# lexsightllc/DEWI-Design-for-an-Entropy-Weighted-Index-for-Text-Image-Corpora

Hardware: AMD Instinct MI355X
Metric: queries/sec + p50 latency, 1M×768 corpus, k=10, η=0.3, at 1/2/4/8 GPUs (higher is better)
Workload: dtype f32; 1 GPU; 1000000 docs x d=768 fp32, query batch=1, k=10, eta=0.3, brute-force cosine kNN + DEWI re-rank (BASELINE.json configs[1]); docs=1000000, dim=768, k=10, batch=1, candidates=20, parallelism=single GPU, queries_in_flight=1, rows_per_gpu=1000000, conditioning_steps_before_warmup=455

## Files before the change

### dewi-design-for-an-entropy-weighted-index-for-text-image-corpora_amd/csrc/abi.cpp

```cpp
#include <hip/hip_runtime.h>
#include <stdlib.h>

#include <cmath>
#include <cstdarg>
#include <cstdio>
#include <cstring>
#include <mutex>
#include <vector>

#include "launch.hpp"

namespace {

thread_local char g_err[512] = "";

int fail(int code, const char* fmt, ...) {
  va_list ap;
  va_start(ap, fmt);
  vsnprintf(g_err, sizeof(g_err), fmt, ap);
  va_end(ap);
  return code;
}
int hip_fail(hipError_t e, const char* what) {
  return fail(DEWI_ERR_HIP, "%s: %s", what, hipGetErrorString(e));
// ... 133 lines not shown
  return rp;
}

struct Batch {
  const void* d_E; int elem_type; int64_t n_rows; int dim;
  const float* d_Q; int n_queries;
  int space; hipStream_t stream;
};

struct SelectOut {
  int k; dewi::RerankParams rp;
  const float* d_dewi32; const float* d_ent32; int64_t id_offset;
  int64_t* d_out_ids; float* d_out_scores; dewi_candidate* d_out_cand;
};

int run_scan(const KnnLayout& L, const Batch& B, int n_candidates, char* ws, const uint32_t* d_filter = nullptr,
             const uint32_t* d_qwords = nullptr, int64_t n_union = 0) {
  uint64_t* keys = reinterpret_cast<uint64_t*>(ws + L.keys_off);
  float* qn = reinterpret_cast<float*>(ws + L.qn_off);
  hipError_t e;
  if (!L.plan.raw_queries) {
    e = dewi::launch_prepare_queries(B.d_Q, qn, B.n_queries, B.dim, B.space, B.elem_type ? 1 : 0, B.stream);
    if (e != hipSuccess) return hip_fail(e, "prepare_queries");
  }
  ScanTimer timer(B.stream);
  const float* q_prepared = L.plan.raw_queries ? nullptr : qn;
  int q = 0;
  while (q < B.n_queries) {
    static const bool nq8_enabled = [] { const char* e = getenv("DEWI_SCAN_NQ8"); return e == nullptr || atoi(e) != 0; }();
    const bool can8 = !B.elem_type && L.plan.fast && L.plan.slots == 1 && nq8_enabled;
    const int left = B.n_queries - q;
    const int nq = (can8 && left >= 8) ? 8 : ((L.plan.nq_max > 1 && left >= L.plan.nq_max) ? L.plan.nq_max : 1);
    if (d_filter) {
      dewi::QWords qw;
      if (d_qwords) {
        qw.words = d_qwords + static_cast<int64_t>(q / 32) * n_union;
        qw.shift = q % 32;
      }
      e = dewi::launch_scan_f32_filtered(L.plan, static_cast<const float*>(B.d_E), B.dim, B.d_Q, q_prepared, q, nq, n_candidates,
                                         B.space, keys, d_filter, B.stream, qw);
    } else if (B.elem_type) {
      e = dewi::launch_scan_bf16(L.plan, static_cast<const uint16_t*>(B.d_E), B.n_rows, B.dim, B.d_Q, q_prepared, q, nq,
                                 n_candidates, B.space, keys, B.stream);
    } else {
      e = dewi::launch_scan_f32(L.plan, static_cast<const float*>(B.d_E), B.n_rows, B.dim, B.d_Q, q_prepared, q, nq, n_candidates,
                                B.space, keys, B.stream);
    }
    if (e != hipSuccess) return hip_fail(e, "scan launch");
    q += nq;
  }
  return DEWI_OK;
}

int check_common(const Batch& B) {
  if (!B.d_E || !B.d_Q) return fail(DEWI_ERR_INVALID_ARG, "null embedding or query pointer");
  if (B.n_rows <= 0) return fail(DEWI_ERR_INVALID_ARG, "n_rows must be positive (got %lld)", static_cast<long long>(B.n_rows));
  if (B.n_rows > 0xFFFFFFFFll) return fail(DEWI_ERR_UNSUPPORTED, "n_rows %lld exceeds 2^32-1 rows per device", static_cast<long long>(B.n_rows));
  if (B.dim <= 0) return fail(DEWI_ERR_INVALID_ARG, "dim must be positive (got %d)", B.dim);
  if (B.n_queries <= 0) return fail(DEWI_ERR_INVALID_ARG, "n_queries must be positive (got %d)", B.n_queries);
  if (B.space != DEWI_SPACE_COSINE && B.space != DEWI_SPACE_L2) return fail(DEWI_ERR_INVALID_ARG, "unknown space %d", B.space);
  return DEWI_OK;
}

int resolve_cut(int k, int64_t n, int n_override, int* c) {
  int64_t c64 = (2ll * k < n) ? 2ll * k : n;
  if (n_override > 0) {
    if (n_override < k) return fail(DEWI_ERR_INVALID_ARG, "n_candidates %d must be at least k = %d", n_override, k);
    c64 = n_override < n ? n_override : n;
  }
  if (c64 > (1ll << 30)) return fail(DEWI_ERR_UNSUPPORTED, "candidate count %lld exceeds 2^30", static_cast<long long>(c64));
  *c = static_cast<int>(c64);
  return DEWI_OK;
}

enum class BatchPath { Rows, Depth, Big };
struct BatchPlan {
  BatchPath path;
  int c_local;
  KnnLayout rows;
  dewi::MfmaF32Layout depth;
  dewi::MfmaLayout big;
  bool shadow;
  size_t flags_off;
  size_t total;
};

bool plan_repair(BatchPlan& P, size_t path_total, int64_t n_rows, int dim, int corpus_elem_bytes, int n_queries, int n_candidates,
                 int cus) {
  if (n_candidates > dewi::kMaxSortCandidates) return false;
  P.rows = layout_knn(n_rows, dim, corpus_elem_bytes, n_queries, n_candidates, cus);
  if (!dewi::scan_flagged_supported(P.rows.plan, corpus_elem_bytes)) return false;
  P.flags_off = align_up(path_total > P.rows.total ? path_total : P.rows.total, 256);
  P.total = P.flags_off + align_up(static_cast<size_t>(n_queries) * 4, 256);
  return true;
}

BatchPlan plan_batch(int elem_type, int64_t n_rows, int dim, int n_queries, int n_candidates, int space, int cus) {
  BatchPlan P{};
  const int elem_bytes = elem_type ? 2 : 4;
  P.c_local = n_candidates < n_rows ? n_candidates : static_cast<int>(n_rows);
  const bool mfma = g_tuning.mfma != 0 && P.c_local == n_candidates &&
                    (space == DEWI_SPACE_COSINE || elem_type == 0 || g_tuning.mfma == 2);
  const bool depth_ok = mfma && dewi::mfma_f32_path_supported(elem_type, n_rows, dim, n_queries, n_candidates, space);
  const bool big_ok = mfma && elem_type == 1 && dewi::mfma_path_supported(n_rows, dim, n_queries, n_candidates, space);
  bool repairable = false;
  if (depth_ok && (elem_type == 0 || n_queries <= 32 || !big_ok)) {
    P.path = BatchPath::Depth;
    P.depth = dewi::plan_mfma_f32(elem_type, n_rows, dim, n_queries, n_candidates, cus);
    repairable = plan_repair(P, P.depth.total, n_rows, dim, elem_bytes, n_queries, n_candidates, cus);
  } else if (big_ok) {
    P.path = BatchPath::Big;
    P.big = dewi::plan_mfma(n_rows, dim, n_queries, n_candidates, cus);
    repairable = plan_repair(P, P.big.total, n_rows, dim, elem_bytes, n_queries, n_candidates, cus);
  }
  if (!repairable) {
    P.path = BatchPath::Rows;
    P.rows = layout_knn(n_rows, dim, elem_bytes, n_queries, P.c_local, cus);
    P.total = P.rows.total;
  }
  return P;
}

int batch_scan(const BatchPlan& P, const Batch& B, int n_candidates, void* d_ws, size_t ws_bytes, int cus) {
  if (int rc = check_workspace(d_ws, ws_bytes, P.total)) return rc;
  char* ws = static_cast<char*>(d_ws);
  switch (P.path) {
    case BatchPath::Depth:
      return launched(dewi::launch_mfma_f32(P.depth, B.elem_type, B.d_E, B.n_rows, B.dim, B.d_Q, B.n_queries, n_candidates, B.space,
                                            ws, B.stream),
                      "depth-split mfma scan launch");
    case BatchPath::Big:
      return launched(dewi::launch_mfma_bf16(P.big, static_cast<const uint16_t*>(B.d_E), B.n_rows, B.dim, B.d_Q, B.n_queries,
                                             n_candidates, B.space, ws, cus, B.stream),
                      "mfma scan launch");
    default:
      return run_scan(P.rows, B, P.c_local, ws);
  }
}

int batch_repair(const BatchPlan& P, char* ws, const Batch& B, const SelectOut& O, int n_candidates) {
  const KnnLayout& L = P.rows;
  uint32_t* flags = reinterpret_cast<uint32_t*>(ws + P.flags_off);
  uint64_t* keys = reinterpret_cast<uint64_t*>(ws + L.keys_off);
  hipError_t e = B.elem_type ? dewi::launch_scan_flagged_bf16(L.plan, static_cast<const uint16_t*>(B.d_E), B.n_rows, B.dim, B.d_Q,
                                                              B.n_queries, n_candidates, B.space, keys, flags, B.stream)
                             : dewi::launch_scan_flagged_f32(L.plan, static_cast<const float*>(B.d_E), B.n_rows, B.dim, B.d_Q,
                                                             B.n_queries, n_candidates, B.space, keys, flags, B.stream);
  if (e != hipSuccess) return hip_fail(e, "repair scan launch");
  const int sorted = L.plan.slots == 1 ? L.plan.n_lists : 0;
  e = dewi::launch_select_rerank(keys, L.plan.keys_per_query, sorted, B.n_queries, n_candidates, O.k, O.rp, O.d_dewi32, O.d_ent32,
                                 O.id_offset, O.d_out_ids, O.d_out_scores, O.d_out_cand, nullptr, dewi::SegmentLayout{}, B.stream,
                                 dewi::RefineParams{nullptr, nullptr, nullptr, 0, 0.f, 0}, dewi::QueryFlags{flags, 2});
  return launched(e, "repair select launch");
}

int batch_select(const BatchPlan& P, const Batch& B, const SelectOut& O, int n_candidates, void* d_ws, size_t ws_bytes) {
  if (int rc = check_workspace(d_ws, ws_bytes, P.total)) return rc;
  char* ws = static_cast<char*>(d_ws);
  const int n_queries = B.n_queries, k = O.k;
  hipError_t e = hipSuccess;
  if (P.path == BatchPath::Rows && P.c_local > dewi::kMaxSortCandidates) {
    const KnnLayout& L = P.rows;
    uint64_t* g1 = reinterpret_cast<uint64_t*>(ws + L.big_off);
    e = dewi::launch_select_rerank_large(reinterpret_cast<const uint64_t*>(ws + L.keys_off), L.plan.keys_per_query, n_queries,
                                         P.c_local, L.p2, k, O.rp, O.d_dewi32, O.d_ent32, O.id_offset, g1,
                                         g1 + static_cast<size_t>(n_queries) * L.p2, O.d_out_ids, O.d_out_scores, O.d_out_cand,
                                         n_candidates, B.stream);
    return launched(e, "select_rerank_large launch");
  }
  if (P.path == BatchPath::Rows) {
    const KnnLayout& L = P.rows;
    const int sorted = (L.plan.slots == 1 && P.c_local == n_candidates) ? L.plan.n_lists : 0;
    e = dewi::launch_select_rerank(reinterpret_cast<const uint64_t*>(ws + L.keys_off), L.plan.keys_per_query, sorted, n_queries,
                                   n_candidates, k, O.rp, O.d_dewi32, O.d_ent32, O.id_offset, O.d_out_ids, O.d_out_scores,
                                   O.d_out_cand, nullptr, dewi::SegmentLayout{}, B.stream);
    return launched(e, "select launch");
  }
  const bool big = P.path == BatchPath::Big;
  const int per = big ? 256 : 32;
  const int groups = big ? P.big.groups : P.depth.groups;
  const int n_seg = big ? P.big.n_seg : P.depth.n_seg;
  const int seg_cap = big ? P.big.seg_cap : P.depth.seg_cap;
  const size_t cand_off = big ? P.big.cand_off : P.depth.cand_off, cnt_off = big ? P.big.cnt_off : P.depth.cnt_off;
  static const int stage_override = [] { const char* e = getenv("DEWI_STAGE_KEYS"); return e ? atoi(e) : 0; }();
  const int stage_keys = stage_override > 0 ? stage_override : ((big && P.shadow) ? 12288 : 8192);
  const dewi::SegmentLayout seg{n_seg, seg_cap, 1, static_cast<int64_t>(per) * seg_cap, big ? 1 : per, stage_keys, big ? n_seg : 1};
  const bool refine_l2 = !big && B.space == DEWI_SPACE_L2 && B.elem_type == 0;
  if (!B.d_E || !B.d_Q) return fail(DEWI_ERR_INVALID_ARG, "a matrix-core batch needs the corpus and the raw queries in its finish step (repair of refused queries)");
  uint32_t* flags = reinterpret_cast<uint32_t*>(ws + P.flags_off);
  for (int g = 0; g < groups && e == hipSuccess; ++g) {
    const int q0 = g * per;
    const int nq = n_queries - q0 < per ? n_queries - q0 : per;
    const uint64_t* keys = reinterpret_cast<const uint64_t*>(ws + cand_off) + static_cast<int64_t>(g) * n_seg * per * seg_cap;
    const uint32_t* counts = reinterpret_cast<const uint32_t*>(ws + cnt_off) + static_cast<int64_t>(g) * n_seg * per;
    dewi::RefineParams rf{nullptr, nullptr, nullptr, 0, 0.f, 0};
    if (refine_l2)
      rf = dewi::RefineParams{static_cast<const float*>(B.d_E),
                              reinterpret_cast<const float*>(ws + P.depth.qn_off) + static_cast<int64_t>(q0) * B.dim,
                              reinterpret_cast<const float*>(ws + P.depth.qn2_off) + q0, B.dim, dewi::depth_l2_margin(B.dim),
                              DEWI_SPACE_L2};
    else if (P.shadow)
      rf = dewi::RefineParams{static_cast<const float*>(B.d_E), B.d_Q + static_cast<int64_t>(q0) * B.dim, nullptr, B.dim,
                              dewi::shadow_margin(B.dim), DEWI_SPACE_COSINE};
    e = dewi::launch_select_rerank(keys, 0, 0, nq, n_candidates, k, O.rp, O.d_dewi32, O.d_ent32, O.id_offset,
                                   O.d_out_ids ? O.d_out_ids + static_cast<int64_t>(q0) * k : nullptr,
                                   O.d_out_scores ? O.d_out_scores + static_cast<int64_t>(q0) * k : nullptr,
                                   O.d_out_cand ? O.d_out_cand + static_cast<int64_t>(q0) * n_candidates : nullptr, counts, seg,
                                   B.stream, rf, dewi::QueryFlags{flags + q0, 1});
  }
  if (e != hipSuccess) return hip_fail(e, "select launch");
  return batch_repair(P, ws, B, O, n_candidates);
}

int knn_rerank_impl(const Batch& B, const float* d_dewi32, const float* d_ent32, int k, double eta, double pref,
                    int64_t* d_out_ids, float* d_out_scores, void* d_ws, size_t ws_bytes, int n_candidates_override = 0,
                    int transform = DEWI_SIM_RAW) {
  int rc = check_common(B);
  if (rc) return rc;
  if (k <= 0) return DEWI_OK;
  if (k > B.n_rows)
    return fail(DEWI_ERR_K_OUT_OF_BOUNDS, "kth(=%lld) out of bounds (%lld)", static_cast<long long>(B.n_rows - k),
                static_cast<long long>(B.n_rows));
  if (!d_dewi32 || !d_ent32 || !d_out_ids || !d_out_scores) return fail(DEWI_ERR_INVALID_ARG, "null payload or output pointer");
  int c = 0;
  rc = resolve_cut(k, B.n_rows, n_candidates_override, &c);
  if (rc) return rc;
  DeviceInfo dev;
  rc = ensure_device(dev);
  if (rc) return rc;
  const BatchPlan P = plan_batch(B.elem_type, B.n_rows, B.dim, B.n_queries, c, B.space, dev.cus);
  rc = batch_scan(P, B, c, d_ws, ws_bytes, dev.cus);
  if (rc) return rc;
  const SelectOut O{k, make_rerank(eta, pref, transform, B.space), d_dewi32, d_ent32, 0, d_out_ids, d_out_scores, nullptr};
  return batch_select(P, B, O, c, d_ws, ws_bytes);
}

enum class ShadowMode { Plain, Lists, Big, Depth };
struct ShadowPlan {
  ShadowMode mode;
  int c;
  int list_len;
  KnnLayout lists;
  BatchPlan P;
};

ShadowPlan plan_shadow(bool have_shadow, int64_t n_rows, int dim, int n_queries, int k, int space, int cus) {
  ShadowPlan S{};
  S.mode = ShadowMode::Plain;
  S.P.shadow = true;
  const int64_t c64 = (2ll * k < n_rows) ? 2ll * k : n_rows;
  S.c = static_cast<int>(c64 < (1ll << 30) ? c64 : (1ll << 30));
  const bool usable = have_shadow && g_tuning.mfma != 0 && space == DEWI_SPACE_COSINE && k > 0 && k <= n_rows &&
                      dim % 8 == 0 && dim >= 136 && dim <= 1536;
  if (!usable) return S;
  const bool use_big = n_queries > 32 && c64 <= 512 && dewi::mfma_path_supported(n_rows, dim, n_queries, S.c, space);
  const bool use_depth = !use_big && c64 <= 256 &&
                         dewi::mfma_f32_path_supported(1, n_rows, dim, n_queries < dewi::kMfmaMinQueries ? dewi::kMfmaMinQueries : n_queries,
                                                       S.c, space);
  const int list_len = (n_queries == 1 && n_rows >= 64 * 1024) ? dewi::shadow_list_len(static_cast<int>(c64 < 64 ? c64 : 64)) : 0;
  if (list_len > 0) {
    S.lists = layout_knn(n_rows, dim, 2, 1, list_len, cus);
    if (S.lists.plan.fast && S.lists.plan.slots == 1 && S.lists.plan.n_lists <= 4 * 64 &&
        plan_repair(S.P, S.lists.total, n_rows, dim, 4, 1, S.c, cus)) {
      S.mode = ShadowMode::Lists;
      S.list_len = list_len;
      return S;
    }
  }
  S.P.c_local = S.c;
  if (use_big) {
    S.P.path = BatchPath::Big;
    S.P.big = dewi::plan_mfma(n_rows, dim, n_queries, S.c, cus, true);
    if (plan_repair(S.P, S.P.big.total, n_rows, dim, 4, n_queries, S.c, cus)) S.mode = ShadowMode::Big;
  } else if (use_depth) {
    S.P.path = BatchPath::Depth;
    S.P.depth = dewi::plan_mfma_f32(1, n_rows, dim, n_queries, S.c, cus, true);
    if (plan_repair(S.P, S.P.depth.total, n_rows, dim, 4, n_queries, S.c, cus)) S.mode = ShadowMode::Depth;
  }
  return S;
}

}

extern "C" {

int dewi_abi_version(void) { return DEWI_ABI_VERSION; }
const char* dewi_last_error(void) { return g_err; }

int dewi_device_info(int* out_compute_units, int* out_wavefront, size_t* out_total_mem) {
  DeviceInfo d;
  int rc = ensure_device(d);
  if (rc) return rc;
  if (out_compute_units) *out_compute_units = d.cus;
  if (out_wavefront) *out_wavefront = d.wave;
  if (out_total_mem) *out_total_mem = d.mem;
  return DEWI_OK;
}

int dewi_normalize_rows_f32(const float* d_src, float* d_dst, int64_t n_rows, int dim, void* stream) {
  if (n_rows < 0 || dim <= 0) return fail(DEWI_ERR_INVALID_ARG, "bad shape %lld x %d", static_cast<long long>(n_rows), dim);
  if (n_rows == 0) return DEWI_OK;
  if (!d_src || !d_dst) return fail(DEWI_ERR_INVALID_ARG, "null pointer");
  return launched(dewi::launch_normalize_rows(d_src, d_dst, n_rows, dim, static_cast<hipStream_t>(stream)), "normalize_rows launch");
}

int dewi_row_cosine_f32(const float* d_a, const float* d_b, float* d_out, int64_t n_rows, int dim, void* stream) {
  if (n_rows < 0 || dim <= 0) return fail(DEWI_ERR_INVALID_ARG, "bad shape %lld x %d", static_cast<long long>(n_rows), dim);
  if (n_rows == 0) return DEWI_OK;
  if (!d_a || !d_b || !d_out) return fail(DEWI_ERR_INVALID_ARG, "null pointer");
  return launched(dewi::launch_row_cosine(d_a, d_b, d_out, n_rows, dim, 1e-8f, static_cast<hipStream_t>(stream)), "row_cosine launch");
}

int dewi_convert_f32_to_bf16(const float* d_src, uint16_t* d_dst, int64_t n_elems, void* stream) {
  if (n_elems < 0) return fail(DEWI_ERR_INVALID_ARG, "negative element count");
  if (n_elems == 0) return DEWI_OK;
  if (!d_src || !d_dst) return fail(DEWI_ERR_INVALID_ARG, "null pointer");
  return launched(dewi::launch_f32_to_bf16(d_src, d_dst, n_elems, static_cast<hipStream_t>(stream)), "f32_to_bf16 launch");
}

int dewi_payload_soa_f64(const double* d_dewi, const double* d_ht_mean, const double* d_hi_mean, float* d_dewi32,
                         float* d_ent32, int64_t n_rows, void* stream) {
  if (n_rows < 0) return fail(DEWI_ERR_INVALID_ARG, "negative row count");
  if (n_rows == 0) return DEWI_OK;
  if (!d_dewi || !d_ht_mean || !d_hi_mean || !d_dewi32 || !d_ent32) return fail(DEWI_ERR_INVALID_ARG, "null pointer");
  return launched(dewi::launch_payload_soa(d_dewi, d_ht_mean, d_hi_mean, d_dewi32, d_ent32, n_rows, static_cast<hipStream_t>(stream)),
                  "payload_soa launch");
}

size_t dewi_knn_workspace_bytes(int64_t n_rows, int dim, int n_queries, int n_candidates) {
  DeviceInfo dev;
  if (ensure_device(dev)) return 0;
  if (n_rows <= 0 || dim <= 0 || n_queries <= 0 || n_candidates <= 0) return 0;
  size_t a = layout_knn(n_rows, dim, 4, n_queries, n_candidates, dev.cus).total;
  const size_t b = layout_knn(n_rows, dim, 2, n_queries, n_candidates, dev.cus).total;
  if (b > a) a = b;
  if (const int ll = dewi::shadow_list_len(n_candidates)) {
    const size_t s = layout_knn(n_rows, dim, 2, n_queries, ll, dev.cus).total;
    if (s > a) a = s;
  }
  if (dewi::mfma_path_supported(n_rows, dim, n_queries, n_candidates, DEWI_SPACE_COSINE)) {
    for (int pre = 0; pre < 2; ++pre) {
      const size_t m = dewi::plan_mfma(n_rows, dim, n_queries, n_candidates, dev.cus, pre != 0).total;
      if (m > a) a = m;
    }
  }
  for (int et = 0; et < 2; ++et) {
    const int nq = et == 1 && n_queries < dewi::kMfmaMinQueries ? dewi::kMfmaMinQueries : n_queries;
    if (dewi::mfma_f32_path_supported(et, n_rows, dim, nq, n_candidates, DEWI_SPACE_COSINE)) {
      for (int pre = 0; pre < 2; ++pre) {
        const size_t m = dewi::plan_mfma_f32(et, n_rows, dim, n_queries, n_candidates, dev.cus, pre != 0).total;
        if (m > a) a = m;
      }
    }
  }
  return align_up(a, 256) + align_up(static_cast<size_t>(n_queries) * 4, 256);
}

int dewi_knn_scan_kernel(int elem_type, int64_t n_rows, int dim, int n_queries, int n_candidates, int space, char* out,
                         size_t out_bytes) {
  if (!out || out_bytes < 16) return fail(DEWI_ERR_INVALID_ARG, "name buffer too small");
  if (n_rows <= 0 || dim <= 0 || n_queries <= 0 || n_candidates <= 0) return fail(DEWI_ERR_INVALID_ARG, "non-positive size");
  DeviceInfo dev;
  int rc = ensure_device(dev);
  if (rc) return rc;
  const BatchPlan P = plan_batch(elem_type, n_rows, dim, n_queries, n_candidates < n_rows ? n_candidates : static_cast<int>(n_rows),
                                 space, dev.cus);
  const char* e = elem_type ? "bf16" : "f32";
  if (P.path == BatchPath::Depth) {
    snprintf(out, out_bytes, "mfma_scan_f32<%s", elem_type ? "true" : "false");
  } else if (P.path == BatchPath::Big) {
    snprintf(out, out_bytes, "mfma_scan_bf16_s16");
  } else {
    const dewi::ScanPlan& p = P.rows.plan;
    const int nq = n_queries >= p.nq_max ? p.nq_max : 1;
    switch (p.kind) {
      case dewi::kScanFast: snprintf(out, out_bytes, "scan_rows_%s", e); break;
      case dewi::kScanAnyLong:
        if (p.odd_contig && nq == 1) {
          snprintf(out, out_bytes, "scan_rows_odd_contig<%d, %d, %d, %d, %d>", elem_type ? 1 : 0, p.u_pad, p.odd_contig_rows, space, p.slots);
          break;
        }
        snprintf(out, out_bytes, "scan_rows_any<%d, %d, %d, %d, %d, %d, %s>", elem_type ? 1 : 0, p.u_pad,
                                        nq > 1 ? p.rows_per_iter_batch : p.rows_per_iter, nq, space, p.slots,
                                        p.odd_rows ? "true" : "false"); break;
      case dewi::kScanAnyShort: snprintf(out, out_bytes, "scan_short_rows_any<%d, %d, %d, %d, %d, %s>", elem_type ? 1 : 0,
                                         p.rows_per_iter / (64 >> p.log2p), nq, space, p.slots, p.odd_rows ? "true" : "false"); break;
      default: snprintf(out, out_bytes, "scan_generic_%s", e); break;
    }
  }
  return DEWI_OK;
}

int dewi_knn_rerank_f32(const float* d_E, int64_t n_rows, int dim, const float* d_Q, int n_queries,
                        const float* d_dewi32, const float* d_ent32, int k, double eta, double entropy_pref, int space,
                        int64_t* d_out_ids, float* d_out_scores, void* d_workspace, size_t workspace_bytes,
                        void* stream) {
  return knn_rerank_impl(Batch{d_E, 0, n_rows, dim, d_Q, n_queries, space, static_cast<hipStream_t>(stream)}, d_dewi32, d_ent32, k,
                         eta, entropy_pref, d_out_ids, d_out_scores, d_workspace, workspace_bytes);
}

int dewi_knn_rerank_f32_shadow(const float* d_E, const uint16_t* d_E_bf16, int64_t n_rows, int dim, const float* d_Q,
                               int n_queries, const float* d_dewi32, const float* d_ent32, int k, double eta,
                               double entropy_pref, int space, int64_t* d_out_ids, float* d_out_scores, void* d_workspace,
                               size_t workspace_bytes, void* stream_) {
  const Batch B{d_E, 0, n_rows, dim, d_Q, n_queries, space, static_cast<hipStream_t>(stream_)};
  int rc = check_common(B);
  if (rc) return rc;
  DeviceInfo dev;
  rc = ensure_device(dev);
  if (rc) return rc;
  const ShadowPlan S = plan_shadow(d_E_bf16 != nullptr, n_rows, dim, n_queries, k, space, dev.cus);
  if (S.mode == ShadowMode::Plain)
    return knn_rerank_impl(B, d_dewi32, d_ent32, k, eta, entropy_pref, d_out_ids, d_out_scores, d_workspace, workspace_bytes);
  if (!d_dewi32 || !d_ent32 || !d_out_ids || !d_out_scores) return fail(DEWI_ERR_INVALID_ARG, "null payload or output pointer");
  const BatchPlan& P = S.P;
  rc = check_workspace(d_workspace, workspace_bytes, P.total);
  if (rc) return rc;
  char* ws = static_cast<char*>(d_workspace);
  hipStream_t stream = B.stream;
  const SelectOut O{k, make_rerank(eta, entropy_pref, DEWI_SIM_RAW, space), d_dewi32, d_ent32, 0, d_out_ids, d_out_scores, nullptr};
  if (S.mode == ShadowMode::Lists) {
    const KnnLayout& L = S.lists;
    rc = run_scan(L, Batch{d_E_bf16, 1, n_rows, dim, d_Q, 1, space, stream}, S.list_len, ws);
    if (rc) return rc;
    const dewi::RefineParams rf{d_E, d_Q, nullptr, dim, dewi::shadow_margin(dim), DEWI_SPACE_COSINE, S.list_len};
    const hipError_t e = dewi::launch_select_rerank(reinterpret_cast<const uint64_t*>(ws + L.keys_off), L.plan.keys_per_query,
                                                    L.plan.n_lists, 1, S.c, k, O.rp, d_dewi32, d_ent32, 0, d_out_ids, d_out_scores,
                                                    nullptr, nullptr, dewi::SegmentLayout{}, stream, rf,
                                                    dewi::QueryFlags{reinterpret_cast<uint32_t*>(ws + P.flags_off), 1});
    if (e != hipSuccess) return hip_fail(e, "select launch (one query, bf16 shadow)");
    return batch_repair(P, ws, B, O, S.c);
  }
  const float bias = 2.f * dewi::shadow_margin(dim);
  hipError_t e = S.mode == ShadowMode::Big
                     ? dewi::launch_mfma_bf16(P.big, d_E_bf16, n_rows, dim, d_Q, n_queries, S.c, space, ws, dev.cus, stream, bias)
                     : dewi::launch_mfma_f32(P.depth, 1, d_E_bf16, n_rows, dim, d_Q, n_queries, S.c, space, ws, stream, bias);
  if (e != hipSuccess) return hip_fail(e, "mfma scan launch (bf16 shadow)");
  return batch_select(P, B, O, S.c, d_workspace, workspace_bytes);
}

int dewi_knn_refusal_flags(int elem_type, int through_shadow, int64_t n_rows, int dim, int n_queries, int k, int n_candidates,
                           int space, size_t* out_offset_bytes) {
  if (!out_offset_bytes) return fail(DEWI_ERR_INVALID_ARG, "null pointer");
  if (n_rows <= 0 || dim <= 0 || n_queries <= 0) return fail(DEWI_ERR_INVALID_ARG, "non-positive size");
  DeviceInfo dev;
  int rc = ensure_device(dev);
  if (rc) return rc;
  *out_offset_bytes = static_cast<size_t>(-1);
  if (through_shadow && elem_type == 0) {
    const ShadowPlan S = plan_shadow(true, n_rows, dim, n_queries, k, space, dev.cus);
    if (S.mode != ShadowMode::Plain) {
      *out_offset_bytes = S.P.flags_off;
      return DEWI_OK;
    }
  }
  int64_t c64 = n_candidates > 0 ? n_candidates : 2ll * k;
  if (c64 > n_rows) c64 = n_rows;
  if (c64 <= 0 || c64 > (1ll << 30)) return DEWI_OK;
  const BatchPlan P = plan_batch(elem_type, n_rows, dim, n_queries, static_cast<int>(c64), space, dev.cus);
  if (P.path != BatchPath::Rows) *out_offset_bytes = P.flags_off;
  return DEWI_OK;
}

int dewi_knn_rerank_candidates(const void* d_E, int elem_type, int64_t n_rows, int dim, const float* d_Q, int n_queries,
                               const float* d_dewi32, const float* d_ent32, int k, int n_candidates, double eta,
                               double entropy_pref, int space, int sim_transform, int64_t* d_out_ids,
                               float* d_out_scores, void* d_workspace, size_t workspace_bytes, void* stream) {
  if (n_candidates <= 0) return fail(DEWI_ERR_INVALID_ARG, "n_candidates must be positive (got %d)", n_candidates);
  if (sim_transform != DEWI_SIM_RAW && sim_transform != DEWI_SIM_ONE_MINUS_DIST && sim_transform != DEWI_SIM_INV_ONE_PLUS_DIST)
    return fail(DEWI_ERR_INVALID_ARG, "unknown sim_transform %d", sim_transform);
  return knn_rerank_impl(Batch{d_E, elem_type, n_rows, dim, d_Q, n_queries, space, static_cast<hipStream_t>(stream)}, d_dewi32,
                         d_ent32, k, eta, entropy_pref, d_out_ids, d_out_scores, d_workspace, workspace_bytes, n_candidates,
                         sim_transform);
}

int dewi_prepare_queries_bf16(const float* d_Q, int n_queries, int dim, int space, uint16_t* d_out, void* stream) {
  if (!d_Q || !d_out) return fail(DEWI_ERR_INVALID_ARG, "null pointer");
  if (n_queries <= 0 || dim <= 0) return fail(DEWI_ERR_INVALID_ARG, "non-positive size");
  if (space != DEWI_SPACE_COSINE && space != DEWI_SPACE_L2) return fail(DEWI_ERR_INVALID_ARG, "unknown space %d", space);
  return launched(dewi::launch_prepare_queries_bf16(d_Q, d_out, n_queries, n_queries, dim, space, nullptr, static_cast<hipStream_t>(stream)),
                  "prepare_queries_bf16 launch");
}

int dewi_knn_scan(const void* d_E, int elem_type, int64_t n_rows, int dim, const float* d_Q, int n_queries,
                  int n_candidates, int space, void* d_workspace, size_t workspace_bytes, void* stream_) {
  const Batch B{d_E, elem_type, n_rows, dim, d_Q, n_queries, space, static_cast<hipStream_t>(stream_)};
  int rc = check_common(B);
  if (rc) return rc;
  if (n_candidates <= 0) return DEWI_OK;
  if (n_candidates > (1 << 30)) return fail(DEWI_ERR_UNSUPPORTED, "n_candidates %d exceeds 2^30", n_candidates);
  DeviceInfo dev;
  rc = ensure_device(dev);
  if (rc) return rc;
  const BatchPlan P = plan_batch(elem_type, n_rows, dim, n_queries, n_candidates, space, dev.cus);
  return batch_scan(P, B, n_candidates, d_workspace, workspace_bytes, dev.cus);
}

int dewi_knn_finish(void* d_workspace, size_t workspace_bytes, const void* d_E, int elem_type, int64_t n_rows, int dim,
                    const float* d_Q, int n_queries, int n_candidates, int space, int k, double eta, double entropy_pref,
                    const float* d_dewi32, const float* d_ent32, int64_t id_offset, int64_t* d_out_ids,
                    float* d_out_scores, dewi_candidate* d_out_cand, void* stream_) {
  if (n_rows <= 0 || dim <= 0 || n_queries <= 0) return fail(DEWI_ERR_INVALID_ARG, "non-positive size");
  if (space != DEWI_SPACE_COSINE && space != DEWI_SPACE_L2) return fail(DEWI_ERR_INVALID_ARG, "unknown space %d", space);
  if (n_candidates <= 0) return DEWI_OK;
  if (n_candidates > (1 << 30)) return fail(DEWI_ERR_UNSUPPORTED, "n_candidates %d exceeds 2^30", n_candidates);
  if (!d_dewi32 || !d_ent32) return fail(DEWI_ERR_INVALID_ARG, "null payload pointer");
  const bool records = d_out_cand != nullptr;
  if (!records) {
    if (k <= 0) return DEWI_OK;
    if (k > n_candidates) return fail(DEWI_ERR_K_OUT_OF_BOUNDS, "kth(=%d) out of bounds (%d)", n_candidates - k, n_candidates);
    if (!d_out_ids || !d_out_scores) return fail(DEWI_ERR_INVALID_ARG, "null output pointer");
  } else if (id_offset < 0 || id_offset + n_rows > 0x7FFFFFFFll) {
// ... 886 lines not shown
```

### dewi-design-for-an-entropy-weighted-index-for-text-image-corpora_amd/csrc/knn_scan.hip

```cpp
#include "scan_any.hpp"

namespace dewi {

template <int U, int R, int NQ, int SPACE, int S, bool NT, bool LIST = false, bool QMASK = false>
__device__ __forceinline__ void scan_rows_f32_body(const float* __restrict__ E, int64_t n_rows,
                                                   const float* __restrict__ Q, int n_candidates,
                                                   uint64_t* __restrict__ keys, int64_t keys_per_query,
                                                   MergeShared& merge_buf, const uint32_t* __restrict__ filt = nullptr,
                                                   const uint32_t* __restrict__ qword = nullptr, int qshift = 0) {
  constexpr int D4 = 64 * U;
  constexpr bool DENSE = S == 0;
  const int lane = lane_id();
  const int wave_in_block = static_cast<int>(threadIdx.x) >> 6;
  const int64_t gwave = static_cast<int64_t>(blockIdx.x) * (kScanThreads / kWave) + wave_in_block;
  const int64_t n_waves = static_cast<int64_t>(gridDim.x) * (kScanThreads / kWave);

  f32x4 qf[NQ][U];
#pragma unroll
  for (int qi = 0; qi < NQ; ++qi) {
    const f32x4* qp = reinterpret_cast<const f32x4*>(Q) + static_cast<int64_t>(qi) * D4 + lane;
#pragma unroll
    for (int u = 0; u < U; ++u) qf[qi][u] = qp[u * 64];
    if constexpr (SPACE == DEWI_SPACE_COSINE) {
      double ss = 0.0;
// ... 72 lines not shown
      for (int r = 0; r < R; ++r) consume(v[r], rows[r], row0 + r, qbits[r]);
      slot = (slot + 1) & (kWave - 1);
    }
  } else if constexpr (LIST) {
    uint32_t ahead[R];
    int slot = 0;
    for (int64_t g = gwave; g < n_groups; g += n_waves) {
      if (slot == 0) {
        const int64_t gl = g + static_cast<int64_t>(lane) * n_waves;
#pragma unroll
        for (int r = 0; r < R; ++r) ahead[r] = gl < n_groups ? list[gl * R + r] : 0u;
      }
      const int64_t row0 = g * R;
      int64_t rows[R];
      f32x4 v[R][U];
#pragma unroll
      for (int r = 0; r < R; ++r) {
        rows[r] = static_cast<uint32_t>(__builtin_amdgcn_readlane(static_cast<int>(ahead[r]), slot));
        const f32x4* p = Ev + rows[r] * D4 + lane;
#pragma unroll
        for (int u = 0; u < U; ++u) v[r][u] = load_x4<NT>(p + u * 64);
      }
#pragma unroll
      for (int r = 0; r < R; ++r) consume(v[r], rows[r], row0 + r);
      slot = (slot + 1) & (kWave - 1);
    }
  } else {
  for (int64_t g = gwave; g < n_groups; g += n_waves) {
    const int64_t row0 = g * R;
    f32x4 v[R][U];
#pragma unroll
    for (int r = 0; r < R; ++r) {
      const f32x4* p = Ev + row_of(row0 + r) * D4 + lane;
#pragma unroll
      for (int u = 0; u < U; ++u) v[r][u] = load_x4<NT>(p + u * 64);
    }
#pragma unroll
    for (int r = 0; r < R; ++r) consume(v[r], row_of(row0 + r), row0 + r);
  }
  }
  for (int64_t row = n_groups * R + gwave; row < n_rows; row += n_waves) {
    f32x4 v[U];
    const f32x4* p = Ev + row_of(row) * D4 + lane;
#pragma unroll
    for (int u = 0; u < U; ++u) v[u] = load_x4<NT>(p + u * 64);
    if constexpr (QMASK) consume(v, row_of(row), row, static_cast<uint32_t>(__builtin_amdgcn_readfirstlane(static_cast<int>(qword[row]))));
    else consume(v, row_of(row), row);
  }

  DEWI_STORE_LISTS(S, NQ, lst);
}

template <int U, int R, int NQ, int SPACE, int S, bool NT>
__global__ __launch_bounds__(kScanThreads) void scan_rows_f32(const float* __restrict__ E, int64_t n_rows,
                                                              const float* __restrict__ Q, int n_candidates,
                                                              uint64_t* __restrict__ keys,
                                                              int64_t keys_per_query) {
  __shared__ MergeShared merge_buf;
  scan_rows_f32_body<U, R, NQ, SPACE, S, NT>(E, n_rows, Q, n_candidates, keys, keys_per_query, merge_buf);
}

template <int U, int R, int NQ, int SPACE, int S, bool NT>
__global__ __launch_bounds__(kScanThreads) void scan_rows_f32_list(const float* __restrict__ E, const uint32_t* __restrict__ filt,
                                                                   const float* __restrict__ Q, int n_candidates,
                                                                   uint64_t* __restrict__ keys, int64_t keys_per_query) {
  __shared__ MergeShared merge_buf;
  scan_rows_f32_body<U, R, NQ, SPACE, S, NT, true>(E, 0, Q, n_candidates, keys, keys_per_query, merge_buf, filt);
}

template <int U, int R, int NQ, int SPACE, int S, bool NT>
__global__ __launch_bounds__(kScanThreads) void scan_rows_f32_qmask(const float* __restrict__ E, const uint32_t* __restrict__ filt,
                                                                    const uint32_t* __restrict__ qword, int qshift,
                                                                    const float* __restrict__ Q, int n_candidates,
                                                                    uint64_t* __restrict__ keys, int64_t keys_per_query) {
  __shared__ MergeShared merge_buf;
  scan_rows_f32_body<U, R, NQ, SPACE, S, NT, true, true>(E, 0, Q, n_candidates, keys, keys_per_query, merge_buf, filt, qword,
                                                          qshift);
}

template <int U, int R, int SPACE, int S>
__global__ __launch_bounds__(kScanThreads) void scan_rows_f32_flagged(const float* __restrict__ E, int64_t n_rows,
                                                                      const float* __restrict__ Q, int n_candidates,
                                                                      uint64_t* __restrict__ keys, int64_t keys_per_query,
                                                                      const uint32_t* __restrict__ flags, int n_queries) {
  __shared__ MergeShared merge_buf;
  for_each_flagged(flags, n_queries, [&](int q) {
    scan_rows_f32_body<U, R, 1, SPACE, S, true>(E, n_rows, Q + static_cast<int64_t>(q) * (256 * U), n_candidates,
                                                keys + static_cast<int64_t>(q) * keys_per_query, keys_per_query, merge_buf);
  });
}

template <int VEC>
struct VecT;
template <>
struct VecT<1> { using type = float; };
template <>
struct VecT<4> { using type = f32x4; };

template <int VEC, int NQ, int SPACE, int S>
__global__ __launch_bounds__(kScanThreads) void scan_generic_f32(const float* __restrict__ E, int64_t n_rows, int dim,
                                                                 const float* __restrict__ Qn, int group,
                                                                 int n_candidates, uint64_t* __restrict__ keys,
                                                                 int64_t keys_per_query) {
  using V = typename VecT<VEC>::type;
  constexpr bool DENSE = S == 0;
  __shared__ MergeShared merge_buf;
  const int lane = lane_id();
  const int wave_in_block = static_cast<int>(threadIdx.x) >> 6;
  const int64_t gwave = static_cast<int64_t>(blockIdx.x) * (kScanThreads / kWave) + wave_in_block;
  const int64_t n_waves = static_cast<int64_t>(gridDim.x) * (kScanThreads / kWave);
  const int rows_per_step = kWave / group;
  const int sub = lane / group;
  const int lg = lane % group;
  const int units = dim / VEC;

  ScanLists<S, NQ> lst;
  DEWI_INIT_LISTS(S, NQ, lst);

  const int64_t n_steps = (n_rows + rows_per_step - 1) / rows_per_step;
  for (int64_t st = gwave; st < n_steps; st += n_waves) {
    const int64_t row = st * rows_per_step + sub;
    float acc[NQ];
#pragma unroll
    for (int qi = 0; qi < NQ; ++qi) acc[qi] = 0.f;
    if (row < n_rows) {
      const V* ep = reinterpret_cast<const V*>(E + row * dim);
      for (int u = lg; u < units; u += group) {
        const V e = ep[u];
#pragma unroll
        for (int qi = 0; qi < NQ; ++qi) {
          const V q = reinterpret_cast<const V*>(Qn + static_cast<int64_t>(qi) * dim)[u];
          if constexpr (VEC == 4) {
            acc[qi] = accum4<SPACE>(e, q, acc[qi]);
          } else {
            if constexpr (SPACE == DEWI_SPACE_COSINE) {
              acc[qi] = __builtin_fmaf(e, q, acc[qi]);
            } else {
              const float d = e - q;
              acc[qi] = __builtin_fmaf(d, d, acc[qi]);
            }
          }
        }
      }
    }
    for (int off = group >> 1; off > 0; off >>= 1) {
#pragma unroll
      for (int qi = 0; qi < NQ; ++qi) acc[qi] += __shfl_xor(acc[qi], off, kWave);
    }
    for (int r = 0; r < rows_per_step; ++r) {
      const int64_t rr = st * rows_per_step + r;
      if (rr >= n_rows) break;
#pragma unroll
      for (int qi = 0; qi < NQ; ++qi) {
        float s = __shfl(acc[qi], r * group, kWave);
        if constexpr (SPACE == DEWI_SPACE_L2) s = -s;
        if constexpr (DENSE) {
          if (lane == 0) keys[qi * keys_per_query + rr] = make_key(s, static_cast<uint32_t>(rr));
        } else {
          lst[qi].offer(s, static_cast<uint32_t>(rr), lane);
        }
      }
    }
  }
  DEWI_STORE_LISTS(S, NQ, lst);
}

template <int VEC, int NQ, int SPACE, int S>
__global__ __launch_bounds__(kScanThreads) void scan_generic_f32_list(const float* __restrict__ E, const uint32_t* __restrict__ filt, int dim,
                                                                      const float* __restrict__ Qn, int group,
                                                                      int n_candidates, uint64_t* __restrict__ keys,
                                                                      int64_t keys_per_query) {
// ... 371 lines not shown

template <int U, int NQ, int SPACE, int S, bool LIST>
static bool launch_fast_r(const ScanPlan& plan, const float* E, int64_t n_rows, const float* Q, int c,
                          uint64_t* keys, hipStream_t stream, const uint32_t* filt, QWords qw) {
  const int r = NQ >= 4 ? plan.rows_per_iter_batch : plan.rows_per_iter;
  if (r >= 8) {
    if constexpr (U <= 3 && NQ == 1 && S == 1) {
      launch_fast_nt<U, 8, NQ, SPACE, S, LIST>(plan, E, n_rows, Q, c, keys, stream, filt, qw);
      return true;
    }
  }
  if (r >= 4) {
    if constexpr (U <= 3 && NQ == 1) {
      launch_fast_nt<U, 4, NQ, SPACE, S, LIST>(plan, E, n_rows, Q, c, keys, stream, filt, qw);
      return true;
    }
  }
  if (r >= 2) {
    if constexpr (U <= 3) {
      launch_fast_nt<U, 2, NQ, SPACE, S, LIST>(plan, E, n_rows, Q, c, keys, stream, filt, qw);
      return true;
    }
  }
  launch_fast_nt<U, 1, NQ, SPACE, S, LIST>(plan, E, n_rows, Q, c, keys, stream, filt, qw);
  return true;
}

template <int NQ, int SPACE, int S, bool LIST>
static bool launch_fast_u(const ScanPlan& plan, int dim, const float* E, int64_t n_rows, const float* Q, int c,
                          uint64_t* keys, hipStream_t stream, const uint32_t* filt, QWords qw) {
  switch (dim / 256) {
    case 1: return launch_fast_r<1, NQ, SPACE, S, LIST>(plan, E, n_rows, Q, c, keys, stream, filt, qw);
    case 2: return launch_fast_r<2, NQ, SPACE, S, LIST>(plan, E, n_rows, Q, c, keys, stream, filt, qw);
    case 3: return launch_fast_r<3, NQ, SPACE, S, LIST>(plan, E, n_rows, Q, c, keys, stream, filt, qw);
    case 4: return launch_fast_r<4, NQ, SPACE, S, LIST>(plan, E, n_rows, Q, c, keys, stream, filt, qw);
    case 6: return launch_fast_r<6, NQ, SPACE, S, LIST>(plan, E, n_rows, Q, c, keys, stream, filt, qw);
    default: return false;
  }
}

template <int NQ, int SPACE, int S, bool LIST>
static void launch_generic(const ScanPlan& plan, int dim, const float* E, int64_t n_rows, const float* Qn, int c,
                           uint64_t* keys, hipStream_t stream, const uint32_t* filt, QWords qw) {
  if constexpr (LIST) {
    if (qw.words) {
      if (plan.vec == 4)
        hipLaunchKernelGGL((scan_generic_f32_qmask<4, NQ, SPACE, S>), dim3(plan.blocks), dim3(kScanThreads), 0, stream, E,
                           filt, qw.words, qw.shift, dim, Qn, plan.group, c, keys, plan.keys_per_query);
      else
        hipLaunchKernelGGL((scan_generic_f32_qmask<1, NQ, SPACE, S>), dim3(plan.blocks), dim3(kScanThreads), 0, stream, E,
                           filt, qw.words, qw.shift, dim, Qn, plan.group, c, keys, plan.keys_per_query);
      return;
    }
    if (plan.vec == 4)
      hipLaunchKernelGGL((scan_generic_f32_list<4, NQ, SPACE, S>), dim3(plan.blocks), dim3(kScanThreads), 0, stream, E,
                         filt, dim, Qn, plan.group, c, keys, plan.keys_per_query);
    else
      hipLaunchKernelGGL((scan_generic_f32_list<1, NQ, SPACE, S>), dim3(plan.blocks), dim3(kScanThreads), 0, stream, E,
                         filt, dim, Qn, plan.group, c, keys, plan.keys_per_query);
    return;
  }
  if (plan.vec == 4)
    hipLaunchKernelGGL((scan_generic_f32<4, NQ, SPACE, S>), dim3(plan.blocks), dim3(kScanThreads), 0, stream, E,
                       n_rows, dim, Qn, plan.group, c, keys, plan.keys_per_query);
  else
    hipLaunchKernelGGL((scan_generic_f32<1, NQ, SPACE, S>), dim3(plan.blocks), dim3(kScanThreads), 0, stream, E,
                       n_rows, dim, Qn, plan.group, c, keys, plan.keys_per_query);
}

template <int NQ, int SPACE, int S, bool LIST = false>
static hipError_t launch_scan_impl(const ScanPlan& plan, const float* E, int64_t n_rows, int dim, const float* Qraw,
                                   const float* Qn, int c, uint64_t* keys, hipStream_t stream, const uint32_t* filt = nullptr,
                                   QWords qw = {}) {
  if (plan.fast) {
    if (!launch_fast_u<NQ, SPACE, S, LIST>(plan, dim, E, n_rows, Qraw, c, keys, stream, filt, qw)) return hipErrorInvalidValue;
  } else {
    launch_generic<NQ, SPACE, S, LIST>(plan, dim, E, n_rows, Qn, c, keys, stream, filt, qw);
  }
  return hipGetLastError();
}

template <int U, int SPACE>
static hipError_t launch_flagged_s(const ScanPlan& plan, const float* E, int64_t n_rows, const float* Q, int n_queries, int c,
                                   uint64_t* keys, const uint32_t* flags, hipStream_t stream) {
  constexpr int R = U == 1 ? 4 : (U == 2 ? 2 : 1);
  switch (plan.slots) {
    case 0:
      hipLaunchKernelGGL((scan_rows_f32_flagged<U, R, SPACE, 0>), dim3(plan.blocks), dim3(kScanThreads), 0, stream, E, n_rows, Q, c,
                         keys, plan.keys_per_query, flags, n_queries);
      break;
    case 1:
      hipLaunchKernelGGL((scan_rows_f32_flagged<U, R, SPACE, 1>), dim3(plan.blocks), dim3(kScanThreads), 0, stream, E, n_rows, Q, c,
                         keys, plan.keys_per_query, flags, n_queries);
      break;
    default:
      hipLaunchKernelGGL((scan_rows_f32_flagged<U, R, SPACE, kMaxSlots>), dim3(plan.blocks), dim3(kScanThreads), 0, stream, E, n_rows,
                         Q, c, keys, plan.keys_per_query, flags, n_queries);
      break;
  }
  return hipGetLastError();
}

bool scan_flagged_supported(const ScanPlan& plan, int elem_bytes) {
  (void)elem_bytes;
  if (plan.kind == kScanFast) return true;
  return !plan.odd_rows && (plan.kind == kScanAnyShort || (plan.kind == kScanAnyLong && plan.u_pad <= 8));
}

hipError_t launch_scan_flagged_f32(const ScanPlan& plan, const float* d_E, int64_t n_rows, int dim, const float* d_q_raw,
                                   int n_queries, int n_candidates, int space, uint64_t* d_keys, const uint32_t* d_flags,
                                   hipStream_t stream) {
  if (plan.kind == kScanAnyLong || plan.kind == kScanAnyShort)
    return launch_scan_any_flagged_f32(plan, d_E, n_rows, dim, d_q_raw, n_queries, n_candidates, space, d_keys, d_flags, stream);
  if (plan.kind != kScanFast) return hipErrorInvalidValue;
#define DEWI_FLAGGED(UU)                                                                                                 \
  case UU:                                                                                                               \
    return space == DEWI_SPACE_COSINE                                                                                    \
               ? launch_flagged_s<UU, DEWI_SPACE_COSINE>(plan, d_E, n_rows, d_q_raw, n_queries, n_candidates, d_keys, d_flags, stream) \
               : launch_flagged_s<UU, DEWI_SPACE_L2>(plan, d_E, n_rows, d_q_raw, n_queries, n_candidates, d_keys, d_flags, stream);
  switch (dim / 256) {
    DEWI_FLAGGED(1)
    DEWI_FLAGGED(2)
    DEWI_FLAGGED(3)
    DEWI_FLAGGED(4)
    DEWI_FLAGGED(6)
    default: break;
  }
#undef DEWI_FLAGGED
  return hipErrorInvalidValue;
}

template <bool LIST>
static hipError_t scan_f32_dispatch(const ScanPlan& plan, const float* d_E, int64_t n_rows, int dim, const float* d_q_raw,
                                    const float* d_q_norm, int q0, int nq, int n_candidates, int space, uint64_t* d_keys,
                                    hipStream_t stream, const uint32_t* filt, QWords qw) {
  if (plan.odd_rows)
    return LIST ? launch_scan_odd_f32_list(plan, d_E, dim, d_q_raw, q0, nq, n_candidates, space, d_keys, filt, stream, qw)
                : launch_scan_odd_f32(plan, d_E, n_rows, dim, d_q_raw, q0, nq, n_candidates, space, d_keys, stream);
  if (plan.kind == kScanAnyLong || plan.kind == kScanAnyShort)
    return LIST ? launch_scan_any_f32_list(plan, d_E, dim, d_q_raw, q0, nq, n_candidates, space, d_keys, filt, stream, qw)
                : launch_scan_any_f32(plan, d_E, n_rows, dim, d_q_raw, q0, nq, n_candidates, space, d_keys, stream);
  const float* qr = d_q_raw + static_cast<int64_t>(q0) * dim;
  const float* qn = d_q_norm ? d_q_norm + static_cast<int64_t>(q0) * dim : nullptr;
  uint64_t* keys = d_keys + static_cast<int64_t>(q0) * plan.keys_per_query;
#define DEWI_DISPATCH_S(NQ, SPACE)                                                                              \
  switch (plan.slots) {                                                                                          \
    case 0: return launch_scan_impl<NQ, SPACE, 0, LIST>(plan, d_E, n_rows, dim, qr, qn, n_candidates, keys, stream, filt, qw);   \
    case 1: return launch_scan_impl<NQ, SPACE, 1, LIST>(plan, d_E, n_rows, dim, qr, qn, n_candidates, keys, stream, filt, qw);   \
    default: return launch_scan_impl<NQ, SPACE, kMaxSlots, LIST>(plan, d_E, n_rows, dim, qr, qn, n_candidates, keys, stream, filt, qw); \
  }
#define DEWI_DISPATCH(NQ)                                  \
  if (space == DEWI_SPACE_COSINE) {                        \
    DEWI_DISPATCH_S(NQ, DEWI_SPACE_COSINE)                 \
  } else {                                                 \
    DEWI_DISPATCH_S(NQ, DEWI_SPACE_L2)                     \
  }
  if (nq == 1) {
    DEWI_DISPATCH(1)
  } else if (nq == 4) {
    DEWI_DISPATCH(4)
  } else if (nq == 8 && plan.fast && plan.slots == 1) {
    if (space == DEWI_SPACE_COSINE)
      return launch_scan_impl<8, DEWI_SPACE_COSINE, 1, LIST>(plan, d_E, n_rows, dim, qr, qn, n_candidates, keys, stream, filt, qw);
    return launch_scan_impl<8, DEWI_SPACE_L2, 1, LIST>(plan, d_E, n_rows, dim, qr, qn, n_candidates, keys, stream, filt, qw);
  }
#undef DEWI_DISPATCH
#undef DEWI_DISPATCH_S
  return hipErrorInvalidValue;
}

hipError_t launch_scan_f32(const ScanPlan& plan, const float* d_E, int64_t n_rows, int dim, const float* d_q_raw,
                           const float* d_q_norm, int q0, int nq, int n_candidates, int space, uint64_t* d_keys,
                           hipStream_t stream) {
  return scan_f32_dispatch<false>(plan, d_E, n_rows, dim, d_q_raw, d_q_norm, q0, nq, n_candidates, space, d_keys, stream, nullptr,
                                  QWords{});
}

hipError_t launch_scan_f32_filtered(const ScanPlan& plan, const float* d_E, int dim, const float* d_q_raw, const float* d_q_norm,
                                    int q0, int nq, int n_candidates, int space, uint64_t* d_keys, const uint32_t* d_filter,
                                    hipStream_t stream, QWords qw) {
  if (qw.words && (qw.shift < 0 || qw.shift + nq > 32)) return hipErrorInvalidValue;
  return scan_f32_dispatch<true>(plan, d_E, 0, dim, d_q_raw, d_q_norm, q0, nq, n_candidates, space, d_keys, stream, d_filter, qw);
}

}
```

### dewi-design-for-an-entropy-weighted-index-for-text-image-corpora_amd/csrc/knn_scan_any_bf16.hip

```cpp
#include "scan_any.hpp"

namespace dewi {

hipError_t launch_scan_any_bf16(const ScanPlan& plan, const uint16_t* d_E, int64_t n_rows, int dim, const float* d_q_raw, int q0,
                                int nq, int n_candidates, int space, uint64_t* d_keys, hipStream_t stream) {
  return launch_scan_any_impl<1>(plan, d_E, n_rows, dim, d_q_raw, q0, nq, n_candidates, space, d_keys, stream);
}

hipError_t launch_scan_any_flagged_bf16(const ScanPlan& plan, const uint16_t* d_E, int64_t n_rows, int dim, const float* d_q_raw,
                                        int n_queries, int n_candidates, int space, uint64_t* d_keys, const uint32_t* d_flags,
                                        hipStream_t stream) {
  (void)dim;
  return launch_scan_any_flagged_impl<1>(plan, d_E, n_rows, d_q_raw, n_queries, n_candidates, space, d_keys, d_flags, stream);
}

}
```

### dewi-design-for-an-entropy-weighted-index-for-text-image-corpora_amd/csrc/knn_scan_any_f32.hip

```cpp
#include "scan_any.hpp"

namespace dewi {

hipError_t launch_scan_any_f32(const ScanPlan& plan, const float* d_E, int64_t n_rows, int dim, const float* d_q_raw, int q0,
                               int nq, int n_candidates, int space, uint64_t* d_keys, hipStream_t stream) {
  return launch_scan_any_impl<0>(plan, d_E, n_rows, dim, d_q_raw, q0, nq, n_candidates, space, d_keys, stream);
}

hipError_t launch_scan_any_f32_list(const ScanPlan& plan, const float* d_E, int dim, const float* d_q_raw, int q0, int nq,
                                    int n_candidates, int space, uint64_t* d_keys, const uint32_t* d_filter, hipStream_t stream,
                                    QWords qw) {
  return launch_scan_any_impl<0, false, true>(plan, d_E, 0, dim, d_q_raw, q0, nq, n_candidates, space, d_keys, stream, d_filter, qw);
}

hipError_t launch_scan_any_flagged_f32(const ScanPlan& plan, const float* d_E, int64_t n_rows, int dim, const float* d_q_raw,
                                       int n_queries, int n_candidates, int space, uint64_t* d_keys, const uint32_t* d_flags,
                                       hipStream_t stream) {
  (void)dim;
  return launch_scan_any_flagged_impl<0>(plan, d_E, n_rows, d_q_raw, n_queries, n_candidates, space, d_keys, d_flags, stream);
}

}
```

### dewi-design-for-an-entropy-weighted-index-for-text-image-corpora_amd/csrc/knn_scan_bf16.hip

```cpp
#include "scan_common.hpp"

#ifndef DEWI_BF16_PAIRS
#define DEWI_BF16_PAIRS 2
#endif

namespace dewi {

template <int H, int NQ, int SPACE, int S, bool NT>
__device__ __forceinline__ void scan_rows_bf16_body(const uint16_t* __restrict__ E, int64_t n_rows,
                                                    const float* __restrict__ Q, int n_candidates,
                                                    uint64_t* __restrict__ keys, int64_t keys_per_query,
                                                    MergeShared& merge_buf) {
  constexpr int D = 256 * H;
  constexpr int UPR = 32 * H;
  constexpr bool DENSE = S == 0;
  const int lane = lane_id();
  const int wave_in_block = static_cast<int>(threadIdx.x) >> 6;
  const int64_t gwave = static_cast<int64_t>(blockIdx.x) * (kScanThreads / kWave) + wave_in_block;
  const int64_t n_waves = static_cast<int64_t>(gridDim.x) * (kScanThreads / kWave);

  bool second[H];
  float qf[NQ][H][8];
#pragma unroll
  for (int j = 0; j < H; ++j) second[j] = (64 * j + lane) >= UPR;
#pragma unroll
  for (int qi = 0; qi < NQ; ++qi) {
    double ss = 0.0;
#pragma unroll
    for (int j = 0; j < H; ++j) {
      const int unit = 64 * j + lane - (second[j] ? UPR : 0);
      const f32x4* qp = reinterpret_cast<const f32x4*>(Q + static_cast<int64_t>(qi) * D) + 2 * unit;
      const f32x4 a = qp[0], b = qp[1];
      qf[qi][j][0] = a.x; qf[qi][j][1] = a.y; qf[qi][j][2] = a.z; qf[qi][j][3] = a.w;
      qf[qi][j][4] = b.x; qf[qi][j][5] = b.y; qf[qi][j][6] = b.z; qf[qi][j][7] = b.w;
      if (!second[j]) {
#pragma unroll
        for (int i = 0; i < 8; ++i) ss += square_f64(qf[qi][j][i]);
      }
    }
    float norm = 1.f;
    bool scale = false;
    if constexpr (SPACE == DEWI_SPACE_COSINE) {
      norm = wave_query_norm(ss);
      scale = norm > 0.f;
    }
#pragma unroll
    for (int j = 0; j < H; ++j) {
#pragma unroll
      for (int i = 0; i < 8; ++i) {
        const float v = scale ? __fdiv_rn(qf[qi][j][i], norm) : qf[qi][j][i];
        qf[qi][j][i] = round_to_bf16(v);
      }
    }
  }

  uint32_t qp[NQ][H][4];
  if constexpr (SPACE == DEWI_SPACE_COSINE) {
#pragma unroll
    for (int qi = 0; qi < NQ; ++qi) {
#pragma unroll
      for (int j = 0; j < H; ++j) {
#pragma unroll
        for (int i = 0; i < 4; ++i)
          qp[qi][j][i] = (__float_as_uint(qf[qi][j][2 * i]) >> 16) | (__float_as_uint(qf[qi][j][2 * i + 1]) & 0xFFFF0000u);
      }
    }
  }
  auto dot = [&](u32x4 e, int qi, int j, float acc) {
    if constexpr (SPACE == DEWI_SPACE_COSINE) return dot8_packed(e, qp[qi][j], acc);
    else return dot8<SPACE>(e, qf[qi][j], acc);
  };

  ScanLists<S, NQ> lst;
  DEWI_INIT_LISTS(S, NQ, lst);

  auto finish_row = [&](int qi, float acc, int64_t row) {
    float s = wave_sum_f32(acc);
    if constexpr (SPACE == DEWI_SPACE_L2) s = -s;
    if constexpr (DENSE) {
      if (lane == 0) keys[qi * keys_per_query + row] = make_key(s, static_cast<uint32_t>(row));
    } else {
      lst[qi].offer(s, static_cast<uint32_t>(row), lane);
    }
  };
  auto consume_pair = [&](const u32x4(&v)[H], int64_t row0, bool has_second) {
#pragma unroll
    for (int qi = 0; qi < NQ; ++qi) {
      float a0 = 0.f, a1 = 0.f;
#pragma unroll
      for (int j = 0; j < H; ++j) {
        if (2 * j + 1 < H) {
          a0 = dot(v[j], qi, j, a0);
        } else if (2 * j >= H) {
          a1 = dot(v[j], qi, j, a1);
        } else {
          const float t = dot(v[j], qi, j, 0.f);
          a0 += second[j] ? 0.f : t;
          a1 += second[j] ? t : 0.f;
        }
      }
      finish_row(qi, a0, row0);
      if (has_second) finish_row(qi, a1, row0 + 1);
    }
  };

  const u32x4* Ev = reinterpret_cast<const u32x4*>(E);
  const int64_t n_pairs = n_rows >> 1;
  int64_t p = gwave;
  constexpr int P = DEWI_BF16_PAIRS;
  if constexpr (P > 1) {
    for (; p + (P - 1) * n_waves < n_pairs; p += P * n_waves) {
      u32x4 v[P][H];
#pragma unroll
      for (int u = 0; u < P; ++u) {
        const u32x4* base = Ev + (p + u * n_waves) * (2 * UPR) + lane;
#pragma unroll
        for (int j = 0; j < H; ++j) v[u][j] = load_u4<NT>(base + 64 * j);
      }
#pragma unroll
      for (int u = 0; u < P; ++u) consume_pair(v[u], 2 * (p + u * n_waves), true);
    }
  }
  for (; p < n_pairs; p += n_waves) {
    const u32x4* base = Ev + p * (2 * UPR) + lane;
    u32x4 v[H];
#pragma unroll
    for (int j = 0; j < H; ++j) v[j] = load_u4<NT>(base + 64 * j);
    consume_pair(v, 2 * p, true);
  }
  if ((n_rows & 1) && (n_pairs % n_waves) == gwave) {
    const u32x4* base = Ev + n_pairs * (2 * UPR) + lane;
    u32x4 v[H];
#pragma unroll
    for (int j = 0; j < H; ++j) {
      const u32x4 zero = {0u, 0u, 0u, 0u};
      v[j] = zero;
      if (!second[j]) v[j] = load_u4<NT>(base + 64 * j);
    }
    consume_pair(v, 2 * n_pairs, false);
  }

  DEWI_STORE_LISTS(S, NQ, lst);
}

template <int H, int NQ, int SPACE, int S, bool NT>
__global__ __launch_bounds__(kScanThreads) void scan_rows_bf16(const uint16_t* __restrict__ E, int64_t n_rows,
                                                               const float* __restrict__ Q, int n_candidates,
                                                               uint64_t* __restrict__ keys,
                                                               int64_t keys_per_query) {
  __shared__ MergeShared merge_buf;
  scan_rows_bf16_body<H, NQ, SPACE, S, NT>(E, n_rows, Q, n_candidates, keys, keys_per_query, merge_buf);
}

template <int H, int SPACE, int S>
__global__ __launch_bounds__(kScanThreads) void scan_rows_bf16_flagged(const uint16_t* __restrict__ E, int64_t n_rows,
                                                                       const float* __restrict__ Q, int n_candidates,
                                                                       uint64_t* __restrict__ keys, int64_t keys_per_query,
                                                                       const uint32_t* __restrict__ flags, int n_queries) {
  __shared__ MergeShared merge_buf;
  for_each_flagged(flags, n_queries, [&](int q) {
    scan_rows_bf16_body<H, 1, SPACE, S, true>(E, n_rows, Q + static_cast<int64_t>(q) * (256 * H), n_candidates,
                                              keys + static_cast<int64_t>(q) * keys_per_query, keys_per_query, merge_buf);
  });
}

template <int VEC, int NQ, int SPACE, int S>
__global__ __launch_bounds__(kScanThreads) void scan_generic_bf16(const uint16_t* __restrict__ E, int64_t n_rows, int dim,
                                                                  const float* __restrict__ Qn, int group,
                                                                  int n_candidates, uint64_t* __restrict__ keys,
                                                                  int64_t keys_per_query) {
  constexpr bool DENSE = S == 0;
  __shared__ MergeShared merge_buf;
  const int lane = lane_id();
  const int wave_in_block = static_cast<int>(threadIdx.x) >> 6;
  const int64_t gwave = static_cast<int64_t>(blockIdx.x) * (kScanThreads / kWave) + wave_in_block;
  const int64_t n_waves = static_cast<int64_t>(gridDim.x) * (kScanThreads / kWave);
  const int rows_per_step = kWave / group;
  const int sub = lane / group, lg = lane % group;
  const int units = dim / VEC;

  ScanLists<S, NQ> lst;
  DEWI_INIT_LISTS(S, NQ, lst);
  const int64_t n_steps = (n_rows + rows_per_step - 1) / rows_per_step;
  for (int64_t st = gwave; st < n_steps; st += n_waves) {
    const int64_t row = st * rows_per_step + sub;
    float acc[NQ];
#pragma unroll
    for (int qi = 0; qi < NQ; ++qi) acc[qi] = 0.f;
    if (row < n_rows) {
      const uint16_t* ep = E + row * dim;
      for (int u = lg; u < units; u += group) {
        if constexpr (VEC == 8) {
          const u32x4 e = reinterpret_cast<const u32x4*>(ep)[u];
#pragma unroll
          for (int qi = 0; qi < NQ; ++qi) {
            const f32x4* qp = reinterpret_cast<const f32x4*>(Qn + static_cast<int64_t>(qi) * dim) + 2 * u;
            const f32x4 a = qp[0], b = qp[1];
            const float q8[8] = {a.x, a.y, a.z, a.w, b.x, b.y, b.z, b.w};
            acc[qi] = dot8<SPACE>(e, q8, acc[qi]);
          }
        } else {
          const float e = __uint_as_float(static_cast<uint32_t>(ep[u]) << 16);
#pragma unroll
          for (int qi = 0; qi < NQ; ++qi) {
            const float q = Qn[static_cast<int64_t>(qi) * dim + u];
            if constexpr (SPACE == DEWI_SPACE_COSINE) {
              acc[qi] = __builtin_fmaf(e, q, acc[qi]);
            } else {
              const float d = e - q;
              acc[qi] = __builtin_fmaf(d, d, acc[qi]);
            }
          }
        }
      }
    }
    for (int off = group >> 1; off > 0; off >>= 1) {
#pragma unroll
      for (int qi = 0; qi < NQ; ++qi) acc[qi] += __shfl_xor(acc[qi], off, kWave);
    }
    for (int r = 0; r < rows_per_step; ++r) {
      const int64_t rr = st * rows_per_step + r;
      if (rr >= n_rows) break;
#pragma unroll
      for (int qi = 0; qi < NQ; ++qi) {
        float s = __shfl(acc[qi], r * group, kWave);
        if constexpr (SPACE == DEWI_SPACE_L2) s = -s;
        if constexpr (DENSE) {
          if (lane == 0) keys[qi * keys_per_query + rr] = make_key(s, static_cast<uint32_t>(rr));
        } else {
          lst[qi].offer(s, static_cast<uint32_t>(rr), lane);
        }
      }
    }
  }
  DEWI_STORE_LISTS(S, NQ, lst);
}

template <int H, int NQ, int SPACE, int S>
static void launch_fast_h(const ScanPlan& plan, const uint16_t* E, int64_t n_rows, const float* Q, int c, uint64_t* keys,
                          hipStream_t stream) {
  if (plan.nontemporal)
    hipLaunchKernelGGL((scan_rows_bf16<H, NQ, SPACE, S, true>), dim3(plan.blocks), dim3(kScanThreads), 0, stream, E,
                       n_rows, Q, c, keys, plan.keys_per_query);
  else
    hipLaunchKernelGGL((scan_rows_bf16<H, NQ, SPACE, S, false>), dim3(plan.blocks), dim3(kScanThreads), 0, stream, E,
                       n_rows, Q, c, keys, plan.keys_per_query);
}

template <int NQ, int SPACE, int S>
static hipError_t launch_bf16_impl(const ScanPlan& plan, const uint16_t* E, int64_t n_rows, int dim, const float* Qraw,
                                   const float* Qn, int c, uint64_t* keys, hipStream_t stream) {
  if (plan.fast) {
    switch (dim / 256) {
      case 1: launch_fast_h<1, NQ, SPACE, S>(plan, E, n_rows, Qraw, c, keys, stream); break;
      case 2: launch_fast_h<2, NQ, SPACE, S>(plan, E, n_rows, Qraw, c, keys, stream); break;
      case 3: launch_fast_h<3, NQ, SPACE, S>(plan, E, n_rows, Qraw, c, keys, stream); break;
      case 4: launch_fast_h<4, NQ, SPACE, S>(plan, E, n_rows, Qraw, c, keys, stream); break;
      default: return hipErrorInvalidValue;
    }
  } else if (plan.vec == 8) {
    hipLaunchKernelGGL((scan_generic_bf16<8, NQ, SPACE, S>), dim3(plan.blocks), dim3(kScanThreads), 0, stream, E,
                       n_rows, dim, Qn, plan.group, c, keys, plan.keys_per_query);
  } else {
    hipLaunchKernelGGL((scan_generic_bf16<1, NQ, SPACE, S>), dim3(plan.blocks), dim3(kScanThreads), 0, stream, E,
                       n_rows, dim, Qn, plan.group, c, keys, plan.keys_per_query);
  }
  return hipGetLastError();
}

template <int H, int SPACE>
static hipError_t launch_flagged_bf16_s(const ScanPlan& plan, const uint16_t* E, int64_t n_rows, const float* Q, int n_queries, int c,
                                        uint64_t* keys, const uint32_t* flags, hipStream_t stream) {
  switch (plan.slots) {
    case 0:
      hipLaunchKernelGGL((scan_rows_bf16_flagged<H, SPACE, 0>), dim3(plan.blocks), dim3(kScanThreads), 0, stream, E, n_rows, Q, c, keys,
                         plan.keys_per_query, flags, n_queries);
      break;
    case 1:
      hipLaunchKernelGGL((scan_rows_bf16_flagged<H, SPACE, 1>), dim3(plan.blocks), dim3(kScanThreads), 0, stream, E, n_rows, Q, c, keys,
                         plan.keys_per_query, flags, n_queries);
      break;
    default:
      hipLaunchKernelGGL((scan_rows_bf16_flagged<H, SPACE, kMaxSlots>), dim3(plan.blocks), dim3(kScanThreads), 0, stream, E, n_rows, Q,
                         c, keys, plan.keys_per_query, flags, n_queries);
      break;
  }
  return hipGetLastError();
}

hipError_t launch_scan_flagged_bf16(const ScanPlan& plan, const uint16_t* d_E, int64_t n_rows, int dim, const float* d_q_raw,
                                    int n_queries, int n_candidates, int space, uint64_t* d_keys, const uint32_t* d_flags,
                                    hipStream_t stream) {
  if (plan.kind == kScanAnyLong || plan.kind == kScanAnyShort)
    return launch_scan_any_flagged_bf16(plan, d_E, n_rows, dim, d_q_raw, n_queries, n_candidates, space, d_keys, d_flags, stream);
  if (plan.kind != kScanFast) return hipErrorInvalidValue;
#define DEWI_FLAGGED(HH)                                                                                                      \
  case HH:                                                                                                                    \
    return space == DEWI_SPACE_COSINE                                                                                         \
               ? launch_flagged_bf16_s<HH, DEWI_SPACE_COSINE>(plan, d_E, n_rows, d_q_raw, n_queries, n_candidates, d_keys, d_flags, stream) \
               : launch_flagged_bf16_s<HH, DEWI_SPACE_L2>(plan, d_E, n_rows, d_q_raw, n_queries, n_candidates, d_keys, d_flags, stream);
  switch (dim / 256) {
    DEWI_FLAGGED(1)
    DEWI_FLAGGED(2)
    DEWI_FLAGGED(3)
    DEWI_FLAGGED(4)
    default: break;
  }
#undef DEWI_FLAGGED
  return hipErrorInvalidValue;
}

hipError_t launch_scan_bf16(const ScanPlan& plan, const uint16_t* d_E, int64_t n_rows, int dim, const float* d_q_raw,
                            const float* d_q_norm, int q0, int nq, int n_candidates, int space, uint64_t* d_keys,
                            hipStream_t stream) {
  if (plan.odd_rows) return launch_scan_odd_bf16(plan, d_E, n_rows, dim, d_q_raw, q0, nq, n_candidates, space, d_keys, stream);
  if (plan.kind == kScanAnyLong || plan.kind == kScanAnyShort)
    return launch_scan_any_bf16(plan, d_E, n_rows, dim, d_q_raw, q0, nq, n_candidates, space, d_keys, stream);
  const float* qr = d_q_raw + static_cast<int64_t>(q0) * dim;
  const float* qn = d_q_norm ? d_q_norm + static_cast<int64_t>(q0) * dim : nullptr;
  uint64_t* keys = d_keys + static_cast<int64_t>(q0) * plan.keys_per_query;
#define DEWI_BF16_S(NQ, SPACE)                                                                                  \
  switch (plan.slots) {                                                                                         \
    case 0: return launch_bf16_impl<NQ, SPACE, 0>(plan, d_E, n_rows, dim, qr, qn, n_candidates, keys, stream);  \
    case 1: return launch_bf16_impl<NQ, SPACE, 1>(plan, d_E, n_rows, dim, qr, qn, n_candidates, keys, stream);  \
    default: return launch_bf16_impl<NQ, SPACE, kMaxSlots>(plan, d_E, n_rows, dim, qr, qn, n_candidates, keys, stream); \
  }
#define DEWI_BF16(NQ)                    \
  if (space == DEWI_SPACE_COSINE) {      \
    DEWI_BF16_S(NQ, DEWI_SPACE_COSINE)   \
  } else {                               \
    DEWI_BF16_S(NQ, DEWI_SPACE_L2)       \
  }
  if (nq == 1) {
    DEWI_BF16(1)
  } else if (nq == 4) {
    DEWI_BF16(4)
  }
#undef DEWI_BF16
#undef DEWI_BF16_S
  return hipErrorInvalidValue;
}

}
```

### dewi-design-for-an-entropy-weighted-index-for-text-image-corpora_amd/csrc/launch.hpp

```cpp
#pragma once
#include <hip/hip_runtime.h>
#include <stddef.h>
#include <stdint.h>

#include <mutex>

#include "../../include/dewi_hip.h"

namespace dewi {

struct PerDeviceOnce {
  std::mutex mu;
  uint64_t done[4] = {0, 0, 0, 0};
  template <class F>
  hipError_t run(F&& f) {
    int dev = 0;
    hipError_t e = hipGetDevice(&dev);
    if (e != hipSuccess) return e;
    std::lock_guard<std::mutex> lk(mu);
    const bool tracked = dev >= 0 && dev < 256;
    if (tracked && ((done[dev >> 6] >> (dev & 63)) & 1ull)) return hipSuccess;
    e = f();
    if (e == hipSuccess && tracked) done[dev >> 6] |= 1ull << (dev & 63);
    return e;
// ... 39 lines not shown
};

struct Tuning {
  int scan_blocks;
  int rows_per_iter;
  int nontemporal;
  int mfma;
};

void timing_begin(hipStream_t stream);
void timing_end(hipStream_t stream);

ScanPlan plan_scan(int64_t n_rows, int dim, int elem_bytes, int n_candidates, int compute_units,
                   const Tuning& tuning);

hipError_t launch_prepare_queries(const float* d_q, float* d_qn, int n_queries, int dim, int space, int to_bf16,
                                  hipStream_t stream);
hipError_t launch_prepare_queries_padded(const float* d_q, float* d_qn, int n_queries, int n_rows_out, int dim, int space,
                                         float* d_qn2, hipStream_t stream);
hipError_t launch_scan_f32(const ScanPlan& plan, const float* d_E, int64_t n_rows, int dim, const float* d_q_raw,
                           const float* d_q_norm, int q0, int nq, int n_candidates, int space, uint64_t* d_keys,
                           hipStream_t stream);

struct QWords {
  const uint32_t* words = nullptr;
  int shift = 0;
};

hipError_t launch_scan_f32_filtered(const ScanPlan& plan, const float* d_E, int dim, const float* d_q_raw, const float* d_q_norm,
                                    int q0, int nq, int n_candidates, int space, uint64_t* d_keys, const uint32_t* d_filter,
                                    hipStream_t stream, QWords qw = {});
hipError_t launch_scan_any_f32_list(const ScanPlan& plan, const float* d_E, int dim, const float* d_q_raw, int q0, int nq,
                                    int n_candidates, int space, uint64_t* d_keys, const uint32_t* d_filter, hipStream_t stream,
                                    QWords qw = {});
hipError_t launch_scan_odd_f32_list(const ScanPlan& plan, const float* d_E, int dim, const float* d_q_raw, int q0, int nq,
                                    int n_candidates, int space, uint64_t* d_keys, const uint32_t* d_filter, hipStream_t stream,
                                    QWords qw = {});
constexpr int kFilterHeaderWords = 16;
constexpr int kFilterMaxBuckets = 8;
int64_t filter_blocks(int64_t n_rows);
size_t filter_scratch_words(int64_t n_rows, int n_buckets);
hipError_t launch_filter_prepare(const uint8_t* d_mask, int64_t n_rows, int n_buckets, uint32_t* d_filter, uint32_t* d_scratch,
                                 hipStream_t stream);
hipError_t launch_query_filter_prepare(const uint8_t* d_masks, int64_t n_rows, int n_queries, int n_buckets, uint8_t* d_union,
                                       uint32_t* d_counts, uint32_t* d_filter, uint32_t* d_scratch, uint32_t* d_words,
                                       hipStream_t stream);

constexpr int kIvfMaxCells = 65536;
struct IvfListsLayout {
  int64_t bins, chunk, blocks;
  size_t rows_off, err_off, scratch_off, total_words;
};
inline IvfListsLayout ivf_lists_layout(int64_t n_rows, int n_cells, int n_buckets) {
  IvfListsLayout L;
  L.bins = static_cast<int64_t>(n_cells) * n_buckets;
  L.chunk = L.bins > 4096 ? (L.bins + 63) / 64 * 64 : 4096;
  L.blocks = (n_rows + L.chunk - 1) / L.chunk;
  L.rows_off = static_cast<size_t>(L.bins) + 1;
  L.err_off = L.rows_off + static_cast<size_t>(n_rows);
  L.scratch_off = L.err_off + 1;
  L.total_words = L.scratch_off + static_cast<size_t>(L.bins) * static_cast<size_t>(L.blocks);
  return L;
}
hipError_t launch_ivf_lists_build(const int32_t* d_assign, int64_t n_rows, int n_cells, int n_buckets, uint32_t* d_lists,
                                  hipStream_t stream);
struct IvfProbeLayout {
  int n_groups;
  size_t group_words, counts_off, bits_off, seg_off, total_words;
};
hipError_t launch_ivf_probe_prepare(const uint32_t* d_lists, int64_t n_rows, int n_cells, int n_buckets, const int64_t* d_probe_ids,
                                    int n_queries, int nprobe, int group, uint32_t* d_out, const IvfProbeLayout& L,
                                    hipStream_t stream);

hipError_t launch_scan_any_f32(const ScanPlan& plan, const float* d_E, int64_t n_rows, int dim, const float* d_q_raw, int q0,
                               int nq, int n_candidates, int space, uint64_t* d_keys, hipStream_t stream);
hipError_t launch_scan_any_bf16(const ScanPlan& plan, const uint16_t* d_E, int64_t n_rows, int dim, const float* d_q_raw, int q0,
                                int nq, int n_candidates, int space, uint64_t* d_keys, hipStream_t stream);

hipError_t launch_scan_odd_f32(const ScanPlan& plan, const float* d_E, int64_t n_rows, int dim, const float* d_q_raw, int q0,
                               int nq, int n_candidates, int space, uint64_t* d_keys, hipStream_t stream);
hipError_t launch_scan_odd_bf16(const ScanPlan& plan, const uint16_t* d_E, int64_t n_rows, int dim, const float* d_q_raw, int q0,
                                int nq, int n_candidates, int space, uint64_t* d_keys, hipStream_t stream);

bool scan_flagged_supported(const ScanPlan& plan, int elem_bytes);
hipError_t launch_scan_flagged_f32(const ScanPlan& plan, const float* d_E, int64_t n_rows, int dim, const float* d_q_raw,
                                   int n_queries, int n_candidates, int space, uint64_t* d_keys, const uint32_t* d_flags,
                                   hipStream_t stream);
hipError_t launch_scan_flagged_bf16(const ScanPlan& plan, const uint16_t* d_E, int64_t n_rows, int dim, const float* d_q_raw,
                                    int n_queries, int n_candidates, int space, uint64_t* d_keys, const uint32_t* d_flags,
                                    hipStream_t stream);
hipError_t launch_scan_any_flagged_f32(const ScanPlan& plan, const float* d_E, int64_t n_rows, int dim, const float* d_q_raw,
                                       int n_queries, int n_candidates, int space, uint64_t* d_keys, const uint32_t* d_flags,
                                       hipStream_t stream);
hipError_t launch_scan_any_flagged_bf16(const ScanPlan& plan, const uint16_t* d_E, int64_t n_rows, int dim, const float* d_q_raw,
                                        int n_queries, int n_candidates, int space, uint64_t* d_keys, const uint32_t* d_flags,
                                        hipStream_t stream);

hipError_t launch_scan_bf16(const ScanPlan& plan, const uint16_t* d_E, int64_t n_rows, int dim, const float* d_q_raw,
                            const float* d_q_norm, int q0, int nq, int n_candidates, int space, uint64_t* d_keys,
                            hipStream_t stream);

struct MfmaLayout {
  int groups;
  int q_pad;
  int64_t n_tiles;
  int64_t n_sample_tiles;
  int tile_stride;
  int64_t sample_stride;
  int n_blocks;
  int n_seg;
  int seg_cap;
  size_t qb_off, thr_off, cnt_off, dense_off, cand_off, total;
};
hipError_t launch_prepare_queries_bf16(const float* d_Q, uint16_t* d_out, int n_queries, int n_rows_out, int dim, int space,
                                       float* d_qn2, hipStream_t stream);
bool mfma_path_supported(int64_t n_rows, int dim, int n_queries, int n_candidates, int space);
MfmaLayout plan_mfma(int64_t n_rows, int dim, int n_queries, int n_candidates, int compute_units, bool preselect = false);
hipError_t launch_mfma_bf16(const MfmaLayout& m, const uint16_t* d_E, int64_t n_rows, int dim, const float* d_Q,
                            int n_queries, int n_candidates, int space, char* ws, int compute_units,
                            hipStream_t stream, float thr_bias = 0.f);
float shadow_margin(int dim);
hipError_t launch_mfma_bf16_filter(const uint16_t* d_E, int64_t n_rows, int dim, const uint16_t* d_qb, const float* d_thr,
                                   int n_active, float thr_bias, uint64_t* d_out, int seg_cap, uint32_t* d_cnt, int n_blocks,
                                   hipStream_t stream);
hipError_t launch_prepare_queries_bf16_frag(const float* d_Q, uint16_t* d_out, int n_queries, int n_rows_out, int dim,
                                            hipStream_t stream);

constexpr int kMfmaF32MinQueries = 5;
struct MfmaF32Layout {
  int groups;
  int q_pad;
  int64_t n_tiles;
  int64_t tile_stride;
  int64_t n_sample_tiles;
  int sample_blocks;
  int64_t sample_stride;
  int n_blocks;
  int n_seg;
  int seg_cap;
  size_t qn_off, qn2_off, thr_off, cnt_off, dense_off, cand_off, total;
};
bool mfma_f32_path_supported(int elem_type, int64_t n_rows, int dim, int n_queries, int n_candidates, int space);
float depth_l2_margin(int dim);
MfmaF32Layout plan_mfma_f32(int elem_type, int64_t n_rows, int dim, int n_queries, int n_candidates, int compute_units,
                            bool preselect = false);
hipError_t launch_mfma_f32(const MfmaF32Layout& m, int elem_type, const void* d_E, int64_t n_rows, int dim, const float* d_Q,
                           int n_queries, int n_candidates, int space, char* ws, hipStream_t stream, float thr_bias = 0.f);

hipError_t launch_sample_threshold(const float* dense, int64_t n_sample, int64_t stride, int n_candidates, float* thr,
                                   int n_queries, hipStream_t stream);

struct RerankParams {
  float w_sim;
  float w_dewi;
  float w_ent;
  int use_ent;
  int transform;
  int space;
};
struct SegmentLayout {
  int n_seg;
  int cap;
  int raw;
  int64_t seg_stride;
  int64_t count_stride;
  int lds_keys;
  int64_t count_query_stride;
};
struct RefineParams {
  const float* E;
  const float* Q;
  const float* qn2;
  int dim;
  float margin;
  int space;
  int list_len;
};
inline int shadow_list_len(int n_candidates) {
  if (n_candidates > 32) return 0;
  return n_candidates <= 16 ? 32 : 2 * n_candidates;
}
struct QueryFlags {
  uint32_t* p;
  int mode;
};
hipError_t launch_select_rerank(const uint64_t* d_keys, int64_t keys_per_query, int sorted_lists, int n_queries,
                                int n_candidates, int k, const RerankParams& rp, const float* d_dewi32, const float* d_ent32,
                                int64_t id_offset, int64_t* d_out_ids, float* d_out_scores,
                                dewi_candidate* d_out_cand, const uint32_t* d_counts, const SegmentLayout& seg,
                                hipStream_t stream, const RefineParams& refine = RefineParams{nullptr, nullptr, nullptr, 0, 0.f, 0},
                                const QueryFlags& flags = QueryFlags{nullptr, 0});
hipError_t launch_select_rerank_large(const uint64_t* d_keys, int64_t keys_per_query, int n_queries, int n_candidates,
                                      int p2, int k, const RerankParams& rp, const float* d_dewi32,
                                      const float* d_ent32, int64_t id_offset, uint64_t* d_g1, uint64_t* d_g2,
                                      int64_t* d_out_ids, float* d_out_scores, dewi_candidate* d_out_cand, int n_out,
                                      hipStream_t stream);
size_t merge_large_workspace_bytes(int n_queries, int n_candidates);
hipError_t launch_merge_rerank_large(const dewi_candidate* d_lists, int n_lists, int n_queries, int list_len,
                                     int n_candidates, int k, const RerankParams& rp, void* d_ws, int64_t* d_out_ids,
                                     float* d_out_scores, hipStream_t stream);
hipError_t launch_merge_rerank(const dewi_candidate* d_lists, int n_lists, int n_queries, int list_len,
                               int n_candidates, int k, const RerankParams& rp, int64_t* d_out_ids,
                               float* d_out_scores, hipStream_t stream);

int64_t range_chunks(int64_t n_scan);
hipError_t launch_range_count(const uint64_t* d_keys, int64_t n_scan, int n_queries, const float* d_thresholds,
                              uint32_t* d_chunk_counts, int64_t* d_counts, hipStream_t stream);
hipError_t launch_range_collect(const uint64_t* d_keys, int64_t n_scan, int n_queries, const float* d_thresholds,
                                const uint32_t* d_chunk_offsets, const int64_t* d_lims, int64_t capacity, const RerankParams& rp,
                                const float* d_dewi32, const float* d_ent32, int64_t* d_out_rows, float* d_out_sims,
                                float* d_out_scores, hipStream_t stream);

struct RangeShadowLayout {
  int groups;
  int q_pad;
  int n_blocks;
  int n_seg;
  int seg_cap;
  bool fits;
  size_t qb_off, cnt_off, offs_off, pass_off, flags_off, cand_off, total;
};
bool range_shadow_supported(int64_t n_rows, int dim, int space);
RangeShadowLayout plan_range_shadow(int64_t n_rows, int dim, int n_queries, int seg_cap, int compute_units);
hipError_t launch_range_shadow_count(const RangeShadowLayout& L, const float* d_E, const uint16_t* d_E_bf16, int64_t n_rows, int dim,
                                     int64_t first_row, const float* d_Q, int n_queries, const float* d_thresholds,
                                     int64_t* d_counts, char* ws, hipStream_t stream);
hipError_t launch_range_shadow_collect(const RangeShadowLayout& L, int64_t n_rows, int64_t first_row, int n_queries, const char* ws,
                                       const int64_t* d_lims, int64_t capacity, const RerankParams& rp, const float* d_dewi32,
                                       const float* d_ent32, int64_t* d_out_rows, float* d_out_sims, float* d_out_scores,
                                       hipStream_t stream);

constexpr int kGroupsHeaderWords = 16;
constexpr int kGroupsErrBadRow = 0;
constexpr int kGroupsErrGaveUp = 1;
struct GroupsLayout {
  size_t parent_off, count_off, members_off, best_off, total;
};
GroupsLayout groups_layout(int64_t n_rows);
hipError_t launch_groups_begin(const GroupsLayout& L, int64_t n_rows, char* ws, hipStream_t stream);
hipError_t launch_groups_union_lists(const GroupsLayout& L, int64_t n_rows, const int64_t* d_lims, const int64_t* d_rows,
                                     int n_queries, int64_t n_results, int64_t first_row, char* ws, hipStream_t stream);
hipError_t launch_groups_union_pairs(const GroupsLayout& L, int64_t n_rows, const int64_t* d_a, const int64_t* d_b, int64_t n_pairs,
                                     char* ws, hipStream_t stream);
hipError_t launch_groups_finish(const GroupsLayout& L, int64_t n_rows, int keep, const float* d_key, int64_t id_offset,
                                int64_t* d_labels, int64_t* d_sizes, int64_t* d_reps, char* ws, hipStream_t stream);

constexpr int kDiverseMaxCandidates = DEWI_DIVERSE_MAX_CANDIDATES;
hipError_t launch_diverse_rerank(const void* d_E, int elem_type, int64_t n_rows, int dim, const dewi_candidate* d_cand,
                                 int n_queries, int n_candidates, int k, const RerankParams& rp, float lam, float one_minus_lam,
                                 float max_sim, int64_t id_offset, int64_t* d_out_ids, float* d_out_scores, float* d_out_mmr,
                                 hipStream_t stream);

constexpr int kI8MaxCandidates = DEWI_I8_MAX_CANDIDATES;
constexpr int kI8MaxDim = DEWI_I8_MAX_DIM;
constexpr int kI8MaxBlocks = 256;
ScanPlan plan_scan_i8(int64_t n_rows, int dim, int n_candidates);
hipError_t launch_quantize_rows_i8(const float* d_E, int64_t n_rows, int dim, int8_t* d_codes, float* d_scales, hipStream_t stream);
hipError_t launch_prepare_queries_i8(const float* d_Q, int n_queries, int dim, int8_t* d_codes, float* d_scales, float* d_qn,
                                     hipStream_t stream);
hipError_t launch_scan_i8(const ScanPlan& plan, const int8_t* d_codes, const float* d_scales, int64_t n_rows, int dim,
                          const float* d_q_raw, int q0, int nq, int n_candidates, uint64_t* d_keys, hipStream_t stream);
hipError_t launch_rescore_candidates_f32(const float* d_E, int64_t n_rows, int dim, const float* d_Q, int n_queries,
                                         dewi_candidate* d_cand, int n_candidates, int64_t id_offset, hipStream_t stream);

hipError_t launch_rows_move(void* d_E, int elem_type, uint16_t* d_shadow, float* d_dewi32, float* d_ent32, int32_t* d_aux,
                            int64_t n_rows, int dim, int64_t n_keep, const int64_t* d_src, const int64_t* d_dst,
                            int64_t n_moves, int32_t* d_error, hipStream_t stream);
// ... 37 lines not shown
```

### dewi-design-for-an-entropy-weighted-index-for-text-image-corpora_amd/csrc/scan_any.hpp

```cpp
#pragma once
#include "scan_common.hpp"

namespace dewi {

template <int ELEM, int SPACE>
struct UnitFrag;

template <int SPACE>
struct UnitFrag<0, SPACE> {
  f32x4 q;
  __device__ __forceinline__ void load(const float* __restrict__ qrow, int unit, bool active) {
    q = f32x4{0.f, 0.f, 0.f, 0.f};
    if (active) q = reinterpret_cast<const f32x4*>(qrow)[unit];
  }
  __device__ __forceinline__ void load_shifted(const float* __restrict__ qrow, int first, int dim) {
    float t[4];
#pragma unroll
    for (int e = 0; e < 4; ++e) {
      const int idx = first + e;
      t[e] = static_cast<unsigned>(idx) < static_cast<unsigned>(dim) ? qrow[idx] : 0.f;
    }
    q = f32x4{t[0], t[1], t[2], t[3]};
  }
  __device__ __forceinline__ double sumsq() const { return square_f64(q.x) + square_f64(q.y) + square_f64(q.z) + square_f64(q.w); }
  __device__ __forceinline__ void scale(float norm) {
    q.x = __fdiv_rn(q.x, norm);
    q.y = __fdiv_rn(q.y, norm);
    q.z = __fdiv_rn(q.z, norm);
    q.w = __fdiv_rn(q.w, norm);
  }
  __device__ __forceinline__ void finish() {}
  __device__ __forceinline__ float dot(u32x4 e, float acc) const { return accum4<SPACE>(__builtin_bit_cast(f32x4, e), q, acc); }
};

template <int SPACE>
struct UnitFrag<1, SPACE> {
  float f[8];
  uint32_t p[4];
  __device__ __forceinline__ void load(const float* __restrict__ qrow, int unit, bool active) {
    f32x4 a = {0.f, 0.f, 0.f, 0.f}, b = {0.f, 0.f, 0.f, 0.f};
    if (active) {
      a = reinterpret_cast<const f32x4*>(qrow)[2 * unit];
      b = reinterpret_cast<const f32x4*>(qrow)[2 * unit + 1];
    }
    f[0] = a.x; f[1] = a.y; f[2] = a.z; f[3] = a.w;
    f[4] = b.x; f[5] = b.y; f[6] = b.z; f[7] = b.w;
  }
  __device__ __forceinline__ void load_shifted(const float* __restrict__ qrow, int first, int dim) {
#pragma unroll
    for (int e = 0; e < 8; ++e) {
      const int idx = first + e;
      f[e] = static_cast<unsigned>(idx) < static_cast<unsigned>(dim) ? qrow[idx] : 0.f;
    }
  }
  __device__ __forceinline__ double sumsq() const {
    double s = 0.0;
#pragma unroll
    for (int i = 0; i < 8; ++i) s += square_f64(f[i]);
    return s;
  }
  __device__ __forceinline__ void scale(float norm) {
#pragma unroll
    for (int i = 0; i < 8; ++i) f[i] = __fdiv_rn(f[i], norm);
  }
  __device__ __forceinline__ void finish() {
#pragma unroll
    for (int i = 0; i < 8; ++i) f[i] = round_to_bf16(f[i]);
    if constexpr (SPACE == DEWI_SPACE_COSINE) {
#pragma unroll
      for (int i = 0; i < 4; ++i) p[i] = (__float_as_uint(f[2 * i]) >> 16) | (__float_as_uint(f[2 * i + 1]) & 0xFFFF0000u);
    }
  }
  __device__ __forceinline__ float dot(u32x4 e, float acc) const {
    if constexpr (SPACE == DEWI_SPACE_COSINE) return dot8_packed(e, p, acc);
    else return dot8<SPACE>(e, f, acc);
  }
};

template <int ELEM>
__device__ __forceinline__ u32x4 unit_keep_mask(int first, int dim) {
  uint32_t m[4];
#pragma unroll
  for (int d = 0; d < 4; ++d) {
// ... 258 lines not shown
  for (int g = 0; g < G; ++g) {
    const int head = (off0 + g * row_bytes) & 15;
    const int head_el = head / kElemBytes;
    const int units = (head + row_bytes + 15) >> 4;
#pragma unroll
    for (int u = 0; u < U; ++u) {
      act[g][u] = lane + 64 * u < units;
      keep[g][u] = unit_keep_mask<ELEM>((lane + 64 * u) * kCols - head_el, dim);
      qf[g][u].load_shifted(Q, (lane + 64 * u) * kCols - head_el, dim);
    }
  }
  if constexpr (SPACE == DEWI_SPACE_COSINE) {
    const float norm = wave_query_norm(strided_sumsq(Q, dim, lane));
    if (norm > 0.f) {
#pragma unroll
      for (int g = 0; g < G; ++g) {
#pragma unroll
        for (int u = 0; u < U; ++u) qf[g][u].scale(norm);
      }
    }
  }
#pragma unroll
  for (int g = 0; g < G; ++g) {
#pragma unroll
    for (int u = 0; u < U; ++u) qf[g][u].finish();
  }

  WaveList<DENSE ? 1 : S> lst;
  if constexpr (!DENSE) lst.init(n_candidates, lane);

  auto fetch = [&](u32x4(&v)[U], int64_t row, const bool(&a)[U]) {
    const u32x4* p = E + ((off0 + row * row_bytes) >> 4) + lane;
#pragma unroll
    for (int u = 0; u < U; ++u) {
      v[u] = u32x4{0u, 0u, 0u, 0u};
      if (a[u]) v[u] = load_u4<true>(p + 64 * u);
    }
  };
  auto consume = [&](const u32x4(&v)[U], int64_t row, const u32x4(&k)[U], const UnitFrag<ELEM, SPACE>(&q)[U]) {
    float acc = 0.f;
#pragma unroll
    for (int u = 0; u < U; ++u) acc = q[u].dot(and_u4(v[u], k[u]), acc);
    float s = wave_sum_f32(acc);
    if constexpr (SPACE == DEWI_SPACE_L2) s = -s;
    if constexpr (DENSE) {
      if (lane == 0) keys[row] = make_key(s, static_cast<uint32_t>(row));
    } else {
      lst.offer(s, static_cast<uint32_t>(row), lane);
    }
  };

  const int64_t n_groups = n_rows / R;
  for (int64_t grp = gwave; grp < n_groups; grp += n_waves) {
    u32x4 v[R][U];
#pragma unroll
    for (int r = 0; r < R; ++r) fetch(v[r], grp * R + r, act[r % G]);
#pragma unroll
    for (int r = 0; r < R; ++r) consume(v[r], grp * R + r, keep[r % G], qf[r % G]);
  }
  for (int64_t row = n_groups * R + gwave; row < n_rows; row += n_waves) {
    const int g_row = static_cast<int>(row & (G - 1));
#pragma unroll
    for (int g = 0; g < G; ++g) {
      if (g_row == g) {
        u32x4 v[U];
        fetch(v, row, act[g]);
        consume(v, row, keep[g], qf[g]);
      }
    }
  }

  if constexpr (S == 1) {
    block_merge_store(lst, merge_buf, keys + static_cast<int64_t>(blockIdx.x) * n_candidates, n_candidates, lane, wave_in_block);
  } else if constexpr (!DENSE) {
    lst.store(keys + gwave * n_candidates, n_candidates, lane);
  }
}
constexpr int odd_contig_rows(int u, int rows_any) { return u == 1 ? (rows_any >= 12 ? 12 : 8) : (rows_any >= 6 ? 8 : 4); }

template <int ELEM, int U, int R, int SPACE, int S>
__global__ __launch_bounds__(kScanThreads) void scan_rows_any_flagged(const u32x4* __restrict__ E, int64_t n_rows, int units,
                                                                      const float* __restrict__ Q, int n_candidates,
                                                                      uint64_t* __restrict__ keys, int64_t keys_per_query,
                                                                      const uint32_t* __restrict__ flags, int n_queries) {
  __shared__ MergeShared merge_buf;
  const int dim = units * (ELEM ? 8 : 4);
  for_each_flagged(flags, n_queries, [&](int q) {
    scan_rows_any_body<ELEM, U, R, 1, SPACE, S>(E, n_rows, units, Q + static_cast<int64_t>(q) * dim, n_candidates,
                                                keys + static_cast<int64_t>(q) * keys_per_query, keys_per_query, merge_buf);
  });
}

__device__ __forceinline__ float group_sum_f32(float v, int log2p) {
#define DEWI_STEP(CTRL, MASK) v = v + __int_as_float(dpp_i32<CTRL, MASK>(0, __float_as_int(v)));
  if (log2p >= 1) { DEWI_STEP(0xB1, 0xF) }
  if (log2p >= 2) { DEWI_STEP(0x4E, 0xF) }
  if (log2p >= 3) { DEWI_STEP(0x141, 0xF) }
  if (log2p >= 4) { DEWI_STEP(0x140, 0xF) }
  if (log2p >= 5) { DEWI_STEP(0x142, 0xA) }
#undef DEWI_STEP
  return v;
}

template <int ELEM, int R, int NQ, int SPACE, int S, bool PH = false, bool LIST = false, bool QMASK = false>
__device__ __forceinline__ void scan_short_rows_any_body(const u32x4* __restrict__ E, int64_t n_rows, int units, int log2p,
                                                         const float* __restrict__ Q, int n_candidates,
                                                         uint64_t* __restrict__ keys, int64_t keys_per_query,
                                                         MergeShared& merge_buf, const uint32_t* __restrict__ filt = nullptr,
                                                         const uint32_t* __restrict__ qword = nullptr, int qshift = 0) {
  constexpr int kCols = ELEM ? 8 : 4;
  constexpr int kElemBytes = ELEM ? 2 : 4;
  constexpr bool DENSE = S == 0;
  const int lane = lane_id();
  const int wave_in_block = __builtin_amdgcn_readfirstlane(static_cast<int>(threadIdx.x) >> 6);
  const int64_t gwave = static_cast<int64_t>(blockIdx.x) * (kScanThreads / kWave) + wave_in_block;
  const int64_t n_waves = static_cast<int64_t>(gridDim.x) * (kScanThreads / kWave);
  const int dim = PH ? units : units * kCols;
  const int group = 1 << log2p;
  const int rows_per_load = kWave >> log2p;
  const int sub = lane >> log2p;
  const int pos = lane & (group - 1);
  int off0 = 0, row_bytes = 0, head_el = 0;
  [[maybe_unused]] u32x4 keep;
  [[maybe_unused]] ListPart part{0, gwave, n_waves, 0, 0};
  if constexpr (LIST) {
    const int n_buckets = PH ? 16 >> __builtin_ctz(static_cast<unsigned>(dim * kElemBytes) | 16u) : 1;
    part = list_part(filt, n_buckets, gwave, n_waves);
  }
  if constexpr (PH) {
    off0 = static_cast<int>(reinterpret_cast<uintptr_t>(E) & 15u);
    E = reinterpret_cast<const u32x4*>(reinterpret_cast<const char*>(E) - off0);
    row_bytes = dim * kElemBytes;
    const int row_step = 16 >> __builtin_ctz(static_cast<unsigned>(row_bytes) | 16u);
    const int head = (off0 + (LIST ? part.bucket : (sub & (row_step - 1))) * row_bytes) & 15;
    head_el = head / kElemBytes;
    units = (head + row_bytes + 15) >> 4;
    keep = unit_keep_mask<ELEM>(pos * kCols - head_el, dim);
  }
  const bool act = pos < units;
  const bool holder = pos == group - 1;

  UnitFrag<ELEM, SPACE> qf[NQ];
#pragma unroll
  for (int qi = 0; qi < NQ; ++qi) {
    const float* qrow = Q + static_cast<int64_t>(qi) * dim;
    if constexpr (PH) qf[qi].load_shifted(qrow, pos * kCols - head_el, dim);
    else qf[qi].load(qrow, pos, act);
    if constexpr (SPACE == DEWI_SPACE_COSINE) {
      const float norm = wave_query_norm(PH ? strided_sumsq(qrow, dim, lane) : (sub == 0 ? qf[qi].sumsq() : 0.0));
      if (norm > 0.f) qf[qi].scale(norm);
    }
    qf[qi].finish();
  }

  ScanLists<S, NQ> lst;
  DEWI_INIT_LISTS(S, NQ, lst);

  const int64_t rows_per_step = static_cast<int64_t>(rows_per_load) * R;
  if constexpr (LIST) {
    const uint32_t* __restrict__ list = filt + kFilterHeaderWords + part.base;
    const int64_t n_steps = (part.count + rows_per_step - 1) / rows_per_step;
    for (int64_t st = part.wave_pos; st < n_steps; st += part.wave_cnt) {
      u32x4 v[R];
      int64_t row[R];
      [[maybe_unused]] uint32_t qb[R];
#pragma unroll
      for (int r = 0; r < R; ++r) {
        const int64_t j = st * rows_per_step + static_cast<int64_t>(r) * rows_per_load + sub;
        row[r] = j < part.count ? static_cast<int64_t>(list[j]) : -1;
        if constexpr (QMASK) qb[r] = j < part.count ? qword[part.base + j] >> qshift : 0u;
      }
#pragma unroll
// ... 22 lines not shown
              m &= m - 1ull;
              const float sc = __int_as_float(__builtin_amdgcn_readlane(__float_as_int(s), src));
              const uint32_t rw = static_cast<uint32_t>(__builtin_amdgcn_readlane(static_cast<int>(static_cast<uint32_t>(row[r])), src));
              lst[qi].offer(sc, rw, lane);
            }
          }
        }
      }
    }
  } else {
  const int64_t n_steps = (n_rows + rows_per_step - 1) / rows_per_step;
  const int64_t load_units = PH ? (static_cast<int64_t>(rows_per_load) * row_bytes) >> 4 : static_cast<int64_t>(rows_per_load) * units;
  for (int64_t st = gwave; st < n_steps; st += n_waves) {
    const int64_t row_first = st * rows_per_step + sub;
    u32x4 v[R];
    const u32x4* p = E + (PH ? (off0 + row_first * row_bytes) >> 4 : row_first * units) + pos;
#pragma unroll
    for (int r = 0; r < R; ++r) {
      const int64_t row = row_first + static_cast<int64_t>(r) * rows_per_load;
      v[r] = u32x4{0u, 0u, 0u, 0u};
      if (act && row < n_rows) v[r] = load_u4<true>(p + r * load_units);
    }
#pragma unroll
    for (int r = 0; r < R; ++r) {
      const int64_t row = row_first + static_cast<int64_t>(r) * rows_per_load;
      const bool mine = holder && row < n_rows;
      if constexpr (PH) v[r] = and_u4(v[r], keep);
#pragma unroll
      for (int qi = 0; qi < NQ; ++qi) {
        float s = group_sum_f32(qf[qi].dot(v[r], 0.f), log2p);
        if constexpr (SPACE == DEWI_SPACE_L2) s = -s;
        if constexpr (DENSE) {
          if (mine) keys[qi * keys_per_query + row] = make_key(s, static_cast<uint32_t>(row));
        } else {
          unsigned long long m = __ballot(mine && !(s < lst[qi].thr_s));
          while (m != 0ull) {
            const int src = __ffsll(m) - 1;
            m &= m - 1ull;
            const float sc = __int_as_float(__builtin_amdgcn_readlane(__float_as_int(s), src));
            const uint32_t rw = static_cast<uint32_t>(__builtin_amdgcn_readlane(static_cast<int>(static_cast<uint32_t>(row)), src));
            lst[qi].offer(sc, rw, lane);
          }
        }
      }
    }
  }
  }

  DEWI_STORE_LISTS(S, NQ, lst);
}

template <int ELEM, int R, int NQ, int SPACE, int S, bool PH = false>
__global__ __launch_bounds__(kScanThreads) void scan_short_rows_any(const u32x4* __restrict__ E, int64_t n_rows, int units,
                                                                    int log2p, const float* __restrict__ Q, int n_candidates,
                                                                    uint64_t* __restrict__ keys, int64_t keys_per_query) {
  __shared__ MergeShared merge_buf;
  scan_short_rows_any_body<ELEM, R, NQ, SPACE, S, PH>(E, n_rows, units, log2p, Q, n_candidates, keys, keys_per_query, merge_buf);
}

template <int ELEM, int R, int NQ, int SPACE, int S, bool PH = false>
__global__ __launch_bounds__(kScanThreads) void scan_short_rows_any_list(const u32x4* __restrict__ E, const uint32_t* __restrict__ filt,
                                                                         int units, int log2p, const float* __restrict__ Q,
                                                                         int n_candidates, uint64_t* __restrict__ keys,
                                                                         int64_t keys_per_query) {
  __shared__ MergeShared merge_buf;
  scan_short_rows_any_body<ELEM, R, NQ, SPACE, S, PH, true>(E, 0, units, log2p, Q, n_candidates, keys, keys_per_query, merge_buf, filt);
}

template <int ELEM, int R, int NQ, int SPACE, int S, bool PH = false>
__global__ __launch_bounds__(kScanThreads) void scan_short_rows_any_qmask(const u32x4* __restrict__ E, const uint32_t* __restrict__ filt,
                                                                          const uint32_t* __restrict__ qword, int qshift, int units,
                                                                          int log2p, const float* __restrict__ Q, int n_candidates,
                                                                          uint64_t* __restrict__ keys, int64_t keys_per_query) {
  __shared__ MergeShared merge_buf;
  scan_short_rows_any_body<ELEM, R, NQ, SPACE, S, PH, true, true>(E, 0, units, log2p, Q, n_candidates, keys, keys_per_query, merge_buf,
                                                                  filt, qword, qshift);
}

template <int ELEM, int R, int SPACE, int S>
__global__ __launch_bounds__(kScanThreads) void scan_short_rows_any_flagged(const u32x4* __restrict__ E, int64_t n_rows, int units,
                                                                            int log2p, const float* __restrict__ Q,
                                                                            int n_candidates, uint64_t* __restrict__ keys,
                                                                            int64_t keys_per_query,
                                                                            const uint32_t* __restrict__ flags, int n_queries) {
  __shared__ MergeShared merge_buf;
  const int dim = units * (ELEM ? 8 : 4);
  for_each_flagged(flags, n_queries, [&](int q) {
    scan_short_rows_any_body<ELEM, R, 1, SPACE, S>(E, n_rows, units, log2p, Q + static_cast<int64_t>(q) * dim, n_candidates,
                                                   keys + static_cast<int64_t>(q) * keys_per_query, keys_per_query, merge_buf);
  });
}

template <int ELEM, int NQ, int SPACE, int S, bool PH, bool LIST = false>
static hipError_t launch_any_long(const ScanPlan& plan, const u32x4* E, int64_t n_rows, const float* Q, int c, uint64_t* keys,
                                  hipStream_t stream, const uint32_t* filt = nullptr, QWords qw = {}) {
  const int width = PH ? plan.row_cols : plan.units;
#define DEWI_ANY_LAUNCH(UU, RR)                                                                                          \
  if constexpr (LIST) {                                                                                                  \
    if (qw.words)                                                                                                        \
      hipLaunchKernelGGL((scan_rows_any_qmask<ELEM, UU, RR, NQ, SPACE, S, PH>), dim3(plan.blocks), dim3(kScanThreads), 0, stream,\
                         E, filt, qw.words, qw.shift, width, Q, c, keys, plan.keys_per_query);                           \
    else                                                                                                                 \
      hipLaunchKernelGGL((scan_rows_any_list<ELEM, UU, RR, NQ, SPACE, S, PH>), dim3(plan.blocks), dim3(kScanThreads), 0, stream,\
                         E, filt, width, Q, c, keys, plan.keys_per_query);                                               \
  } else {                                                                                                               \
    hipLaunchKernelGGL((scan_rows_any<ELEM, UU, RR, NQ, SPACE, S, PH>), dim3(plan.blocks), dim3(kScanThreads), 0, stream, E,\
                       n_rows, width, Q, c, keys, plan.keys_per_query);                                                  \
  }                                                                                                                      \
  return hipGetLastError();
#define DEWI_ANY_CASE(UU)                                                                                       \
  case UU:                                                                                                      \
    if constexpr (any_rows(UU, NQ, 0) != any_rows(UU, NQ, 1)) {                                                 \
      if (plan.level == 0) { DEWI_ANY_LAUNCH(UU, any_rows(UU, NQ, 0)) }                                         \
    }                                                                                                           \
    if constexpr (any_rows(UU, NQ, 2) != any_rows(UU, NQ, 1)) {                                                 \
      if (plan.level == 2) { DEWI_ANY_LAUNCH(UU, any_rows(UU, NQ, 2)) }                                         \
    }                                                                                                           \
    DEWI_ANY_LAUNCH(UU, any_rows(UU, NQ, 1))
  constexpr bool kNarrow = PH ? (NQ == 1 || NQ == 4) : (ELEM == 0 ? (NQ == 1 || NQ == 4) : true);
  constexpr bool kMiddle = PH ? NQ == 1 : (ELEM == 0 ? (NQ == 1 || NQ == 4) : (NQ == 1 || NQ == 2));
  constexpr bool kWide = PH ? NQ == 1 : (ELEM == 0 ? (NQ == 1 || NQ == 2) : NQ == 1);
  if constexpr (kNarrow && NQ != 2) {
    switch (plan.u_pad) {
      DEWI_ANY_CASE(1)
      DEWI_ANY_CASE(2)
      DEWI_ANY_CASE(3)
      DEWI_ANY_CASE(4)
      default: break;
    }
  }
  if constexpr (kMiddle) {
    switch (plan.u_pad) {
      DEWI_ANY_CASE(5)
      DEWI_ANY_CASE(6)
      DEWI_ANY_CASE(8)
      default: break;
    }
  }
  if constexpr (kWide) {
    switch (plan.u_pad) {
      DEWI_ANY_CASE(10)
      DEWI_ANY_CASE(12)
      DEWI_ANY_CASE(16)
      default: break;
    }
  }
#undef DEWI_ANY_LAUNCH
#undef DEWI_ANY_CASE
  return hipErrorInvalidValue;
}

template <int ELEM, int NQ, int SPACE, int S, bool PH, bool LIST = false>
static hipError_t launch_any_kind(const ScanPlan& plan, const u32x4* E, int64_t n_rows, const float* Q, int c, uint64_t* keys,
                                  hipStream_t stream, const uint32_t* filt = nullptr, QWords qw = {}) {
  if (plan.kind == kScanAnyShort) {
    if constexpr (NQ == 2) {
      return hipErrorInvalidValue;
    } else if constexpr (LIST) {
      if (qw.words) {
        hipLaunchKernelGGL((scan_short_rows_any_qmask<ELEM, kAnyShortRows, NQ, SPACE, S, PH>), dim3(plan.blocks), dim3(kScanThreads),
                           0, stream, E, filt, qw.words, qw.shift, PH ? plan.row_cols : plan.units, plan.log2p, Q, c, keys,
                           plan.keys_per_query);
        return hipGetLastError();
      }
      hipLaunchKernelGGL((scan_short_rows_any_list<ELEM, kAnyShortRows, NQ, SPACE, S, PH>), dim3(plan.blocks), dim3(kScanThreads), 0,
                         stream, E, filt, PH ? plan.row_cols : plan.units, plan.log2p, Q, c, keys, plan.keys_per_query);
      return hipGetLastError();
    } else {
      hipLaunchKernelGGL((scan_short_rows_any<ELEM, kAnyShortRows, NQ, SPACE, S, PH>), dim3(plan.blocks), dim3(kScanThreads), 0, stream,
                         E, n_rows, PH ? plan.row_cols : plan.units, plan.log2p, Q, c, keys, plan.keys_per_query);
      return hipGetLastError();
    }
  }
  return launch_any_long<ELEM, NQ, SPACE, S, PH, LIST>(plan, E, n_rows, Q, c, keys, stream, filt, qw);
}

template <int ELEM, bool PH = false, bool LIST = false>
static hipError_t launch_scan_any_impl(const ScanPlan& plan, const void* d_E, int64_t n_rows, int dim, const float* d_q_raw, int q0,
                                       int nq, int n_candidates, int space, uint64_t* d_keys, hipStream_t stream,
                                       const uint32_t* filt = nullptr, QWords qw = {}) {
  const u32x4* E = static_cast<const u32x4*>(d_E);
  const float* Q = d_q_raw + static_cast<int64_t>(q0) * dim;
  uint64_t* keys = d_keys + static_cast<int64_t>(q0) * plan.keys_per_query;
#define DEWI_ANY_S(NQ, SPACE)                                                                                        \
  switch (plan.slots) {                                                                                              \
    case 0: return launch_any_kind<ELEM, NQ, SPACE, 0, PH, LIST>(plan, E, n_rows, Q, n_candidates, keys, stream, filt, qw);          \
    case 1: return launch_any_kind<ELEM, NQ, SPACE, 1, PH, LIST>(plan, E, n_rows, Q, n_candidates, keys, stream, filt, qw);          \
    default: return launch_any_kind<ELEM, NQ, SPACE, kMaxSlots, PH, LIST>(plan, E, n_rows, Q, n_candidates, keys, stream, filt, qw); \
  }
#define DEWI_ANY_Q(NQ)                 \
  if (space == DEWI_SPACE_COSINE) {    \
    DEWI_ANY_S(NQ, DEWI_SPACE_COSINE)  \
  } else {                             \
    DEWI_ANY_S(NQ, DEWI_SPACE_L2)      \
  }
  if constexpr (PH && !LIST) {
    if (nq == 1 && plan.odd_contig) {
#define DEWI_ODD_CONTIG(UU, RR, SPACE)                                                                                              \
  switch (plan.slots) {                                                                                                             \
    case 0: hipLaunchKernelGGL((scan_rows_odd_contig<ELEM, UU, RR, SPACE, 0>), dim3(plan.blocks), dim3(kScanThreads), 0, stream, E,  \
                               n_rows, dim, Q, n_candidates, keys, plan.keys_per_query); break;                                      \
    case 1: hipLaunchKernelGGL((scan_rows_odd_contig<ELEM, UU, RR, SPACE, 1>), dim3(plan.blocks), dim3(kScanThreads), 0, stream, E,  \
                               n_rows, dim, Q, n_candidates, keys, plan.keys_per_query); break;                                      \
    default: hipLaunchKernelGGL((scan_rows_odd_contig<ELEM, UU, RR, SPACE, kMaxSlots>), dim3(plan.blocks), dim3(kScanThreads), 0,    \
                                stream, E, n_rows, dim, Q, n_candidates, keys, plan.keys_per_query); break;                          \
  }                                                                                                                                 \
  return hipGetLastError();
#define DEWI_ODD_CONTIG_R(UU, RR)                                       \
  if (plan.u_pad == UU && plan.odd_contig_rows == RR) {                  \
    if (space == DEWI_SPACE_COSINE) { DEWI_ODD_CONTIG(UU, RR, DEWI_SPACE_COSINE) } \
    else { DEWI_ODD_CONTIG(UU, RR, DEWI_SPACE_L2) }                      \
  }
      DEWI_ODD_CONTIG_R(1, 12)
      DEWI_ODD_CONTIG_R(1, 8)
      DEWI_ODD_CONTIG_R(2, 8)
      DEWI_ODD_CONTIG_R(2, 4)
#undef DEWI_ODD_CONTIG_R
#undef DEWI_ODD_CONTIG
      return hipErrorInvalidValue;
    }
  }
  if (nq == 1) {
    DEWI_ANY_Q(1)
  } else if (nq == 2) {
    if constexpr (!PH) { DEWI_ANY_Q(2) }
  } else if (nq == 4) {
    if constexpr (PH && ELEM == 1) {
      if (space != DEWI_SPACE_COSINE) {
        for (int i = 0; i < 4; ++i) {
          const hipError_t e = launch_scan_any_impl<ELEM, PH, LIST>(plan, d_E, n_rows, dim, d_q_raw, q0 + i, 1, n_candidates, space, d_keys,
                                                                    stream, filt, qw);
          if (e != hipSuccess) return e;
        }
        return hipSuccess;
      }
      DEWI_ANY_S(4, DEWI_SPACE_COSINE)
    } else {
      DEWI_ANY_Q(4)
    }
  }
#undef DEWI_ANY_Q
#undef DEWI_ANY_S
  return hipErrorInvalidValue;
}

template <int ELEM, int SPACE, int S>
static hipError_t launch_any_flagged_s(const ScanPlan& plan, const u32x4* E, int64_t n_rows, const float* Q, int n_queries, int c,
                                       uint64_t* keys, const uint32_t* flags, hipStream_t stream) {
  if (plan.kind == kScanAnyShort) {
    hipLaunchKernelGGL((scan_short_rows_any_flagged<ELEM, kAnyShortRows, SPACE, S>), dim3(plan.blocks), dim3(kScanThreads), 0, stream,
                       E, n_rows, plan.units, plan.log2p, Q, c, keys, plan.keys_per_query, flags, n_queries);
    return hipGetLastError();
  }
#define DEWI_ANY_FLAGGED(UU)                                                                                                     \
  case UU:                                                                                                                       \
    hipLaunchKernelGGL((scan_rows_any_flagged<ELEM, UU, any_rows(UU, 1, 1), SPACE, S>), dim3(plan.blocks), dim3(kScanThreads), 0,  \
                       stream, E, n_rows, plan.units, Q, c, keys, plan.keys_per_query, flags, n_queries);                         \
    return hipGetLastError();
  switch (plan.u_pad) {
    DEWI_ANY_FLAGGED(1)
    DEWI_ANY_FLAGGED(2)
    DEWI_ANY_FLAGGED(3)
    DEWI_ANY_FLAGGED(4)
    DEWI_ANY_FLAGGED(5)
    DEWI_ANY_FLAGGED(6)
    DEWI_ANY_FLAGGED(8)
    default: break;
  }
#undef DEWI_ANY_FLAGGED
  return hipErrorInvalidValue;
}

template <int ELEM>
static hipError_t launch_scan_any_flagged_impl(const ScanPlan& plan, const void* d_E, int64_t n_rows, const float* d_q_raw,
                                               int n_queries, int n_candidates, int space, uint64_t* d_keys,
                                               const uint32_t* d_flags, hipStream_t stream) {
  const u32x4* E = static_cast<const u32x4*>(d_E);
#define DEWI_ANY_FS(SPACE)                                                                                                         \
  switch (plan.slots) {                                                                                                            \
    case 0: return launch_any_flagged_s<ELEM, SPACE, 0>(plan, E, n_rows, d_q_raw, n_queries, n_candidates, d_keys, d_flags, stream); \
    case 1: return launch_any_flagged_s<ELEM, SPACE, 1>(plan, E, n_rows, d_q_raw, n_queries, n_candidates, d_keys, d_flags, stream); \
    default: return launch_any_flagged_s<ELEM, SPACE, kMaxSlots>(plan, E, n_rows, d_q_raw, n_queries, n_candidates, d_keys, d_flags, stream); \
  }
  if (space == DEWI_SPACE_COSINE) {
    DEWI_ANY_FS(DEWI_SPACE_COSINE)
  } else {
    DEWI_ANY_FS(DEWI_SPACE_L2)
  }
#undef DEWI_ANY_FS
}

}
```

### dewi-design-for-an-entropy-weighted-index-for-text-image-corpora_amd/csrc/select_rerank.hip

```cpp
#include <stdlib.h>

#include "blend.hpp"
#include "select_common.hpp"

namespace dewi {

__device__ __forceinline__ int pow2_at_least(int v) {
  int p = 2;
  while (p < v) p <<= 1;
  return p;
}

constexpr uint32_t kOrdNaN = 0xFFFFFFFFu;
__device__ __forceinline__ int emit_position(int j, bool is_nan, int kk, uint32_t n_nan) {
  const int z = n_nan < static_cast<uint32_t>(kk) ? static_cast<int>(n_nan) : kk;
  return is_nan ? kk - z + j : j - z;
}

template <class Fetch>
__device__ void rerank_and_emit(SelectShared& sh, uint32_t& n_nan, int n_sel, int k, const RerankParams& rp, Fetch fetch,
                                int64_t* __restrict__ out_ids, float* __restrict__ out_scores) {
  const int tid = static_cast<int>(threadIdx.x), nt = static_cast<int>(blockDim.x);
  const int p2 = pow2_at_least(n_sel);
  const int kk = k < n_sel ? k : n_sel;
  int64_t my_id = -1;
  for (int t = tid; t < p2; t += nt) {
    uint64_t k2 = kKeyEmpty;
    if (t < n_sel) {
      float dewi, ent;
      int64_t id;
      fetch(t, dewi, ent, id);
      if (t == tid) my_id = id;
      const float adj = blend(rp, key_score(sh.sel[t]), dewi, ent);
      if (adj != adj) atomicAdd(&n_nan, 1u);
      k2 = (static_cast<uint64_t>(ord_f32(adj)) << 32) | static_cast<uint64_t>(0xFFFFFFFFu - static_cast<uint32_t>(t));
    }
    sh.sel2[t] = k2;
  }
  if (n_sel <= kRankSortMax) {
    __syncthreads();
    const int S = rank_split(n_sel, nt);
    if (S == 1) {
      for (int t = tid; t < n_sel; t += nt) {
        const uint64_t mine = sh.sel2[t];
        int rank = 0;
#pragma unroll 4
        for (int j = 0; j < n_sel; ++j) rank += sh.sel2[j] > mine ? 1 : 0;
        if (rank < k) {
          int64_t id = my_id;
          if (t != tid) {
            float dewi, ent;
            fetch(t, dewi, ent, id);
          }
          const uint32_t hi = static_cast<uint32_t>(mine >> 32);
          const int at = emit_position(rank, hi == kOrdNaN, kk, n_nan);
          out_ids[at] = id;
          out_scores[at] = unord_f32(hi);
        }
      }
    } else {
      const int part = tid & (S - 1);
      for (int t = tid / S; t < n_sel; t += nt / S) {
        const uint64_t mine = sh.sel2[t];
        int rank = 0;
        const int iters = (n_sel + S - 1) / S;
#pragma unroll 8
        for (int i = 0; i < iters; ++i) {
          const int j = part + i * S;
          rank += sh.sel2[j < p2 ? j : p2 - 1] > mine ? 1 : 0;
        }
        for (int m = 1; m < S; m <<= 1) rank += __shfl_xor(rank, m, kWave);
        if (part == 0 && rank < k) {
          float dewi, ent;
          int64_t id;
          fetch(t, dewi, ent, id);
          const uint32_t hi = static_cast<uint32_t>(mine >> 32);
          const int at = emit_position(rank, hi == kOrdNaN, kk, n_nan);
          out_ids[at] = id;
          out_scores[at] = unord_f32(hi);
        }
      }
    }
    return;
  }
  bitonic_sort_desc<false>(sh.sel2, nullptr, p2);
  for (int j = tid; j < kk; j += nt) {
    const uint64_t k2 = sh.sel2[j];
    const int t = static_cast<int>(0xFFFFFFFFu - static_cast<uint32_t>(k2));
    float dewi, ent;
    int64_t id;
    fetch(t, dewi, ent, id);
    const uint32_t hi = static_cast<uint32_t>(k2 >> 32);
    const int at = emit_position(j, hi == kOrdNaN, kk, n_nan);
    out_ids[at] = id;
    out_scores[at] = unord_f32(hi);
  }
}

template <class Keys>
__device__ int exact_top_candidates(const Keys& keys, int n_candidates, SelectShared& sh) {
  const int tid = static_cast<int>(threadIdx.x), nt = static_cast<int>(blockDim.x);
  const uint64_t thr = block_kth_largest(keys, static_cast<uint32_t>(n_candidates), sh);
  if (tid == 0) sh.count = 0;
  const int p2 = pow2_at_least(n_candidates);
  for (int t = tid; t < p2; t += nt) sh.sel[t] = kKeyEmpty;
  __syncthreads();
  keys.for_each(tid, nt, [&](uint64_t key) {
    if (key >= thr) {
      const uint32_t pos = atomicAdd(&sh.count, 1u);
      if (pos < static_cast<uint32_t>(p2)) sh.sel[pos] = key;
    }
  });
  __syncthreads();
  const int n_sel = static_cast<int>(sh.count < static_cast<uint32_t>(n_candidates) ? sh.count : n_candidates);
  if (n_sel <= kRankSortMax && sh.count <= static_cast<uint32_t>(kRankSortMax)) {
    for (int t = tid; t < n_sel; t += nt) sh.sel2[t] = sh.sel[t];
    __syncthreads();
    rank_sort_desc(sh.sel2, sh.sel, n_sel);
    return n_sel;
  }
  bitonic_sort_desc<false>(sh.sel, nullptr, p2);
  return n_sel;
}

__device__ int top_candidates_lds(const uint64_t* keys, int n, int n_candidates, SelectShared& sh, WideRadixShared& ws) {
  const int tid = static_cast<int>(threadIdx.x), nt = static_cast<int>(blockDim.x);
  const uint64_t thr = block_kth_largest_lds(keys, n, static_cast<uint32_t>(n_candidates), ws);
  if (tid == 0) sh.count = 0;
  __syncthreads();
  for (int i = tid; i < n; i += nt) {
    const uint64_t key = keys[i];
    if (key >= thr) {
      const uint32_t pos = atomicAdd(&sh.count, 1u);
      sh.sel2[pos] = key;
    }
  }
  __syncthreads();
  const int n_sel = static_cast<int>(sh.count);
  if (n_sel <= kRankSortMax) {
    if (tid < kWave) sh.sel2[n_sel + tid] = kKeyEmpty;
    __syncthreads();
    rank_sort_desc<true>(sh.sel2, sh.sel, n_sel);
    return n_sel;
  }
  const int p2 = pow2_at_least(n_sel);
  for (int t = tid; t < p2; t += nt) sh.sel[t] = t < n_sel ? sh.sel2[t] : kKeyEmpty;
  bitonic_sort_desc<false>(sh.sel, nullptr, p2);
  return n_sel;
}

__device__ __forceinline__ float refine_bound(const RefineParams& rf, float q2, float a) {
  const float d = a < 0.f ? -a : 0.f;
  return a == a ? (rf.space == DEWI_SPACE_L2 ? rf.margin * (3.f * q2 + 2.f * d) * 1.01f : rf.margin) : __builtin_inff();
}
__device__ __forceinline__ float refine_low(const RefineParams& rf, float q2, uint64_t thr) {
  if (thr == 1ull) return -__builtin_inff();
  const float a_c = key_score(thr);
  const float low = a_c - refine_bound(rf, q2, a_c);
  return low == low ? low : -__builtin_inff();
}
__device__ __forceinline__ void refine_append(SelectShared& sh, bool pass, uint64_t key, int lane) {
  const unsigned long long m = __ballot(pass);
  if (m != 0ull) {
    uint32_t base = 0;
    if (lane == 0) base = atomicAdd(&sh.count, static_cast<uint32_t>(__popcll(m)));
    base = static_cast<uint32_t>(__builtin_amdgcn_readfirstlane(static_cast<int>(base)));
    const uint32_t pos = base + static_cast<uint32_t>(__popcll(m & ((1ull << lane) - 1ull)));
    if (pass && pos < static_cast<uint32_t>(kMaxSortCandidates)) sh.sel2[pos] = key;
  }
}

__device__ __forceinline__ int refine_rescore(uint64_t* keys, int n_candidates, SelectShared& sh, const RefineParams& rf, int q);

__device__ __forceinline__ int refine_top_candidates(uint64_t* keys, int n, int n_candidates, SelectShared& sh,
                                                     WideRadixShared& ws, const RefineParams& rf, int q) {
  const int tid = static_cast<int>(threadIdx.x), nt = static_cast<int>(blockDim.x);
  const int lane = tid & 63;
  const uint64_t thr = block_kth_largest_lds(keys, n, static_cast<uint32_t>(n_candidates), ws);
  const float q2 = rf.space == DEWI_SPACE_L2 ? rf.qn2[q] : 0.f;
  const float low = refine_low(rf, q2, thr);
  if (tid == 0) sh.count = 0;
  __syncthreads();
  for (int i0 = 0; i0 < n; i0 += nt) {
    const int i = i0 + tid;
    const uint64_t key = i < n ? keys[i] : kKeyEmpty;
    const float a = key_score(key);
    refine_append(sh, key != kKeyEmpty && !(a + refine_bound(rf, q2, a) < low), key, lane);
  }
  __syncthreads();
  return refine_rescore(keys, n_candidates, sh, rf, q);
}

__device__ __forceinline__ int refine_from_segments(const SegmentKeys& kv, uint64_t* scratch, int n_candidates, SelectShared& sh,
                                                    const RefineParams& rf, int q) {
  const int tid = static_cast<int>(threadIdx.x), nt = static_cast<int>(blockDim.x);
  const int lane = tid & 63;
  const uint64_t thr = block_kth_largest(kv, static_cast<uint32_t>(n_candidates), sh);
  const float q2 = rf.space == DEWI_SPACE_L2 ? rf.qn2[q] : 0.f;
  const float low = refine_low(rf, q2, thr);
  if (tid == 0) sh.count = 0;
  __syncthreads();
  constexpr int kGroup = 4;
  const int sub = tid % kGroup;
  for (int seg0 = 0; seg0 < kv.n_seg; seg0 += nt / kGroup) {
    const int seg = seg0 + tid / kGroup;
    uint32_t cnt = seg < kv.n_seg ? kv.count[seg * kv.count_stride] : 0u;
// ... 76 lines not shown
  const int n4 = rf.dim >> 2;
  const int units = (n4 + 63) >> 6;
  bool have[kMaxUnits];
#pragma unroll
  for (int u = 0; u < kMaxUnits; ++u) have[u] = lane + 64 * u < n4;
  typedef float f32x4r __attribute__((ext_vector_type(4)));
  const f32x4r* qp = reinterpret_cast<const f32x4r*>(rf.Q + static_cast<int64_t>(q) * rf.dim) + lane;
  f32x4r qv[kMaxUnits];
#pragma unroll
  for (int u = 0; u < kMaxUnits; ++u) {
    qv[u] = f32x4r{0.f, 0.f, 0.f, 0.f};
    if (u < units && have[u]) qv[u] = qp[u * 64];
  }
  if (!l2) {
    double ss = 0.0;
#pragma unroll
    for (int u = 0; u < kMaxUnits; ++u)
      if (u < units) ss += square_f64(qv[u].x) + square_f64(qv[u].y) + square_f64(qv[u].z) + square_f64(qv[u].w);
    const float norm = wave_query_norm(ss);
    if (norm > 0.f) {
#pragma unroll
      for (int u = 0; u < kMaxUnits; ++u) {
        qv[u].x = __fdiv_rn(qv[u].x, norm);
        qv[u].y = __fdiv_rn(qv[u].y, norm);
        qv[u].z = __fdiv_rn(qv[u].z, norm);
        qv[u].w = __fdiv_rn(qv[u].w, norm);
      }
    }
  }
  for (int t0 = wave * kBatch; t0 < n_cand; t0 += n_waves * kBatch) {
    f32x4r e[kBatch][kMaxUnits];
    uint32_t rows[kBatch];
#pragma unroll
    for (int bb = 0; bb < kBatch; ++bb) {
      const int t = t0 + bb < n_cand ? t0 + bb : t0;
      rows[bb] = key_row(sh.sel2[t]);
      const f32x4r* ev = reinterpret_cast<const f32x4r*>(rf.E + static_cast<int64_t>(rows[bb]) * rf.dim) + lane;
#pragma unroll
      for (int u = 0; u < kMaxUnits; ++u) {
        e[bb][u] = f32x4r{0.f, 0.f, 0.f, 0.f};
        if (u < units && have[u]) e[bb][u] = ev[u * 64];
      }
    }
#pragma unroll
    for (int bb = 0; bb < kBatch; ++bb) {
      float acc = 0.f;
#pragma unroll
      for (int u = 0; u < kMaxUnits; ++u) {
        if (u < units) {
          if (l2) {
            float d;
            d = e[bb][u].x - qv[u].x; acc = __builtin_fmaf(d, d, acc);
            d = e[bb][u].y - qv[u].y; acc = __builtin_fmaf(d, d, acc);
            d = e[bb][u].z - qv[u].z; acc = __builtin_fmaf(d, d, acc);
            d = e[bb][u].w - qv[u].w; acc = __builtin_fmaf(d, d, acc);
          } else {
            acc = __builtin_fmaf(e[bb][u].x, qv[u].x, acc);
            acc = __builtin_fmaf(e[bb][u].y, qv[u].y, acc);
            acc = __builtin_fmaf(e[bb][u].z, qv[u].z, acc);
            acc = __builtin_fmaf(e[bb][u].w, qv[u].w, acc);
          }
        }
      }
      const float sum = wave_sum_f32(acc);
      const float sc = l2 ? -sum : sum;
      if (lane == 0 && t0 + bb < n_cand) keys[t0 + bb] = make_key(sc, rows[bb]);
    }
  }
  __syncthreads();
  if (n_cand <= 1024) {
    rank_sort_desc(keys, sh.sel, n_cand);
  } else {
    const int p2 = pow2_at_least(n_cand);
    for (int t = tid; t < p2; t += nt) sh.sel[t] = t < n_cand ? keys[t] : kKeyEmpty;
    bitonic_sort_desc<false>(sh.sel, nullptr, p2);
  }
  return n_cand < n_candidates ? n_cand : n_candidates;
}
__device__ __forceinline__ int refine_rescore(uint64_t* keys, int n_candidates, SelectShared& sh, const RefineParams& rf, int q) {
  if (rf.dim > 1024) return refine_rescore_units<6, 2>(keys, n_candidates, sh, rf, q);
  return refine_rescore_units<4, 4>(keys, n_candidates, sh, rf, q);
}

__device__ int gather_top_candidates(const uint64_t* __restrict__ keys, int64_t keys_per_query, int sorted_lists,
                                     int n_candidates, SelectShared& sh) {
  const int tid = static_cast<int>(threadIdx.x), nt = static_cast<int>(blockDim.x);
  if (sorted_lists > 0 && sorted_lists <= 4 * kWave && n_candidates <= kWave) {
    if (tid == 0) {
      sh.n_contrib = 0;
      sh.count = 0;
    }
    __syncthreads();
    if (tid < kWave) {
      uint64_t m[4];
      uint64_t lane_max = kKeyEmpty;
#pragma unroll
      for (int u = 0; u < 4; ++u) {
        const int l = tid + kWave * u;
        m[u] = l < sorted_lists ? keys[static_cast<int64_t>(l) * n_candidates] : kKeyEmpty;
        lane_max = m[u] > lane_max ? m[u] : lane_max;
      }
      const uint32_t mh = static_cast<uint32_t>(lane_max >> 32), ml = static_cast<uint32_t>(lane_max);
      int rank = 0;
#pragma unroll
      for (int j = 0; j < kWave; ++j) {
        const uint64_t o = (static_cast<uint64_t>(static_cast<uint32_t>(__builtin_amdgcn_readlane(static_cast<int>(mh), j))) << 32) |
                           static_cast<uint32_t>(__builtin_amdgcn_readlane(static_cast<int>(ml), j));
        rank += (o > lane_max || (o == lane_max && j < tid)) ? 1 : 0;
      }
      const unsigned long long who = __ballot(rank == n_candidates - 1);
      uint64_t bound = 1ull;
      if (who != 0ull) {
        const int src = __ffsll(who) - 1;
        bound = (static_cast<uint64_t>(static_cast<uint32_t>(__builtin_amdgcn_readlane(static_cast<int>(mh), src))) << 32) |
                static_cast<uint32_t>(__builtin_amdgcn_readlane(static_cast<int>(ml), src));
        if (bound == kKeyEmpty) bound = 1ull;
      }
#pragma unroll
      for (int u = 0; u < 4; ++u) {
        if (m[u] != kKeyEmpty && m[u] >= bound) sh.val[atomicAdd(&sh.n_contrib, 1u)] = static_cast<uint32_t>(tid + kWave * u);
      }
      if (tid == 0) sh.bound = bound;
    }
    __syncthreads();
    const uint64_t bound = sh.bound;
    for (int t = tid; t < static_cast<int>(sh.n_contrib); t += nt) {
      const uint64_t* lst = keys + static_cast<int64_t>(sh.val[t]) * n_candidates;
      for (int j = 0; j < n_candidates; ++j) {
        const uint64_t key = lst[j];
        if (key == kKeyEmpty || key < bound) break;
        const uint32_t pos = atomicAdd(&sh.count, 1u);
        if (pos < static_cast<uint32_t>(kMaxSortCandidates)) sh.sel2[pos] = key;
      }
    }
    __syncthreads();
    const int survivors = static_cast<int>(sh.count);
    if (survivors <= kRankSortMax) {
      rank_sort_desc(sh.sel2, sh.sel, survivors);
      return survivors < n_candidates ? survivors : n_candidates;
    }
    if (survivors <= kMaxSortCandidates) {
      const int p2 = pow2_at_least(survivors);
      for (int t = tid; t < p2; t += nt) sh.sel[t] = t < survivors ? sh.sel2[t] : kKeyEmpty;
      bitonic_sort_desc<false>(sh.sel, nullptr, p2);
      return survivors < n_candidates ? survivors : n_candidates;
    }
    __syncthreads();
  } else
  if (sorted_lists > 0 && sorted_lists <= kMaxSortCandidates) {
    uint64_t second = kKeyEmpty;
    for (int t = tid; t < sorted_lists; t += nt) {
      const uint64_t* lst = keys + static_cast<int64_t>(t) * n_candidates;
      sh.sel2[t] = lst[0];
      if (t == tid && n_candidates > 1) second = lst[1];
    }
    if (tid == 0) {
      sh.count = 0;
      sh.total = 0;
      sh.pick_digit = 0;
    }
    __syncthreads();
    const bool all_lists = sorted_lists < n_candidates;
    for (int t = tid; t < sorted_lists; t += nt) sh.val[t] = 0;
    __syncthreads();
    const int parts = nt / sorted_lists > 1 ? nt / sorted_lists : 1;
    const int slice = (sorted_lists + parts - 1) / parts;
    for (int idx = tid; idx < sorted_lists * parts; idx += nt) {
      const int t = idx / parts, part = idx % parts;
      const uint64_t mine = sh.sel2[t];
      const int j0 = part * slice, j1 = j0 + slice < sorted_lists ? j0 + slice : sorted_lists;
      uint32_t cnt = 0;
      for (int j = j0; j < j1; ++j) {
        const uint64_t o = sh.sel2[j];
        cnt += (o > mine || (o == mine && j < t)) ? 1u : 0u;
      }
      if (cnt) atomicAdd(&sh.val[t], cnt);
    }
    __syncthreads();
    for (int t = tid; t < sorted_lists; t += nt) {
      if (sh.val[t] == static_cast<uint32_t>(n_candidates - 1)) {
        sh.pick_digit = static_cast<uint32_t>(t);
        sh.total = 1;
      }
    }
    __syncthreads();
    uint64_t bound = 1ull;
    if (!all_lists && sh.total != 0) bound = sh.sel2[sh.pick_digit];
    if (bound == kKeyEmpty) bound = 1ull;
    __syncthreads();
    for (int t = tid; t < sorted_lists; t += nt) {
      if (!all_lists && sh.val[t] >= static_cast<uint32_t>(n_candidates)) continue;
      const uint64_t* lst = keys + static_cast<int64_t>(t) * n_candidates;
      for (int j = 0; j < n_candidates; ++j) {
        const uint64_t key = (j == 1 && t == tid) ? second : lst[j];
        if (key == kKeyEmpty || key < bound) break;
        const uint32_t pos = atomicAdd(&sh.count, 1u);
        if (pos < static_cast<uint32_t>(kMaxSortCandidates)) sh.sel2[pos] = key;
      }
    }
    __syncthreads();
    const int survivors = static_cast<int>(sh.count);
    if (survivors <= kRankSortMax) {
      rank_sort_desc(sh.sel2, sh.sel, survivors);
      return survivors < n_candidates ? survivors : n_candidates;
    }
    if (survivors <= kMaxSortCandidates) {
      const int p2 = pow2_at_least(survivors);
      for (int t = tid; t < p2; t += nt) sh.sel[t] = t < survivors ? sh.sel2[t] : kKeyEmpty;
      bitonic_sort_desc<false>(sh.sel, nullptr, p2);
      return survivors < n_candidates ? survivors : n_candidates;
    }
  }
  return exact_top_candidates(ArrayKeys{keys, keys_per_query}, n_candidates, sh);
}

__global__ __launch_bounds__(kSelectThreads) void select_rerank_kernel(
    const uint64_t* __restrict__ keys_all, int64_t keys_per_query, int sorted_lists, int n_candidates, int k,
    RerankParams rp, const float* __restrict__ dewi32, const float* __restrict__ ent32, int64_t id_offset,
    int64_t* __restrict__ out_ids, float* __restrict__ out_scores, dewi_candidate* __restrict__ out_cand,
    const uint32_t* __restrict__ counts, SegmentLayout seg, RefineParams refine, QueryFlags flags) {
  __shared__ SelectShared sh;
  __shared__ uint32_t n_nan;
  const int tid = static_cast<int>(threadIdx.x), nt = static_cast<int>(blockDim.x);
  const int q = static_cast<int>(blockIdx.x);
  const uint64_t* keys = keys_all + static_cast<int64_t>(q) * keys_per_query;
  int n_sel;
  if (tid == 0) n_nan = 0;
  if (flags.mode == 2) {
    if (flags.p[q] == 0u) return;
  } else if (flags.mode == 1 && tid == 0) {
    flags.p[q] = 0u;
  }
  auto refuse = [&]() {
    if (flags.mode == 1) {
      if (tid == 0) flags.p[q] = 1u;
      return;
    }
    if (out_cand != nullptr) {
      for (int j = tid; j < n_candidates; j += nt) {
        dewi_candidate rec;
        rec.sim = __builtin_nanf("");
        rec.dewi = 0.f;
        rec.ent = 0.f;
        rec.id = -2;
        out_cand[static_cast<int64_t>(q) * n_candidates + j] = rec;
      }
      return;
    }
    for (int j = tid; j < k; j += nt) {
      out_ids[static_cast<int64_t>(q) * k + j] = -1;
      out_scores[static_cast<int64_t>(q) * k + j] = __builtin_nanf("");
    }
  };
  if (counts != nullptr) {
    SegmentKeys kv{keys_all + static_cast<int64_t>(q) * seg.cap, counts + q * seg.count_query_stride, seg.seg_stride, seg.count_stride, seg.n_seg,
                   seg.cap, seg.raw != 0};
    extern __shared__ __attribute__((aligned(16))) uint64_t dyn_keys[];
    __shared__ WideRadixShared ws;
    __shared__ uint32_t seg_base[kSelectThreads], seg_cnt[kSelectThreads];
    const uint32_t cap = static_cast<uint32_t>(seg.cap);
    if (tid == 0) sh.total = 0;
    __syncthreads();
    if (seg.n_seg <= nt && seg.raw != 0) {
      const int lane = tid & 63, wave = tid >> 6, n_waves = nt >> 6;
      uint32_t c = 0;
      if (tid < seg.n_seg) {
        c = kv.count[tid * kv.count_stride];
        if (c > cap) sh.total = 1;
        c = c < cap ? c : cap;
      }
      uint32_t incl = c;
      for (int off = 1; off < 64; off <<= 1) {
        const uint32_t o = __shfl_up(incl, off, kWave);
        if (lane >= off) incl += o;
      }
      if (lane == 63) ws.wave_tot[wave] = incl;
      __syncthreads();
      if (sh.total) {
        refuse();
        return;
      }
      uint32_t before = 0, total = 0;
      for (int w = 0; w < n_waves; ++w) {
        const uint32_t wt = ws.wave_tot[w];
        before += w < wave ? wt : 0u;
        total += wt;
      }
      seg_base[tid] = before + incl - c;
      seg_cnt[tid] = c;
      __syncthreads();
      if (total <= static_cast<uint32_t>(seg.lds_keys)) {
        constexpr int kGroup = 2, kBatch = 8;
        const int sub = tid % kGroup;
        for (int sg = tid / kGroup; sg < seg.n_seg; sg += nt / kGroup) {
          const uint32_t n_rec = seg_cnt[sg], b = seg_base[sg];
          const uint64_t* sp = kv.p + sg * kv.seg_stride;
          for (uint32_t j0 = 0; j0 < n_rec; j0 += kGroup * kBatch) {
            uint64_t v[kBatch];
#pragma unroll
            for (int u = 0; u < kBatch; ++u) {
              const uint32_t j = j0 + sub + u * kGroup;
              v[u] = j < n_rec ? sp[j] : 0ull;
            }
#pragma unroll
            for (int u = 0; u < kBatch; ++u) {
              const uint32_t j = j0 + sub + u * kGroup;
              if (j < n_rec)
                dyn_keys[b + j] = make_key(__uint_as_float(static_cast<uint32_t>(v[u])), static_cast<uint32_t>(v[u] >> 32));
            }
          }
        }
        __syncthreads();
        if (refine.E != nullptr) {
          n_sel = refine_top_candidates(dyn_keys, static_cast<int>(total), n_candidates, sh, ws, refine, q);
          if (n_sel == -2) {
            refuse();
            return;
          }
        } else {
          n_sel = top_candidates_lds(dyn_keys, static_cast<int>(total), n_candidates, sh, ws);
        }
      } else if (refine.E != nullptr) {
        n_sel = refine_from_segments(kv, dyn_keys, n_candidates, sh, refine, q);
        if (n_sel == -2) {
          refuse();
          return;
        }
      } else {
        n_sel = exact_top_candidates(kv, n_candidates, sh);
      }
    } else {
      for (int s = tid; s < seg.n_seg; s += nt)
        if (kv.count[s * kv.count_stride] > cap) sh.total = 1;
      __syncthreads();
      if (sh.total) {
        refuse();
        return;
      }
      __syncthreads();
      if (refine.E != nullptr) {
        n_sel = refine_from_segments(kv, dyn_keys, n_candidates, sh, refine, q);
        if (n_sel == -2) {
          refuse();
          return;
        }
      } else {
        if (tid == 0) sh.count = 0;
        __syncthreads();
        kv.for_each(tid, nt, [&](uint64_t key) {
          const uint32_t pos = atomicAdd(&sh.count, 1u);
          if (pos < static_cast<uint32_t>(seg.lds_keys)) dyn_keys[pos] = key;
        });
        __syncthreads();
        const uint32_t total = sh.count;
        __syncthreads();
        if (total <= static_cast<uint32_t>(seg.lds_keys))
          n_sel = exact_top_candidates(ArrayKeys{dyn_keys, static_cast<int64_t>(total)}, n_candidates, sh);
        else
          n_sel = exact_top_candidates(kv, n_candidates, sh);
      }
    }
  } else if (refine.E != nullptr && refine.list_len > 0) {
    extern __shared__ __attribute__((aligned(16))) uint64_t dyn_scratch[];
    n_sel = refine_from_sorted_lists(keys, sorted_lists, refine.list_len, n_candidates, sh, dyn_scratch, refine, q);
    if (n_sel == -2) {
      refuse();
      return;
    }
  } else {
    n_sel = gather_top_candidates(keys, keys_per_query, sorted_lists, n_candidates, sh);
  }
  if (out_cand != nullptr) {
    dewi_candidate* oc = out_cand + static_cast<int64_t>(q) * n_candidates;
    for (int t = tid; t < n_candidates; t += nt) {
      dewi_candidate rec;
      if (t < n_sel) {
        const uint32_t row = key_row(sh.sel[t]);
        rec.sim = key_score(sh.sel[t]);
        rec.dewi = dewi32[row];
        rec.ent = ent32[row];
        rec.id = static_cast<int32_t>(static_cast<int64_t>(row) + id_offset);
      } else {
        rec.sim = -__builtin_inff();
        rec.dewi = 0.f;
        rec.ent = 0.f;
        rec.id = -1;
      }
      oc[t] = rec;
    }
    return;
  }
  auto fetch = [&](int t, float& dewi, float& ent, int64_t& id) {
    const uint32_t row = key_row(sh.sel[t]);
    dewi = dewi32[row];
    ent = ent32[row];
    id = static_cast<int64_t>(row) + id_offset;
  };
  rerank_and_emit(sh, n_nan, n_sel, k, rp, fetch, out_ids + static_cast<int64_t>(q) * k,
                  out_scores + static_cast<int64_t>(q) * k);
}

__global__ __launch_bounds__(kSelectThreads) void merge_rerank_kernel(const dewi_candidate* __restrict__ lists,
                                                                      int n_lists, int n_queries, int list_len,
                                                                      int n_candidates, int k, RerankParams rp,
                                                                      int64_t* __restrict__ out_ids,
                                                                      float* __restrict__ out_scores) {
  __shared__ SelectShared sh;
  __shared__ uint32_t n_nan;
  const int tid = static_cast<int>(threadIdx.x), nt = static_cast<int>(blockDim.x);
  const int q = static_cast<int>(blockIdx.x);
  const int m = n_lists * list_len;
  const int p2 = pow2_at_least(m);
  if (tid == 0) {
    sh.count = 0;
    sh.total = 0;
    n_nan = 0;
  }
  __syncthreads();
  const bool small = m <= kRankSortMax;
  for (int t = tid; t < p2; t += nt) {
    uint64_t key = kKeyEmpty;
    uint32_t src = 0;
    if (t < m) {
      const int l = t / list_len, j = t % list_len;
      const int64_t at = (static_cast<int64_t>(l) * n_queries + q) * list_len + j;
      const dewi_candidate rec = lists[at];
      if (rec.id == -2) sh.total = 1;
      if (rec.id >= 0) {
        key = make_key(rec.sim, static_cast<uint32_t>(rec.id));
        src = static_cast<uint32_t>(t);
        atomicAdd(&sh.count, 1u);
      }
    }
    if (small) {
      sh.sel2[t] = key;
    } else {
      sh.sel[t] = key;
      sh.val[t] = src;
    }
  }
  __syncthreads();
  if (sh.total) {
    for (int j = tid; j < k; j += nt) {
      out_ids[static_cast<int64_t>(q) * k + j] = -1;
      out_scores[static_cast<int64_t>(q) * k + j] = __builtin_nanf("");
    }
    return;
  }
  if (small) {
    for (int t = tid; t < m; t += nt) {
      const uint64_t mine = sh.sel2[t];
      int rank = 0;
      for (int j = 0; j < m; ++j) {
        const uint64_t o = sh.sel2[j];
        rank += (o > mine || (o == mine && j < t)) ? 1 : 0;
      }
      sh.sel[rank] = mine;
      sh.val[rank] = static_cast<uint32_t>(t);
    }
    __syncthreads();
  } else {
    bitonic_sort_desc<true>(sh.sel, sh.val, p2);
  }
  const int n_sel = static_cast<int>(sh.count < static_cast<uint32_t>(n_candidates) ? sh.count : n_candidates);
  auto fetch = [&](int t, float& dewi, float& ent, int64_t& id) {
    const int s = static_cast<int>(sh.val[t]);
    const int l = s / list_len, j = s % list_len;
    const dewi_candidate rec = lists[(static_cast<int64_t>(l) * n_queries + q) * list_len + j];
    dewi = rec.dewi;
    ent = rec.ent;
    id = rec.id;
  };
  rerank_and_emit(sh, n_nan, n_sel, k, rp, fetch, out_ids + static_cast<int64_t>(q) * k,
                  out_scores + static_cast<int64_t>(q) * k);
}

__device__ void bitonic_sort_desc_global(uint64_t* key, int p2) {
  const int tid = static_cast<int>(threadIdx.x), nt = static_cast<int>(blockDim.x);
  for (int size = 2; size <= p2; size <<= 1) {
    for (int stride = size >> 1; stride > 0; stride >>= 1) {
      __syncthreads();
      for (int t = tid; t < (p2 >> 1); t += nt) {
// ... 129 lines not shown
      while (lo < hi) {
        const int mid = (lo + hi) >> 1;
        const uint64_t ok = record_key(other[mid]);
        const bool beats = ok > mine || (ok == mine && o < l);
        if (beats) lo = mid + 1; else hi = mid;
      }
      rank += lo;
    }
    if (rank < n_candidates) {
      g1[rank] = mine;
      src[rank] = static_cast<uint32_t>(t);
    }
  }
  __syncthreads();
  if (refused) {
    for (int j = tid; j < k; j += nt) {
      out_ids[static_cast<int64_t>(q) * k + j] = -1;
      out_scores[static_cast<int64_t>(q) * k + j] = __builtin_nanf("");
    }
    return;
  }
  const int n_sel = static_cast<int>(n_valid < static_cast<uint32_t>(n_candidates) ? n_valid : n_candidates);
  auto record_at = [&](int t) {
    const uint32_t s = src[t];
    return list_of(static_cast<int>(s / list_len))[s % list_len];
  };
  for (int t = tid; t < p2; t += nt) {
    uint64_t k2 = kKeyEmpty;
    if (t < n_sel) {
      const dewi_candidate rec = record_at(t);
      const float adj = blend(rp, rec.sim, rec.dewi, rec.ent);
      if (adj != adj) atomicAdd(&n_nan, 1u);
      k2 = (static_cast<uint64_t>(ord_f32(adj)) << 32) | static_cast<uint64_t>(0xFFFFFFFFu - static_cast<uint32_t>(t));
    }
    g2[t] = k2;
  }
  bitonic_sort_desc_global(g2, p2);
  const int kk = k < n_sel ? k : n_sel;
  for (int j = tid; j < kk; j += nt) {
    const uint64_t k2 = g2[j];
    const int t = static_cast<int>(0xFFFFFFFFu - static_cast<uint32_t>(k2));
    const uint32_t hi = static_cast<uint32_t>(k2 >> 32);
    const int at = emit_position(j, hi == kOrdNaN, kk, n_nan);
    out_ids[static_cast<int64_t>(q) * k + at] = record_at(t).id;
    out_scores[static_cast<int64_t>(q) * k + at] = unord_f32(hi);
  }
}

size_t merge_large_workspace_bytes(int n_queries, int n_candidates) {
  int p2 = 2;
  while (p2 < n_candidates) p2 <<= 1;
  return static_cast<size_t>(n_queries) * p2 * (8 + 8 + 4);
}

hipError_t launch_merge_rerank_large(const dewi_candidate* d_lists, int n_lists, int n_queries, int list_len,
                                     int n_candidates, int k, const RerankParams& rp, void* d_ws, int64_t* d_out_ids,
                                     float* d_out_scores, hipStream_t stream) {
  int p2 = 2;
  while (p2 < n_candidates) p2 <<= 1;
  uint64_t* g1 = static_cast<uint64_t*>(d_ws);
  uint64_t* g2 = g1 + static_cast<size_t>(n_queries) * p2;
  uint32_t* src = reinterpret_cast<uint32_t*>(g2 + static_cast<size_t>(n_queries) * p2);
  hipLaunchKernelGGL(merge_rerank_large_kernel, dim3(n_queries), dim3(kSelectThreads), 0, stream, d_lists, n_lists,
                     n_queries, list_len, n_candidates, p2, k, rp, g1, g2, src, d_out_ids, d_out_scores);
  return hipGetLastError();
}

hipError_t launch_select_rerank(const uint64_t* d_keys, int64_t keys_per_query, int sorted_lists, int n_queries,
                                int n_candidates, int k, const RerankParams& rp, const float* d_dewi32,
                                const float* d_ent32, int64_t id_offset, int64_t* d_out_ids, float* d_out_scores,
                                dewi_candidate* d_out_cand, const uint32_t* d_counts, const SegmentLayout& seg,
                                hipStream_t stream, const RefineParams& refine, const QueryFlags& flags) {
  int threads = kSelectThreads;
  const bool refine_lists = refine.E != nullptr && refine.list_len > 0;
  if (refine_lists) {
    if (d_counts != nullptr || sorted_lists <= 0 || sorted_lists > 4 * kWave || refine.list_len > kWave ||
        n_candidates > refine.list_len || refine.space != DEWI_SPACE_COSINE)
      return hipErrorInvalidValue;
  } else if (sorted_lists > 0) {
    threads = sorted_lists <= 4 * kWave ? 256 : kSelectThreads;
  } else if (keys_per_query <= 4096 && n_candidates <= 128 && refine.E == nullptr) {
    threads = 256;
  }
  if (flags.mode == 2) threads = 256;
  static const int threads_override = [] { const char* e = getenv("DEWI_SELECT_THREADS"); return e ? atoi(e) : 0; }();
  if (d_counts != nullptr && threads_override >= 256 && threads_override <= kSelectThreads && threads_override % kWave == 0)
    threads = threads_override;
  size_t dyn = refine_lists ? static_cast<size_t>(kMaxSortCandidates) * 8 : 0;
  if (d_counts != nullptr && seg.lds_keys > 0) {
    const int alloc_keys = (refine.E != nullptr && seg.lds_keys < kMaxSortCandidates) ? kMaxSortCandidates : seg.lds_keys;
    dyn = static_cast<size_t>(alloc_keys) * 8;
    static PerDeviceOnce attr_once;
    const hipError_t e = attr_once.run([] {
      return hipFuncSetAttribute(reinterpret_cast<const void*>(&select_rerank_kernel),
                                 hipFuncAttributeMaxDynamicSharedMemorySize, 96 * 1024);
    });
    if (e != hipSuccess) return e;
  }
  hipLaunchKernelGGL(select_rerank_kernel, dim3(n_queries), dim3(threads), dyn, stream, d_keys, keys_per_query,
                     sorted_lists, n_candidates, k, rp, d_dewi32, d_ent32, id_offset, d_out_ids, d_out_scores,
                     d_out_cand, d_counts, seg, refine, flags);
  return hipGetLastError();
}

hipError_t launch_merge_rerank(const dewi_candidate* d_lists, int n_lists, int n_queries, int list_len,
                               int n_candidates, int k, const RerankParams& rp, int64_t* d_out_ids,
                               float* d_out_scores, hipStream_t stream) {
  const int threads = n_lists * list_len <= 512 ? 256 : kSelectThreads;
  hipLaunchKernelGGL(merge_rerank_kernel, dim3(n_queries), dim3(threads), 0, stream, d_lists, n_lists, n_queries,
                     list_len, n_candidates, k, rp, d_out_ids, d_out_scores);
  return hipGetLastError();
}

}
```

Measured before the change: 2312 queries/s.

## Fuse repair select into flagged scan kernel via completion tickets

The separate select/rerank launch that followed the repair scan is removed. Each flagged scan block now runs a repair_select_tail, and a per-query ticket counter in the workspace elects the last finishing block to do the top-k selection and DEWI rerank. Select code is moved into shared helpers (gather_top_candidates, emit_selected) so the scan kernels can call them. This saves one kernel launch per batch, at the cost of extra shared memory in the scan kernels, an atomic ticket protocol, and a larger workspace.

```diff
diff --git a/dewi-design-for-an-entropy-weighted-index-for-text-image-corpora_amd/csrc/abi.cpp b/dewi-design-for-an-entropy-weighted-index-for-text-image-corpora_amd/csrc/abi.cpp
--- a/dewi-design-for-an-entropy-weighted-index-for-text-image-corpora_amd/csrc/abi.cpp
+++ b/dewi-design-for-an-entropy-weighted-index-for-text-image-corpora_amd/csrc/abi.cpp
@@ -239,8 +239,10 @@
   dewi::MfmaLayout big;
   bool shadow;
   size_t flags_off;
+  size_t tickets_off;
   size_t total;
 };
+size_t repair_words_bytes(int n_queries) { return 2 * align_up(static_cast<size_t>(n_queries) * 4, 256); }
 
 bool plan_repair(BatchPlan& P, size_t path_total, int64_t n_rows, int dim, int corpus_elem_bytes, int n_queries, int n_candidates,
                  int cus) {
@@ -248,7 +250,8 @@
   P.rows = layout_knn(n_rows, dim, corpus_elem_bytes, n_queries, n_candidates, cus);
   if (!dewi::scan_flagged_supported(P.rows.plan, corpus_elem_bytes)) return false;
   P.flags_off = align_up(path_total > P.rows.total ? path_total : P.rows.total, 256);
-  P.total = P.flags_off + align_up(static_cast<size_t>(n_queries) * 4, 256);
+  P.tickets_off = P.flags_off + repair_words_bytes(n_queries) / 2;
+  P.total = P.flags_off + repair_words_bytes(n_queries);
   return true;
 }
 
@@ -299,16 +302,14 @@
   const KnnLayout& L = P.rows;
   uint32_t* flags = reinterpret_cast<uint32_t*>(ws + P.flags_off);
   uint64_t* keys = reinterpret_cast<uint64_t*>(ws + L.keys_off);
-  hipError_t e = B.elem_type ? dewi::launch_scan_flagged_bf16(L.plan, static_cast<const uint16_t*>(B.d_E), B.n_rows, B.dim, B.d_Q,
-                                                              B.n_queries, n_candidates, B.space, keys, flags, B.stream)
-                             : dewi::launch_scan_flagged_f32(L.plan, static_cast<const float*>(B.d_E), B.n_rows, B.dim, B.d_Q,
-                                                             B.n_queries, n_candidates, B.space, keys, flags, B.stream);
-  if (e != hipSuccess) return hip_fail(e, "repair scan launch");
-  const int sorted = L.plan.slots == 1 ? L.plan.n_lists : 0;
-  e = dewi::launch_select_rerank(keys, L.plan.keys_per_query, sorted, B.n_queries, n_candidates, O.k, O.rp, O.d_dewi32, O.d_ent32,
-                                 O.id_offset, O.d_out_ids, O.d_out_scores, O.d_out_cand, nullptr, dewi::SegmentLayout{}, B.stream,
-                                 dewi::RefineParams{nullptr, nullptr, nullptr, 0, 0.f, 0}, dewi::QueryFlags{flags, 2});
-  return launched(e, "repair select launch");
+  const dewi::RepairSelect sel{reinterpret_cast<uint32_t*>(ws + P.tickets_off), L.plan.slots == 1 ? L.plan.n_lists : 0, O.k, O.rp,
+                               O.d_dewi32, O.d_ent32, O.id_offset, O.d_out_ids, O.d_out_scores, O.d_out_cand};
+  const hipError_t e =
+      B.elem_type ? dewi::launch_scan_flagged_bf16(L.plan, static_cast<const uint16_t*>(B.d_E), B.n_rows, B.dim, B.d_Q, B.n_queries,
+                                                   n_candidates, B.space, keys, flags, sel, B.stream)
+                  : dewi::launch_scan_flagged_f32(L.plan, static_cast<const float*>(B.d_E), B.n_rows, B.dim, B.d_Q, B.n_queries,
+                                                  n_candidates, B.space, keys, flags, sel, B.stream);
+  return launched(e, "repair launch");
 }
 
 int batch_select(const BatchPlan& P, const Batch& B, const SelectOut& O, int n_candidates, void* d_ws, size_t ws_bytes) {
@@ -345,6 +346,7 @@
   const bool refine_l2 = !big && B.space == DEWI_SPACE_L2 && B.elem_type == 0;
   if (!B.d_E || !B.d_Q) return fail(DEWI_ERR_INVALID_ARG, "a matrix-core batch needs the corpus and the raw queries in its finish step (repair of refused queries)");
   uint32_t* flags = reinterpret_cast<uint32_t*>(ws + P.flags_off);
+  uint32_t* tickets = reinterpret_cast<uint32_t*>(ws + P.tickets_off);
   for (int g = 0; g < groups && e == hipSuccess; ++g) {
     const int q0 = g * per;
     const int nq = n_queries - q0 < per ? n_queries - q0 : per;
@@ -363,7 +365,7 @@
                                    O.d_out_ids ? O.d_out_ids + static_cast<int64_t>(q0) * k : nullptr,
                                    O.d_out_scores ? O.d_out_scores + static_cast<int64_t>(q0) * k : nullptr,
                                    O.d_out_cand ? O.d_out_cand + static_cast<int64_t>(q0) * n_candidates : nullptr, counts, seg,
-                                   B.stream, rf, dewi::QueryFlags{flags + q0, 1});
+                                   B.stream, rf, dewi::QueryFlags{flags + q0, 1, tickets + q0});
   }
   if (e != hipSuccess) return hip_fail(e, "select launch");
   return batch_repair(P, ws, B, O, n_candidates);
@@ -510,7 +512,7 @@
       }
     }
   }
-  return align_up(a, 256) + align_up(static_cast<size_t>(n_queries) * 4, 256);
+  return align_up(a, 256) + repair_words_bytes(n_queries);
 }
 
 int dewi_knn_scan_kernel(int elem_type, int64_t n_rows, int dim, int n_queries, int n_candidates, int space, char* out,
@@ -584,7 +586,8 @@
     const hipError_t e = dewi::launch_select_rerank(reinterpret_cast<const uint64_t*>(ws + L.keys_off), L.plan.keys_per_query,
                                                     L.plan.n_lists, 1, S.c, k, O.rp, d_dewi32, d_ent32, 0, d_out_ids, d_out_scores,
                                                     nullptr, nullptr, dewi::SegmentLayout{}, stream, rf,
-                                                    dewi::QueryFlags{reinterpret_cast<uint32_t*>(ws + P.flags_off), 1});
+                                                    dewi::QueryFlags{reinterpret_cast<uint32_t*>(ws + P.flags_off), 1,
+                                                                     reinterpret_cast<uint32_t*>(ws + P.tickets_off)});
     if (e != hipSuccess) return hip_fail(e, "select launch (one query, bf16 shadow)");
     return batch_repair(P, ws, B, O, S.c);
   }
diff --git a/dewi-design-for-an-entropy-weighted-index-for-text-image-corpora_amd/csrc/knn_scan.hip b/dewi-design-for-an-entropy-weighted-index-for-text-image-corpora_amd/csrc/knn_scan.hip
--- a/dewi-design-for-an-entropy-weighted-index-for-text-image-corpora_amd/csrc/knn_scan.hip
+++ b/dewi-design-for-an-entropy-weighted-index-for-text-image-corpora_amd/csrc/knn_scan.hip
@@ -178,11 +178,15 @@
 __global__ __launch_bounds__(kScanThreads) void scan_rows_f32_flagged(const float* __restrict__ E, int64_t n_rows,
                                                                       const float* __restrict__ Q, int n_candidates,
                                                                       uint64_t* __restrict__ keys, int64_t keys_per_query,
-                                                                      const uint32_t* __restrict__ flags, int n_queries) {
+                                                                      const uint32_t* __restrict__ flags, int n_queries,
+                                                                      RepairSelect sel) {
   __shared__ MergeShared merge_buf;
+  __shared__ RepairShared tail;
   for_each_flagged(flags, n_queries, [&](int q) {
-    scan_rows_f32_body<U, R, 1, SPACE, S, true>(E, n_rows, Q + static_cast<int64_t>(q) * (256 * U), n_candidates,
-                                                keys + static_cast<int64_t>(q) * keys_per_query, keys_per_query, merge_buf);
+    uint64_t* keys_q = keys + static_cast<int64_t>(q) * keys_per_query;
+    scan_rows_f32_body<U, R, 1, SPACE, S, true>(E, n_rows, Q + static_cast<int64_t>(q) * (256 * U), n_candidates, keys_q,
+                                                keys_per_query, merge_buf);
+    repair_select_tail(q, keys_q, keys_per_query, n_candidates, sel, tail);
   });
 }
 
@@ -720,20 +724,20 @@
 
 template <int U, int SPACE>
 static hipError_t launch_flagged_s(const ScanPlan& plan, const float* E, int64_t n_rows, const float* Q, int n_queries, int c,
-                                   uint64_t* keys, const uint32_t* flags, hipStream_t stream) {
+                                   uint64_t* keys, const uint32_t* flags, const RepairSelect& sel, hipStream_t stream) {
   constexpr int R = U == 1 ? 4 : (U == 2 ? 2 : 1);
   switch (plan.slots) {
     case 0:
       hipLaunchKernelGGL((scan_rows_f32_flagged<U, R, SPACE, 0>), dim3(plan.blocks), dim3(kScanThreads), 0, stream, E, n_rows, Q, c,
-                         keys, plan.keys_per_query, flags, n_queries);
+                         keys, plan.keys_per_query, flags, n_queries, sel);
       break;
     case 1:
       hipLaunchKernelGGL((scan_rows_f32_flagged<U, R, SPACE, 1>), dim3(plan.blocks), dim3(kScanThreads), 0, stream, E, n_rows, Q, c,
-                         keys, plan.keys_per_query, flags, n_queries);
+                         keys, plan.keys_per_query, flags, n_queries, sel);
       break;
     default:
       hipLaunchKernelGGL((scan_rows_f32_flagged<U, R, SPACE, kMaxSlots>), dim3(plan.blocks), dim3(kScanThreads), 0, stream, E, n_rows,
-                         Q, c, keys, plan.keys_per_query, flags, n_queries);
+                         Q, c, keys, plan.keys_per_query, flags, n_queries, sel);
       break;
   }
   return hipGetLastError();
@@ -747,15 +751,15 @@
 
 hipError_t launch_scan_flagged_f32(const ScanPlan& plan, const float* d_E, int64_t n_rows, int dim, const float* d_q_raw,
                                    int n_queries, int n_candidates, int space, uint64_t* d_keys, const uint32_t* d_flags,
-                                   hipStream_t stream) {
+                                   const RepairSelect& sel, hipStream_t stream) {
   if (plan.kind == kScanAnyLong || plan.kind == kScanAnyShort)
-    return launch_scan_any_flagged_f32(plan, d_E, n_rows, dim, d_q_raw, n_queries, n_candidates, space, d_keys, d_flags, stream);
+    return launch_scan_any_flagged_f32(plan, d_E, n_rows, dim, d_q_raw, n_queries, n_candidates, space, d_keys, d_flags, sel, stream);
   if (plan.kind != kScanFast) return hipErrorInvalidValue;
 #define DEWI_FLAGGED(UU)                                                                                                 \
   case UU:                                                                                                               \
     return space == DEWI_SPACE_COSINE                                                                                    \
-               ? launch_flagged_s<UU, DEWI_SPACE_COSINE>(plan, d_E, n_rows, d_q_raw, n_queries, n_candidates, d_keys, d_flags, stream) \
-               : launch_flagged_s<UU, DEWI_SPACE_L2>(plan, d_E, n_rows, d_q_raw, n_queries, n_candidates, d_keys, d_flags, stream);
+               ? launch_flagged_s<UU, DEWI_SPACE_COSINE>(plan, d_E, n_rows, d_q_raw, n_queries, n_candidates, d_keys, d_flags, sel, stream) \
+               : launch_flagged_s<UU, DEWI_SPACE_L2>(plan, d_E, n_rows, d_q_raw, n_queries, n_candidates, d_keys, d_flags, sel, stream);
   switch (dim / 256) {
     DEWI_FLAGGED(1)
     DEWI_FLAGGED(2)
diff --git a/dewi-design-for-an-entropy-weighted-index-for-text-image-corpora_amd/csrc/knn_scan_any_bf16.hip b/dewi-design-for-an-entropy-weighted-index-for-text-image-corpora_amd/csrc/knn_scan_any_bf16.hip
--- a/dewi-design-for-an-entropy-weighted-index-for-text-image-corpora_amd/csrc/knn_scan_any_bf16.hip
+++ b/dewi-design-for-an-entropy-weighted-index-for-text-image-corpora_amd/csrc/knn_scan_any_bf16.hip
@@ -9,9 +9,9 @@
 
 hipError_t launch_scan_any_flagged_bf16(const ScanPlan& plan, const uint16_t* d_E, int64_t n_rows, int dim, const float* d_q_raw,
                                         int n_queries, int n_candidates, int space, uint64_t* d_keys, const uint32_t* d_flags,
-                                        hipStream_t stream) {
+                                        const RepairSelect& sel, hipStream_t stream) {
   (void)dim;
-  return launch_scan_any_flagged_impl<1>(plan, d_E, n_rows, d_q_raw, n_queries, n_candidates, space, d_keys, d_flags, stream);
+  return launch_scan_any_flagged_impl<1>(plan, d_E, n_rows, d_q_raw, n_queries, n_candidates, space, d_keys, d_flags, sel, stream);
 }
 
 }
diff --git a/dewi-design-for-an-entropy-weighted-index-for-text-image-corpora_amd/csrc/knn_scan_any_f32.hip b/dewi-design-for-an-entropy-weighted-index-for-text-image-corpora_amd/csrc/knn_scan_any_f32.hip
--- a/dewi-design-for-an-entropy-weighted-index-for-text-image-corpora_amd/csrc/knn_scan_any_f32.hip
+++ b/dewi-design-for-an-entropy-weighted-index-for-text-image-corpora_amd/csrc/knn_scan_any_f32.hip
@@ -15,9 +15,9 @@
 
 hipError_t launch_scan_any_flagged_f32(const ScanPlan& plan, const float* d_E, int64_t n_rows, int dim, const float* d_q_raw,
                                        int n_queries, int n_candidates, int space, uint64_t* d_keys, const uint32_t* d_flags,
-                                       hipStream_t stream) {
+                                       const RepairSelect& sel, hipStream_t stream) {
   (void)dim;
-  return launch_scan_any_flagged_impl<0>(plan, d_E, n_rows, d_q_raw, n_queries, n_candidates, space, d_keys, d_flags, stream);
+  return launch_scan_any_flagged_impl<0>(plan, d_E, n_rows, d_q_raw, n_queries, n_candidates, space, d_keys, d_flags, sel, stream);
 }
 
 }
diff --git a/dewi-design-for-an-entropy-weighted-index-for-text-image-corpora_amd/csrc/knn_scan_bf16.hip b/dewi-design-for-an-entropy-weighted-index-for-text-image-corpora_amd/csrc/knn_scan_bf16.hip
--- a/dewi-design-for-an-entropy-weighted-index-for-text-image-corpora_amd/csrc/knn_scan_bf16.hip
+++ b/dewi-design-for-an-entropy-weighted-index-for-text-image-corpora_amd/csrc/knn_scan_bf16.hip
@@ -1,3 +1,4 @@
+#include "repair_tail.hpp"
 #include "scan_common.hpp"
 
 #ifndef DEWI_BF16_PAIRS
@@ -156,11 +157,15 @@
 __global__ __launch_bounds__(kScanThreads) void scan_rows_bf16_flagged(const uint16_t* __restrict__ E, int64_t n_rows,
                                                                        const float* __restrict__ Q, int n_candidates,
                                                                        uint64_t* __restrict__ keys, int64_t keys_per_query,
-                                                                       const uint32_t* __restrict__ flags, int n_queries) {
+                                                                       const uint32_t* __restrict__ flags, int n_queries,
+                                                                       RepairSelect sel) {
   __shared__ MergeShared merge_buf;
+  __shared__ RepairShared tail;
   for_each_flagged(flags, n_queries, [&](int q) {
-    scan_rows_bf16_body<H, 1, SPACE, S, true>(E, n_rows, Q + static_cast<int64_t>(q) * (256 * H), n_candidates,
-                                              keys + static_cast<int64_t>(q) * keys_per_query, keys_per_query, merge_buf);
+    uint64_t* keys_q = keys + static_cast<int64_t>(q) * keys_per_query;
+    scan_rows_bf16_body<H, 1, SPACE, S, true>(E, n_rows, Q + static_cast<int64_t>(q) * (256 * H), n_candidates, keys_q,
+                                              keys_per_query, merge_buf);
+    repair_select_tail(q, keys_q, keys_per_query, n_candidates, sel, tail);
   });
 }
 
@@ -270,19 +275,19 @@
 
 template <int H, int SPACE>
 static hipError_t launch_flagged_bf16_s(const ScanPlan& plan, const uint16_t* E, int64_t n_rows, const float* Q, int n_queries, int c,
-                                        uint64_t* keys, const uint32_t* flags, hipStream_t stream) {
+                                        uint64_t* keys, const uint32_t* flags, const RepairSelect& sel, hipStream_t stream) {
   switch (plan.slots) {
     case 0:
       hipLaunchKernelGGL((scan_rows_bf16_flagged<H, SPACE, 0>), dim3(plan.blocks), dim3(kScanThreads), 0, stream, E, n_rows, Q, c, keys,
-                         plan.keys_per_query, flags, n_queries);
+                         plan.keys_per_query, flags, n_queries, sel);
       break;
     case 1:
       hipLaunchKernelGGL((scan_rows_bf16_flagged<H, SPACE, 1>), dim3(plan.blocks), dim3(kScanThreads), 0, stream, E, n_rows, Q, c, keys,
-                         plan.keys_per_query, flags, n_queries);
+                         plan.keys_per_query, flags, n_queries, sel);
       break;
     default:
       hipLaunchKernelGGL((scan_rows_bf16_flagged<H, SPACE, kMaxSlots>), dim3(plan.blocks), dim3(kScanThreads), 0, stream, E, n_rows, Q,
-                         c, keys, plan.keys_per_query, flags, n_queries);
+                         c, keys, plan.keys_per_query, flags, n_queries, sel);
       break;
   }
   return hipGetLastError();
@@ -290,15 +295,15 @@
 
 hipError_t launch_scan_flagged_bf16(const ScanPlan& plan, const uint16_t* d_E, int64_t n_rows, int dim, const float* d_q_raw,
                                     int n_queries, int n_candidates, int space, uint64_t* d_keys, const uint32_t* d_flags,
-                                    hipStream_t stream) {
+                                    const RepairSelect& sel, hipStream_t stream) {
   if (plan.kind == kScanAnyLong || plan.kind == kScanAnyShort)
-    return launch_scan_any_flagged_bf16(plan, d_E, n_rows, dim, d_q_raw, n_queries, n_candidates, space, d_keys, d_flags, stream);
+    return launch_scan_any_flagged_bf16(plan, d_E, n_rows, dim, d_q_raw, n_queries, n_candidates, space, d_keys, d_flags, sel, stream);
   if (plan.kind != kScanFast) return hipErrorInvalidValue;
 #define DEWI_FLAGGED(HH)                                                                                                      \
   case HH:                                                                                                                    \
     return space == DEWI_SPACE_COSINE                                                                                         \
-               ? launch_flagged_bf16_s<HH, DEWI_SPACE_COSINE>(plan, d_E, n_rows, d_q_raw, n_queries, n_candidates, d_keys, d_flags, stream) \
-               : launch_flagged_bf16_s<HH, DEWI_SPACE_L2>(plan, d_E, n_rows, d_q_raw, n_queries, n_candidates, d_keys, d_flags, stream);
+               ? launch_flagged_bf16_s<HH, DEWI_SPACE_COSINE>(plan, d_E, n_rows, d_q_raw, n_queries, n_candidates, d_keys, d_flags, sel, stream) \
+               : launch_flagged_bf16_s<HH, DEWI_SPACE_L2>(plan, d_E, n_rows, d_q_raw, n_queries, n_candidates, d_keys, d_flags, sel, stream);
   switch (dim / 256) {
     DEWI_FLAGGED(1)
     DEWI_FLAGGED(2)
diff --git a/dewi-design-for-an-entropy-weighted-index-for-text-image-corpora_amd/csrc/launch.hpp b/dewi-design-for-an-entropy-weighted-index-for-text-image-corpora_amd/csrc/launch.hpp
--- a/dewi-design-for-an-entropy-weighted-index-for-text-image-corpora_amd/csrc/launch.hpp
+++ b/dewi-design-for-an-entropy-weighted-index-for-text-image-corpora_amd/csrc/launch.hpp
@@ -145,19 +145,20 @@
 hipError_t launch_scan_odd_bf16(const ScanPlan& plan, const uint16_t* d_E, int64_t n_rows, int dim, const float* d_q_raw, int q0,
                                 int nq, int n_candidates, int space, uint64_t* d_keys, hipStream_t stream);
 
+struct RepairSelect;
 bool scan_flagged_supported(const ScanPlan& plan, int elem_bytes);
 hipError_t launch_scan_flagged_f32(const ScanPlan& plan, const float* d_E, int64_t n_rows, int dim, const float* d_q_raw,
                                    int n_queries, int n_candidates, int space, uint64_t* d_keys, const uint32_t* d_flags,
-                                   hipStream_t stream);
+                                   const RepairSelect& sel, hipStream_t stream);
 hipError_t launch_scan_flagged_bf16(const ScanPlan& plan, const uint16_t* d_E, int64_t n_rows, int dim, const float* d_q_raw,
                                     int n_queries, int n_candidates, int space, uint64_t* d_keys, const uint32_t* d_flags,
-                                    hipStream_t stream);
+                                    const RepairSelect& sel, hipStream_t stream);
 hipError_t launch_scan_any_flagged_f32(const ScanPlan& plan, const float* d_E, int64_t n_rows, int dim, const float* d_q_raw,
                                        int n_queries, int n_candidates, int space, uint64_t* d_keys, const uint32_t* d_flags,
-                                       hipStream_t stream);
+                                       const RepairSelect& sel, hipStream_t stream);
 hipError_t launch_scan_any_flagged_bf16(const ScanPlan& plan, const uint16_t* d_E, int64_t n_rows, int dim, const float* d_q_raw,
                                         int n_queries, int n_candidates, int space, uint64_t* d_keys, const uint32_t* d_flags,
-                                        hipStream_t stream);
+                                        const RepairSelect& sel, hipStream_t stream);
 
 hipError_t launch_scan_bf16(const ScanPlan& plan, const uint16_t* d_E, int64_t n_rows, int dim, const float* d_q_raw,
                             const float* d_q_norm, int q0, int nq, int n_candidates, int space, uint64_t* d_keys,
@@ -221,6 +222,18 @@
   int transform;
   int space;
 };
+struct RepairSelect {
+  uint32_t* tickets;
+  int sorted_lists;
+  int k;
+  RerankParams rp;
+  const float* dewi32;
+  const float* ent32;
+  int64_t id_offset;
+  int64_t* out_ids;
+  float* out_scores;
+  dewi_candidate* out_cand;
+};
 struct SegmentLayout {
   int n_seg;
   int cap;
@@ -246,6 +259,7 @@
 struct QueryFlags {
   uint32_t* p;
   int mode;
+  uint32_t* tickets;
 };
 hipError_t launch_select_rerank(const uint64_t* d_keys, int64_t keys_per_query, int sorted_lists, int n_queries,
                                 int n_candidates, int k, const RerankParams& rp, const float* d_dewi32, const float* d_ent32,
diff --git a/dewi-design-for-an-entropy-weighted-index-for-text-image-corpora_amd/csrc/repair_tail.hpp b/dewi-design-for-an-entropy-weighted-index-for-text-image-corpora_amd/csrc/repair_tail.hpp
--- /dev/null
+++ b/dewi-design-for-an-entropy-weighted-index-for-text-image-corpora_amd/csrc/repair_tail.hpp
@@ -0,0 +1,35 @@
+#pragma once
+#include "select_body.hpp"
+
+namespace dewi {
+
+struct RepairShared {
+  SelectShared sel;
+  uint32_t n_nan;
+  uint32_t ticket;
+};
+
+__device__ __forceinline__ void repair_select_tail(int q, const uint64_t* keys, int64_t keys_per_query, int n_candidates,
+                                                   const RepairSelect& rs, RepairShared& sh) {
+  asm volatile("s_waitcnt vmcnt(0)" ::: "memory");
+  __syncthreads();
+  if (threadIdx.x == 0) {
+    __builtin_amdgcn_fence(__ATOMIC_RELEASE, "agent");
+    asm volatile("s_waitcnt vmcnt(0)" ::: "memory");
+    sh.ticket = __hip_atomic_fetch_add(rs.tickets + q, 1u, __ATOMIC_RELAXED, __HIP_MEMORY_SCOPE_AGENT);
+    sh.n_nan = 0;
+  }
+  __syncthreads();
+  if (sh.ticket != gridDim.x - 1u) return;
+  if (threadIdx.x == 0) {
+    __builtin_amdgcn_fence(__ATOMIC_ACQUIRE, "agent");
+    asm volatile("s_waitcnt vmcnt(0)" ::: "memory");
+  }
+  __syncthreads();
+  const int n_sel = gather_top_candidates(keys, keys_per_query, rs.sorted_lists, n_candidates, sh.sel);
+  emit_selected(sh.sel, sh.n_nan, n_sel, q, n_candidates, rs.k, rs.rp, rs.dewi32, rs.ent32, rs.id_offset, rs.out_ids,
+                rs.out_scores, rs.out_cand);
+  __syncthreads();
+}
+
+}
diff --git a/dewi-design-for-an-entropy-weighted-index-for-text-image-corpora_amd/csrc/scan_any.hpp b/dewi-design-for-an-entropy-weighted-index-for-text-image-corpora_amd/csrc/scan_any.hpp
--- a/dewi-design-for-an-entropy-weighted-index-for-text-image-corpora_amd/csrc/scan_any.hpp
+++ b/dewi-design-for-an-entropy-weighted-index-for-text-image-corpora_amd/csrc/scan_any.hpp
@@ -1,4 +1,5 @@
 #pragma once
+#include "repair_tail.hpp"
 #include "scan_common.hpp"
 
 namespace dewi {
@@ -423,12 +424,16 @@
 __global__ __launch_bounds__(kScanThreads) void scan_rows_any_flagged(const u32x4* __restrict__ E, int64_t n_rows, int units,
                                                                       const float* __restrict__ Q, int n_candidates,
                                                                       uint64_t* __restrict__ keys, int64_t keys_per_query,
-                                                                      const uint32_t* __restrict__ flags, int n_queries) {
+                                                                      const uint32_t* __restrict__ flags, int n_queries,
+                                                                      RepairSelect sel) {
   __shared__ MergeShared merge_buf;
+  __shared__ RepairShared tail;
   const int dim = units * (ELEM ? 8 : 4);
   for_each_flagged(flags, n_queries, [&](int q) {
-    scan_rows_any_body<ELEM, U, R, 1, SPACE, S>(E, n_rows, units, Q + static_cast<int64_t>(q) * dim, n_candidates,
-                                                keys + static_cast<int64_t>(q) * keys_per_query, keys_per_query, merge_buf);
+    uint64_t* keys_q = keys + static_cast<int64_t>(q) * keys_per_query;
+    scan_rows_any_body<ELEM, U, R, 1, SPACE, S>(E, n_rows, units, Q + static_cast<int64_t>(q) * dim, n_candidates, keys_q,
+                                                keys_per_query, merge_buf);
+    repair_select_tail(q, keys_q, keys_per_query, n_candidates, sel, tail);
   });
 }
 
@@ -617,12 +622,16 @@
                                                                             int log2p, const float* __restrict__ Q,
                                                                             int n_candidates, uint64_t* __restrict__ keys,
                                                                             int64_t keys_per_query,
-                                                                            const uint32_t* __restrict__ flags, int n_queries) {
+                                                                            const uint32_t* __restrict__ flags, int n_queries,
+                                                                            RepairSelect sel) {
   __shared__ MergeShared merge_buf;
+  __shared__ RepairShared tail;
   const int dim = units * (ELEM ? 8 : 4);
   for_each_flagged(flags, n_queries, [&](int q) {
+    uint64_t* keys_q = keys + static_cast<int64_t>(q) * keys_per_query;
     scan_short_rows_any_body<ELEM, R, 1, SPACE, S>(E, n_rows, units, log2p, Q + static_cast<int64_t>(q) * dim, n_candidates,
-                                                   keys + static_cast<int64_t>(q) * keys_per_query, keys_per_query, merge_buf);
+                                                   keys_q, keys_per_query, merge_buf);
+    repair_select_tail(q, keys_q, keys_per_query, n_candidates, sel, tail);
   });
 }
 
@@ -781,16 +790,16 @@
 
 template <int ELEM, int SPACE, int S>
 static hipError_t launch_any_flagged_s(const ScanPlan& plan, const u32x4* E, int64_t n_rows, const float* Q, int n_queries, int c,
-                                       uint64_t* keys, const uint32_t* flags, hipStream_t stream) {
+                                       uint64_t* keys, const uint32_t* flags, const RepairSelect& sel, hipStream_t stream) {
   if (plan.kind == kScanAnyShort) {
     hipLaunchKernelGGL((scan_short_rows_any_flagged<ELEM, kAnyShortRows, SPACE, S>), dim3(plan.blocks), dim3(kScanThreads), 0, stream,
-                       E, n_rows, plan.units, plan.log2p, Q, c, keys, plan.keys_per_query, flags, n_queries);
+                       E, n_rows, plan.units, plan.log2p, Q, c, keys, plan.keys_per_query, flags, n_queries, sel);
     return hipGetLastError();
   }
 #define DEWI_ANY_FLAGGED(UU)                                                                                                     \
   case UU:                                                                                                                       \
     hipLaunchKernelGGL((scan_rows_any_flagged<ELEM, UU, any_rows(UU, 1, 1), SPACE, S>), dim3(plan.blocks), dim3(kScanThreads), 0,  \
-                       stream, E, n_rows, plan.units, Q, c, keys, plan.keys_per_query, flags, n_queries);                         \
+                       stream, E, n_rows, plan.units, Q, c, keys, plan.keys_per_query, flags, n_queries, sel);                    \
     return hipGetLastError();
   switch (plan.u_pad) {
     DEWI_ANY_FLAGGED(1)
@@ -809,13 +818,13 @@
 template <int ELEM>
 static hipError_t launch_scan_any_flagged_impl(const ScanPlan& plan, const void* d_E, int64_t n_rows, const float* d_q_raw,
                                                int n_queries, int n_candidates, int space, uint64_t* d_keys,
-                                               const uint32_t* d_flags, hipStream_t stream) {
+                                               const uint32_t* d_flags, const RepairSelect& sel, hipStream_t stream) {
   const u32x4* E = static_cast<const u32x4*>(d_E);
 #define DEWI_ANY_FS(SPACE)                                                                                                         \
   switch (plan.slots) {                                                                                                            \
-    case 0: return launch_any_flagged_s<ELEM, SPACE, 0>(plan, E, n_rows, d_q_raw, n_queries, n_candidates, d_keys, d_flags, stream); \
-    case 1: return launch_any_flagged_s<ELEM, SPACE, 1>(plan, E, n_rows, d_q_raw, n_queries, n_candidates, d_keys, d_flags, stream); \
-    default: return launch_any_flagged_s<ELEM, SPACE, kMaxSlots>(plan, E, n_rows, d_q_raw, n_queries, n_candidates, d_keys, d_flags, stream); \
+    case 0: return launch_any_flagged_s<ELEM, SPACE, 0>(plan, E, n_rows, d_q_raw, n_queries, n_candidates, d_keys, d_flags, sel, stream); \
+    case 1: return launch_any_flagged_s<ELEM, SPACE, 1>(plan, E, n_rows, d_q_raw, n_queries, n_candidates, d_keys, d_flags, sel, stream); \
+    default: return launch_any_flagged_s<ELEM, SPACE, kMaxSlots>(plan, E, n_rows, d_q_raw, n_queries, n_candidates, d_keys, d_flags, sel, stream); \
   }
   if (space == DEWI_SPACE_COSINE) {
     DEWI_ANY_FS(DEWI_SPACE_COSINE)
diff --git a/dewi-design-for-an-entropy-weighted-index-for-text-image-corpora_amd/csrc/select_body.hpp b/dewi-design-for-an-entropy-weighted-index-for-text-image-corpora_amd/csrc/select_body.hpp
--- /dev/null
+++ b/dewi-design-for-an-entropy-weighted-index-for-text-image-corpora_amd/csrc/select_body.hpp
@@ -0,0 +1,292 @@
+#pragma once
+#include "blend.hpp"
+#include "select_common.hpp"
+
+namespace dewi {
+
+__device__ __forceinline__ int pow2_at_least(int v) {
+  int p = 2;
+  while (p < v) p <<= 1;
+  return p;
+}
+
+constexpr uint32_t kOrdNaN = 0xFFFFFFFFu;
+__device__ __forceinline__ int emit_position(int j, bool is_nan, int kk, uint32_t n_nan) {
+  const int z = n_nan < static_cast<uint32_t>(kk) ? static_cast<int>(n_nan) : kk;
+  return is_nan ? kk - z + j : j - z;
+}
+
+template <class Fetch>
+__device__ void rerank_and_emit(SelectShared& sh, uint32_t& n_nan, int n_sel, int k, const RerankParams& rp, Fetch fetch,
+                                int64_t* __restrict__ out_ids, float* __restrict__ out_scores) {
+  const int tid = static_cast<int>(threadIdx.x), nt = static_cast<int>(blockDim.x);
+  const int p2 = pow2_at_least(n_sel);
+  const int kk = k < n_sel ? k : n_sel;
+  int64_t my_id = -1;
+  for (int t = tid; t < p2; t += nt) {
+    uint64_t k2 = kKeyEmpty;
+    if (t < n_sel) {
+      float dewi, ent;
+      int64_t id;
+      fetch(t, dewi, ent, id);
+      if (t == tid) my_id = id;
+      const float adj = blend(rp, key_score(sh.sel[t]), dewi, ent);
+      if (adj != adj) atomicAdd(&n_nan, 1u);
+      k2 = (static_cast<uint64_t>(ord_f32(adj)) << 32) | static_cast<uint64_t>(0xFFFFFFFFu - static_cast<uint32_t>(t));
+    }
+    sh.sel2[t] = k2;
+  }
+  if (n_sel <= kRankSortMax) {
+    __syncthreads();
+    const int S = rank_split(n_sel, nt);
+    if (S == 1) {
+      for (int t = tid; t < n_sel; t += nt) {
+        const uint64_t mine = sh.sel2[t];
+        int rank = 0;
+#pragma unroll 4
+        for (int j = 0; j < n_sel; ++j) rank += sh.sel2[j] > mine ? 1 : 0;
+        if (rank < k) {
+          int64_t id = my_id;
+          if (t != tid) {
+            float dewi, ent;
+            fetch(t, dewi, ent, id);
+          }
+          const uint32_t hi = static_cast<uint32_t>(mine >> 32);
+          const int at = emit_position(rank, hi == kOrdNaN, kk, n_nan);
+          out_ids[at] = id;
+          out_scores[at] = unord_f32(hi);
+        }
+      }
+    } else {
+      const int part = tid & (S - 1);
+      for (int t = tid / S; t < n_sel; t += nt / S) {
+        const uint64_t mine = sh.sel2[t];
+        int rank = 0;
+        const int iters = (n_sel + S - 1) / S;
+#pragma unroll 8
+        for (int i = 0; i < iters; ++i) {
+          const int j = part + i * S;
+          rank += sh.sel2[j < p2 ? j : p2 - 1] > mine ? 1 : 0;
+        }
+        for (int m = 1; m < S; m <<= 1) rank += __shfl_xor(rank, m, kWave);
+        if (part == 0 && rank < k) {
+          float dewi, ent;
+          int64_t id;
+          fetch(t, dewi, ent, id);
+          const uint32_t hi = static_cast<uint32_t>(mine >> 32);
+          const int at = emit_position(rank, hi == kOrdNaN, kk, n_nan);
+          out_ids[at] = id;
+          out_scores[at] = unord_f32(hi);
+        }
+      }
+    }
+    return;
+  }
+  bitonic_sort_desc<false>(sh.sel2, nullptr, p2);
+  for (int j = tid; j < kk; j += nt) {
+    const uint64_t k2 = sh.sel2[j];
+    const int t = static_cast<int>(0xFFFFFFFFu - static_cast<uint32_t>(k2));
+    float dewi, ent;
+    int64_t id;
+    fetch(t, dewi, ent, id);
+    const uint32_t hi = static_cast<uint32_t>(k2 >> 32);
+    const int at = emit_position(j, hi == kOrdNaN, kk, n_nan);
+    out_ids[at] = id;
+    out_scores[at] = unord_f32(hi);
+  }
+}
+
+template <class Keys>
+__device__ int exact_top_candidates(const Keys& keys, int n_candidates, SelectShared& sh) {
+  const int tid = static_cast<int>(threadIdx.x), nt = static_cast<int>(blockDim.x);
+  const uint64_t thr = block_kth_largest(keys, static_cast<uint32_t>(n_candidates), sh);
+  if (tid == 0) sh.count = 0;
+  const int p2 = pow2_at_least(n_candidates);
+  for (int t = tid; t < p2; t += nt) sh.sel[t] = kKeyEmpty;
+  __syncthreads();
+  keys.for_each(tid, nt, [&](uint64_t key) {
+    if (key >= thr) {
+      const uint32_t pos = atomicAdd(&sh.count, 1u);
+      if (pos < static_cast<uint32_t>(p2)) sh.sel[pos] = key;
+    }
+  });
+  __syncthreads();
+  const int n_sel = static_cast<int>(sh.count < static_cast<uint32_t>(n_candidates) ? sh.count : n_candidates);
+  if (n_sel <= kRankSortMax && sh.count <= static_cast<uint32_t>(kRankSortMax)) {
+    for (int t = tid; t < n_sel; t += nt) sh.sel2[t] = sh.sel[t];
+    __syncthreads();
+    rank_sort_desc(sh.sel2, sh.sel, n_sel);
+    return n_sel;
+  }
+  bitonic_sort_desc<false>(sh.sel, nullptr, p2);
+  return n_sel;
+}
+
+__device__ inline int gather_top_candidates(const uint64_t* __restrict__ keys, int64_t keys_per_query, int sorted_lists,
+                                            int n_candidates, SelectShared& sh) {
+  const int tid = static_cast<int>(threadIdx.x), nt = static_cast<int>(blockDim.x);
+  if (sorted_lists > 0 && sorted_lists <= 4 * kWave && n_candidates <= kWave) {
+    if (tid == 0) {
+      sh.n_contrib = 0;
+      sh.count = 0;
+    }
+    __syncthreads();
+    if (tid < kWave) {
+      uint64_t m[4];
+      uint64_t lane_max = kKeyEmpty;
+#pragma unroll
+      for (int u = 0; u < 4; ++u) {
+        const int l = tid + kWave * u;
+        m[u] = l < sorted_lists ? keys[static_cast<int64_t>(l) * n_candidates] : kKeyEmpty;
+        lane_max = m[u] > lane_max ? m[u] : lane_max;
+      }
+      const uint32_t mh = static_cast<uint32_t>(lane_max >> 32), ml = static_cast<uint32_t>(lane_max);
+      int rank = 0;
+#pragma unroll
+      for (int j = 0; j < kWave; ++j) {
+        const uint64_t o = (static_cast<uint64_t>(static_cast<uint32_t>(__builtin_amdgcn_readlane(static_cast<int>(mh), j))) << 32) |
+                           static_cast<uint32_t>(__builtin_amdgcn_readlane(static_cast<int>(ml), j));
+        rank += (o > lane_max || (o == lane_max && j < tid)) ? 1 : 0;
+      }
+      const unsigned long long who = __ballot(rank == n_candidates - 1);
+      uint64_t bound = 1ull;
+      if (who != 0ull) {
+        const int src = __ffsll(who) - 1;
+        bound = (static_cast<uint64_t>(static_cast<uint32_t>(__builtin_amdgcn_readlane(static_cast<int>(mh), src))) << 32) |
+                static_cast<uint32_t>(__builtin_amdgcn_readlane(static_cast<int>(ml), src));
+        if (bound == kKeyEmpty) bound = 1ull;
+      }
+#pragma unroll
+      for (int u = 0; u < 4; ++u) {
+        if (m[u] != kKeyEmpty && m[u] >= bound) sh.val[atomicAdd(&sh.n_contrib, 1u)] = static_cast<uint32_t>(tid + kWave * u);
+      }
+      if (tid == 0) sh.bound = bound;
+    }
+    __syncthreads();
+    const uint64_t bound = sh.bound;
+    for (int t = tid; t < static_cast<int>(sh.n_contrib); t += nt) {
+      const uint64_t* lst = keys + static_cast<int64_t>(sh.val[t]) * n_candidates;
+      for (int j = 0; j < n_candidates; ++j) {
+        const uint64_t key = lst[j];
+        if (key == kKeyEmpty || key < bound) break;
+        const uint32_t pos = atomicAdd(&sh.count, 1u);
+        if (pos < static_cast<uint32_t>(kMaxSortCandidates)) sh.sel2[pos] = key;
+      }
+    }
+    __syncthreads();
+    const int survivors = static_cast<int>(sh.count);
+    if (survivors <= kRankSortMax) {
+      rank_sort_desc(sh.sel2, sh.sel, survivors);
+      return survivors < n_candidates ? survivors : n_candidates;
+    }
+    if (survivors <= kMaxSortCandidates) {
+      const int p2 = pow2_at_least(survivors);
+      for (int t = tid; t < p2; t += nt) sh.sel[t] = t < survivors ? sh.sel2[t] : kKeyEmpty;
+      bitonic_sort_desc<false>(sh.sel, nullptr, p2);
+      return survivors < n_candidates ? survivors : n_candidates;
+    }
+    __syncthreads();
+  } else
+  if (sorted_lists > 0 && sorted_lists <= kMaxSortCandidates) {
+    uint64_t second = kKeyEmpty;
+    for (int t = tid; t < sorted_lists; t += nt) {
+      const uint64_t* lst = keys + static_cast<int64_t>(t) * n_candidates;
+      sh.sel2[t] = lst[0];
+      if (t == tid && n_candidates > 1) second = lst[1];
+    }
+    if (tid == 0) {
+      sh.count = 0;
+      sh.total = 0;
+      sh.pick_digit = 0;
+    }
+    __syncthreads();
+    const bool all_lists = sorted_lists < n_candidates;
+    for (int t = tid; t < sorted_lists; t += nt) sh.val[t] = 0;
+    __syncthreads();
+    const int parts = nt / sorted_lists > 1 ? nt / sorted_lists : 1;
+    const int slice = (sorted_lists + parts - 1) / parts;
+    for (int idx = tid; idx < sorted_lists * parts; idx += nt) {
+      const int t = idx / parts, part = idx % parts;
+      const uint64_t mine = sh.sel2[t];
+      const int j0 = part * slice, j1 = j0 + slice < sorted_lists ? j0 + slice : sorted_lists;
+      uint32_t cnt = 0;
+      for (int j = j0; j < j1; ++j) {
+        const uint64_t o = sh.sel2[j];
+        cnt += (o > mine || (o == mine && j < t)) ? 1u : 0u;
+      }
+      if (cnt) atomicAdd(&sh.val[t], cnt);
+    }
+    __syncthreads();
+    for (int t = tid; t < sorted_lists; t += nt) {
+      if (sh.val[t] == static_cast<uint32_t>(n_candidates - 1)) {
+        sh.pick_digit = static_cast<uint32_t>(t);
+        sh.total = 1;
+      }
+    }
+    __syncthreads();
+    uint64_t bound = 1ull;
+    if (!all_lists && sh.total != 0) bound = sh.sel2[sh.pick_digit];
+    if (bound == kKeyEmpty) bound = 1ull;
+    __syncthreads();
+    for (int t = tid; t < sorted_lists; t += nt) {
+      if (!all_lists && sh.val[t] >= static_cast<uint32_t>(n_candidates)) continue;
+      const uint64_t* lst = keys + static_cast<int64_t>(t) * n_candidates;
+      for (int j = 0; j < n_candidates; ++j) {
+        const uint64_t key = (j == 1 && t == tid) ? second : lst[j];
+        if (key == kKeyEmpty || key < bound) break;
+        const uint32_t pos = atomicAdd(&sh.count, 1u);
+        if (pos < static_cast<uint32_t>(kMaxSortCandidates)) sh.sel2[pos] = key;
+      }
+    }
+    __syncthreads();
+    const int survivors = static_cast<int>(sh.count);
+    if (survivors <= kRankSortMax) {
+      rank_sort_desc(sh.sel2, sh.sel, survivors);
+      return survivors < n_candidates ? survivors : n_candidates;
+    }
+    if (survivors <= kMaxSortCandidates) {
+      const int p2 = pow2_at_least(survivors);
+      for (int t = tid; t < p2; t += nt) sh.sel[t] = t < survivors ? sh.sel2[t] : kKeyEmpty;
+      bitonic_sort_desc<false>(sh.sel, nullptr, p2);
+      return survivors < n_candidates ? survivors : n_candidates;
+    }
+  }
+  return exact_top_candidates(ArrayKeys{keys, keys_per_query}, n_candidates, sh);
+}
+
+__device__ __forceinline__ void emit_selected(SelectShared& sh, uint32_t& n_nan, int n_sel, int q, int n_candidates, int k,
+                                              const RerankParams& rp, const float* __restrict__ dewi32,
+                                              const float* __restrict__ ent32, int64_t id_offset, int64_t* __restrict__ out_ids,
+                                              float* __restrict__ out_scores, dewi_candidate* __restrict__ out_cand) {
+  const int tid = static_cast<int>(threadIdx.x), nt = static_cast<int>(blockDim.x);
+  if (out_cand != nullptr) {
+    dewi_candidate* oc = out_cand + static_cast<int64_t>(q) * n_candidates;
+    for (int t = tid; t < n_candidates; t += nt) {
+      dewi_candidate rec;
+      if (t < n_sel) {
+        const uint32_t row = key_row(sh.sel[t]);
+        rec.sim = key_score(sh.sel[t]);
+        rec.dewi = dewi32[row];
+        rec.ent = ent32[row];
+        rec.id = static_cast<int32_t>(static_cast<int64_t>(row) + id_offset);
+      } else {
+        rec.sim = -__builtin_inff();
+        rec.dewi = 0.f;
+        rec.ent = 0.f;
+        rec.id = -1;
+      }
+      oc[t] = rec;
+    }
+    return;
+  }
+  auto fetch = [&](int t, float& dewi, float& ent, int64_t& id) {
+    const uint32_t row = key_row(sh.sel[t]);
+    dewi = dewi32[row];
+    ent = ent32[row];
+    id = static_cast<int64_t>(row) + id_offset;
+  };
+  rerank_and_emit(sh, n_nan, n_sel, k, rp, fetch, out_ids + static_cast<int64_t>(q) * k,
+                  out_scores + static_cast<int64_t>(q) * k);
+}
+
+}
diff --git a/dewi-design-for-an-entropy-weighted-index-for-text-image-corpora_amd/csrc/select_rerank.hip b/dewi-design-for-an-entropy-weighted-index-for-text-image-corpora_amd/csrc/select_rerank.hip
--- a/dewi-design-for-an-entropy-weighted-index-for-text-image-corpora_amd/csrc/select_rerank.hip
+++ b/dewi-design-for-an-entropy-weighted-index-for-text-image-corpora_amd/csrc/select_rerank.hip
@@ -1,127 +1,8 @@
 #include <stdlib.h>
 
-#include "blend.hpp"
-#include "select_common.hpp"
+#include "select_body.hpp"
 
 namespace dewi {
-
-__device__ __forceinline__ int pow2_at_least(int v) {
-  int p = 2;
-  while (p < v) p <<= 1;
-  return p;
-}
-
-constexpr uint32_t kOrdNaN = 0xFFFFFFFFu;
-__device__ __forceinline__ int emit_position(int j, bool is_nan, int kk, uint32_t n_nan) {
-  const int z = n_nan < static_cast<uint32_t>(kk) ? static_cast<int>(n_nan) : kk;
-  return is_nan ? kk - z + j : j - z;
-}
-
-template <class Fetch>
-__device__ void rerank_and_emit(SelectShared& sh, uint32_t& n_nan, int n_sel, int k, const RerankParams& rp, Fetch fetch,
-                                int64_t* __restrict__ out_ids, float* __restrict__ out_scores) {
-  const int tid = static_cast<int>(threadIdx.x), nt = static_cast<int>(blockDim.x);
-  const int p2 = pow2_at_least(n_sel);
-  const int kk = k < n_sel ? k : n_sel;
-  int64_t my_id = -1;
-  for (int t = tid; t < p2; t += nt) {
-    uint64_t k2 = kKeyEmpty;
-    if (t < n_sel) {
-      float dewi, ent;
-      int64_t id;
-      fetch(t, dewi, ent, id);
-      if (t == tid) my_id = id;
-      const float adj = blend(rp, key_score(sh.sel[t]), dewi, ent);
-      if (adj != adj) atomicAdd(&n_nan, 1u);
-      k2 = (static_cast<uint64_t>(ord_f32(adj)) << 32) | static_cast<uint64_t>(0xFFFFFFFFu - static_cast<uint32_t>(t));
-    }
-    sh.sel2[t] = k2;
-  }
-  if (n_sel <= kRankSortMax) {
-    __syncthreads();
-    const int S = rank_split(n_sel, nt);
-    if (S == 1) {
-      for (int t = tid; t < n_sel; t += nt) {
-        const uint64_t mine = sh.sel2[t];
-        int rank = 0;
-#pragma unroll 4
-        for (int j = 0; j < n_sel; ++j) rank += sh.sel2[j] > mine ? 1 : 0;
-        if (rank < k) {
-          int64_t id = my_id;
-          if (t != tid) {
-            float dewi, ent;
-            fetch(t, dewi, ent, id);
-          }
-          const uint32_t hi = static_cast<uint32_t>(mine >> 32);
-          const int at = emit_position(rank, hi == kOrdNaN, kk, n_nan);
-          out_ids[at] = id;
-          out_scores[at] = unord_f32(hi);
-        }
-      }
-    } else {
-      const int part = tid & (S - 1);
-      for (int t = tid / S; t < n_sel; t += nt / S) {
-        const uint64_t mine = sh.sel2[t];
-        int rank = 0;
-        const int iters = (n_sel + S - 1) / S;
-#pragma unroll 8
-        for (int i = 0; i < iters; ++i) {
-          const int j = part + i * S;
-          rank += sh.sel2[j < p2 ? j : p2 - 1] > mine ? 1 : 0;
-        }
-        for (int m = 1; m < S; m <<= 1) rank += __shfl_xor(rank, m, kWave);
-        if (part == 0 && rank < k) {
-          float dewi, ent;
-          int64_t id;
-          fetch(t, dewi, ent, id);
-          const uint32_t hi = static_cast<uint32_t>(mine >> 32);
-          const int at = emit_position(rank, hi == kOrdNaN, kk, n_nan);
-          out_ids[at] = id;
-          out_scores[at] = unord_f32(hi);
-        }
-      }
-    }
-    return;
-  }
-  bitonic_sort_desc<false>(sh.sel2, nullptr, p2);
-  for (int j = tid; j < kk; j += nt) {
-    const uint64_t k2 = sh.sel2[j];
-    const int t = static_cast<int>(0xFFFFFFFFu - static_cast<uint32_t>(k2));
-    float dewi, ent;
-    int64_t id;
-    fetch(t, dewi, ent, id);
-    const uint32_t hi = static_cast<uint32_t>(k2 >> 32);
-    const int at = emit_position(j, hi == kOrdNaN, kk, n_nan);
-    out_ids[at] = id;
-    out_scores[at] = unord_f32(hi);
-  }
-}
-
-template <class Keys>
-__device__ int exact_top_candidates(const Keys& keys, int n_candidates, SelectShared& sh) {
-  const int tid = static_cast<int>(threadIdx.x), nt = static_cast<int>(blockDim.x);
-  const uint64_t thr = block_kth_largest(keys, static_cast<uint32_t>(n_candidates), sh);
-  if (tid == 0) sh.count = 0;
-  const int p2 = pow2_at_least(n_candidates);
-  for (int t = tid; t < p2; t += nt) sh.sel[t] = kKeyEmpty;
-  __syncthreads();
-  keys.for_each(tid, nt, [&](uint64_t key) {
-    if (key >= thr) {
-      const uint32_t pos = atomicAdd(&sh.count, 1u);
-      if (pos < static_cast<uint32_t>(p2)) sh.sel[pos] = key;
-    }
-  });
-  __syncthreads();
-  const int n_sel = static_cast<int>(sh.count < static_cast<uint32_t>(n_candidates) ? sh.count : n_candidates);
-  if (n_sel <= kRankSortMax && sh.count <= static_cast<uint32_t>(kRankSortMax)) {
-    for (int t = tid; t < n_sel; t += nt) sh.sel2[t] = sh.sel[t];
-    __syncthreads();
-    rank_sort_desc(sh.sel2, sh.sel, n_sel);
-    return n_sel;
-  }
-  bitonic_sort_desc<false>(sh.sel, nullptr, p2);
-  return n_sel;
-}
 
 __device__ int top_candidates_lds(const uint64_t* keys, int n, int n_candidates, SelectShared& sh, WideRadixShared& ws) {
   const int tid = static_cast<int>(threadIdx.x), nt = static_cast<int>(blockDim.x);
@@ -364,138 +245,6 @@
   return refine_rescore_units<4, 4>(keys, n_candidates, sh, rf, q);
 }
 
-__device__ int gather_top_candidates(const uint64_t* __restrict__ keys, int64_t keys_per_query, int sorted_lists,
-                                     int n_candidates, SelectShared& sh) {
-  const int tid = static_cast<int>(threadIdx.x), nt = static_cast<int>(blockDim.x);
-  if (sorted_lists > 0 && sorted_lists <= 4 * kWave && n_candidates <= kWave) {
-    if (tid == 0) {
-      sh.n_contrib = 0;
-      sh.count = 0;
-    }
-    __syncthreads();
-    if (tid < kWave) {
-      uint64_t m[4];
-      uint64_t lane_max = kKeyEmpty;
-#pragma unroll
-      for (int u = 0; u < 4; ++u) {
-        const int l = tid + kWave * u;
-        m[u] = l < sorted_lists ? keys[static_cast<int64_t>(l) * n_candidates] : kKeyEmpty;
-        lane_max = m[u] > lane_max ? m[u] : lane_max;
-      }
-      const uint32_t mh = static_cast<uint32_t>(lane_max >> 32), ml = static_cast<uint32_t>(lane_max);
-      int rank = 0;
-#pragma unroll
-      for (int j = 0; j < kWave; ++j) {
-        const uint64_t o = (static_cast<uint64_t>(static_cast<uint32_t>(__builtin_amdgcn_readlane(static_cast<int>(mh), j))) << 32) |
-                           static_cast<uint32_t>(__builtin_amdgcn_readlane(static_cast<int>(ml), j));
-        rank += (o > lane_max || (o == lane_max && j < tid)) ? 1 : 0;
-      }
-      const unsigned long long who = __ballot(rank == n_candidates - 1);
-      uint64_t bound = 1ull;
-      if (who != 0ull) {
-        const int src = __ffsll(who) - 1;
-        bound = (static_cast<uint64_t>(static_cast<uint32_t>(__builtin_amdgcn_readlane(static_cast<int>(mh), src))) << 32) |
-                static_cast<uint32_t>(__builtin_amdgcn_readlane(static_cast<int>(ml), src));
-        if (bound == kKeyEmpty) bound = 1ull;
-      }
-#pragma unroll
-      for (int u = 0; u < 4; ++u) {
-        if (m[u] != kKeyEmpty && m[u] >= bound) sh.val[atomicAdd(&sh.n_contrib, 1u)] = static_cast<uint32_t>(tid + kWave * u);
-      }
-      if (tid == 0) sh.bound = bound;
-    }
-    __syncthreads();
-    const uint64_t bound = sh.bound;
-    for (int t = tid; t < static_cast<int>(sh.n_contrib); t += nt) {
-      const uint64_t* lst = keys + static_cast<int64_t>(sh.val[t]) * n_candidates;
-      for (int j = 0; j < n_candidates; ++j) {
-        const uint64_t key = lst[j];
-        if (key == kKeyEmpty || key < bound) break;
-        const uint32_t pos = atomicAdd(&sh.count, 1u);
-        if (pos < static_cast<uint32_t>(kMaxSortCandidates)) sh.sel2[pos] = key;
-      }
-    }
-    __syncthreads();
-    const int survivors = static_cast<int>(sh.count);
-    if (survivors <= kRankSortMax) {
-      rank_sort_desc(sh.sel2, sh.sel, survivors);
-      return survivors < n_candidates ? survivors : n_candidates;
-    }
-    if (survivors <= kMaxSortCandidates) {
-      const int p2 = pow2_at_least(survivors);
-      for (int t = tid; t < p2; t += nt) sh.sel[t] = t < survivors ? sh.sel2[t] : kKeyEmpty;
-      bitonic_sort_desc<false>(sh.sel, nullptr, p2);
-      return survivors < n_candidates ? survivors : n_candidates;
-    }
-    __syncthreads();
-  } else
-  if (sorted_lists > 0 && sorted_lists <= kMaxSortCandidates) {
-    uint64_t second = kKeyEmpty;
-    for (int t = tid; t < sorted_lists; t += nt) {
-      const uint64_t* lst = keys + static_cast<int64_t>(t) * n_candidates;
-      sh.sel2[t] = lst[0];
-      if (t == tid && n_candidates > 1) second = lst[1];
-    }
-    if (tid == 0) {
-      sh.count = 0;
-      sh.total = 0;
-      sh.pick_digit = 0;
-    }
-    __syncthreads();
-    const bool all_lists = sorted_lists < n_candidates;
-    for (int t = tid; t < sorted_lists; t += nt) sh.val[t] = 0;
-    __syncthreads();
-    const int parts = nt / sorted_lists > 1 ? nt / sorted_lists : 1;
-    const int slice = (sorted_lists + parts - 1) / parts;
-    for (int idx = tid; idx < sorted_lists * parts; idx += nt) {
-      const int t = idx / parts, part = idx % parts;
-      const uint64_t mine = sh.sel2[t];
-      const int j0 = part * slice, j1 = j0 + slice < sorted_lists ? j0 + slice : sorted_lists;
-      uint32_t cnt = 0;
-      for (int j = j0; j < j1; ++j) {
-        const uint64_t o = sh.sel2[j];
-        cnt += (o > mine || (o == mine && j < t)) ? 1u : 0u;
-      }
-      if (cnt) atomicAdd(&sh.val[t], cnt);
-    }
-    __syncthreads();
-    for (int t = tid; t < sorted_lists; t += nt) {
-      if (sh.val[t] == static_cast<uint32_t>(n_candidates - 1)) {
-        sh.pick_digit = static_cast<uint32_t>(t);
-        sh.total = 1;
-      }
-    }
-    __syncthreads();
-    uint64_t bound = 1ull;
-    if (!all_lists && sh.total != 0) bound = sh.sel2[sh.pick_digit];
-    if (bound == kKeyEmpty) bound = 1ull;
-    __syncthreads();
-    for (int t = tid; t < sorted_lists; t += nt) {
-      if (!all_lists && sh.val[t] >= static_cast<uint32_t>(n_candidates)) continue;
-      const uint64_t* lst = keys + static_cast<int64_t>(t) * n_candidates;
-      for (int j = 0; j < n_candidates; ++j) {
-        const uint64_t key = (j == 1 && t == tid) ? second : lst[j];
-        if (key == kKeyEmpty || key < bound) break;
-        const uint32_t pos = atomicAdd(&sh.count, 1u);
-        if (pos < static_cast<uint32_t>(kMaxSortCandidates)) sh.sel2[pos] = key;
-      }
-    }
-    __syncthreads();
-    const int survivors = static_cast<int>(sh.count);
-    if (survivors <= kRankSortMax) {
-      rank_sort_desc(sh.sel2, sh.sel, survivors);
-      return survivors < n_candidates ? survivors : n_candidates;
-    }
-    if (survivors <= kMaxSortCandidates) {
-      const int p2 = pow2_at_least(survivors);
-      for (int t = tid; t < p2; t += nt) sh.sel[t] = t < survivors ? sh.sel2[t] : kKeyEmpty;
-      bitonic_sort_desc<false>(sh.sel, nullptr, p2);
-      return survivors < n_candidates ? survivors : n_candidates;
-    }
-  }
-  return exact_top_candidates(ArrayKeys{keys, keys_per_query}, n_candidates, sh);
-}
-
 __global__ __launch_bounds__(kSelectThreads) void select_rerank_kernel(
     const uint64_t* __restrict__ keys_all, int64_t keys_per_query, int sorted_lists, int n_candidates, int k,
     RerankParams rp, const float* __restrict__ dewi32, const float* __restrict__ ent32, int64_t id_offset,
@@ -508,10 +257,9 @@
   const uint64_t* keys = keys_all + static_cast<int64_t>(q) * keys_per_query;
   int n_sel;
   if (tid == 0) n_nan = 0;
-  if (flags.mode == 2) {
-    if (flags.p[q] == 0u) return;
-  } else if (flags.mode == 1 && tid == 0) {
+  if (flags.mode == 1 && tid == 0) {
     flags.p[q] = 0u;
+    flags.tickets[q] = 0u;
   }
   auto refuse = [&]() {
     if (flags.mode == 1) {
@@ -652,34 +400,7 @@
   } else {
     n_sel = gather_top_candidates(keys, keys_per_query, sorted_lists, n_candidates, sh);
   }
-  if (out_cand != nullptr) {
-    dewi_candidate* oc = out_cand + static_cast<int64_t>(q) * n_candidates;
-    for (int t = tid; t < n_candidates; t += nt) {
-      dewi_candidate rec;
-      if (t < n_sel) {
-        const uint32_t row = key_row(sh.sel[t]);
-        rec.sim = key_score(sh.sel[t]);
-        rec.dewi = dewi32[row];
-        rec.ent = ent32[row];
-        rec.id = static_cast<int32_t>(static_cast<int64_t>(row) + id_offset);
-      } else {
-        rec.sim = -__builtin_inff();
-        rec.dewi = 0.f;
-        rec.ent = 0.f;
-        rec.id = -1;
-      }
-      oc[t] = rec;
-    }
-    return;
-  }
-  auto fetch = [&](int t, float& dewi, float& ent, int64_t& id) {
-    const uint32_t row = key_row(sh.sel[t]);
-    dewi = dewi32[row];
-    ent = ent32[row];
-    id = static_cast<int64_t>(row) + id_offset;
-  };
-  rerank_and_emit(sh, n_nan, n_sel, k, rp, fetch, out_ids + static_cast<int64_t>(q) * k,
-                  out_scores + static_cast<int64_t>(q) * k);
+  emit_selected(sh, n_nan, n_sel, q, n_candidates, k, rp, dewi32, ent32, id_offset, out_ids, out_scores, out_cand);
 }
 
 __global__ __launch_bounds__(kSelectThreads) void merge_rerank_kernel(const dewi_candidate* __restrict__ lists,
@@ -975,7 +696,7 @@
   } else if (keys_per_query <= 4096 && n_candidates <= 128 && refine.E == nullptr) {
     threads = 256;
   }
-  if (flags.mode == 2) threads = 256;
+  if (flags.mode != 0 && (flags.mode != 1 || flags.p == nullptr || flags.tickets == nullptr)) return hipErrorInvalidValue;
   static const int threads_override = [] { const char* e = getenv("DEWI_SELECT_THREADS"); return e ? atoi(e) : 0; }();
   if (d_counts != nullptr && threads_override >= 256 && threads_override <= kSelectThreads && threads_override % kWave == 0)
     threads = threads_override;
```

Result: no change. 2321 queries/s, median of 6 (+0.4%).
